# penghao-wu/vstar

Hardware: AMD Instinct MI355X
Metric: searched crops/sec (336x336 tiles, 7B VSM bf16) (higher is better)
Workload: dtype bf16; 1 GPU; BASELINE config 2: 32-crop batches/GPU, CLIP-ViT-L/14@336 (P=576) + LLaMA-7B prefill S=640 + OWL-ViT-B/16@768 + det/SAM heads, records all-gathered per step; seq_len=640, parallelism=dp1

## Files before the change

include/vstar_hip.h:

```cpp
#ifndef VSTAR_HIP_H
#define VSTAR_HIP_H

#include <stdint.h>
#include <stddef.h>

#ifdef __cplusplus
extern "C" {
#endif

#define VSTAR_ABI_VERSION 1

enum { VSTAR_F32 = 0, VSTAR_F16 = 1, VSTAR_BF16 = 2 };

enum {
  VSTAR_OK = 0,
  VSTAR_ERR_INVALID = -1,
  VSTAR_ERR_STATE = -2,
  VSTAR_ERR_MISSING = -3,
  VSTAR_ERR_HIP = -4,
  VSTAR_ERR_NOMEM = -5
};

typedef struct vstar_config {
  int32_t abi_version;
  int32_t clip_image_size;
  int32_t clip_patch;
  int32_t clip_hidden;
  int32_t clip_heads;
  int32_t clip_mlp;
  int32_t clip_layers;
  int32_t clip_select_layer;
  int32_t llm_hidden;
  int32_t llm_heads;
  int32_t llm_mlp;
  int32_t llm_layers;
  int32_t llm_vocab;
  float   llm_rms_eps;
  float   llm_rope_theta;
  int32_t owl_image_size;
  int32_t owl_patch;
  int32_t owl_hidden;
  int32_t owl_heads;
  int32_t owl_mlp;
  int32_t owl_layers;
  int32_t owl_query_dim;
  int32_t max_batch;
  int32_t max_text_len;
  int32_t llm_w8a8;
  int32_t reserved[7];
} vstar_config;

typedef struct vstar_engine vstar_handle;

#define VSTAR_N_BOXES 2304
#define VSTAR_MASK_RES 192
#define VSTAR_MAX_VERIFY 8
typedef struct vstar_result {
  float   pred_logits[VSTAR_N_BOXES];
  float   pred_boxes[VSTAR_N_BOXES * 4];
  float   lowres_mask[VSTAR_MASK_RES * VSTAR_MASK_RES];
  int32_t tf_argmax[VSTAR_MAX_VERIFY];
} vstar_result;

int vstar_create(const vstar_config* cfg, int device, vstar_handle** out);
void vstar_destroy(vstar_handle* h);
const char* vstar_last_error(const vstar_handle* h);
const char* vstar_build_source_hash(void);

int vstar_load_tensor(vstar_handle* h, const char* hf_key, const void* host_ptr, int dtype,
                      int ndim, const int64_t* shape);
int vstar_finalize_weights(vstar_handle* h);

#define VSTAR_F_SKIP_OWL       1u
#define VSTAR_F_DEVICE_INPUTS  2u
#define VSTAR_F_DEVICE_OUTPUT  4u
#define VSTAR_F_NO_SYNC        8u
#define VSTAR_F_INTERNAL_PIXELS 16u
#define VSTAR_F_SHARE_PREFIX   32u
int vstar_vsm_score_batch(vstar_handle* h, int B, const uint16_t* clip_pix, const uint16_t* owl_pix,
                          const int32_t* ids, int L, const int32_t* loc_pos,
                          const int32_t* verify_pos, int n_verify, unsigned flags, vstar_result* out);

int vstar_vsm_score_grouped(vstar_handle* h, int G, int T, const uint16_t* clip_pix, const uint16_t* owl_pix,
                            const int32_t* prefix_ids, int Lp, const int32_t* suffix_ids, int Ls, const int32_t* loc_in_suffix,
                            const int32_t* verify_in_suffix, int n_verify, unsigned flags, vstar_result* out);

int vstar_image_set(vstar_handle* h, const uint8_t* rgb, int height, int width);
int vstar_preprocess_crops(vstar_handle* h, int B, const int32_t* boxes_xyxy);

#define VSTAR_MAX_IMAGE_SLOTS 64
int vstar_image_set_slot(vstar_handle* h, int slot, const uint8_t* rgb, int height, int width);
int vstar_preprocess_crops_slots(vstar_handle* h, int B, const int32_t* boxes_xyxy, const int32_t* slots);
int vstar_image_set_slot_async(vstar_handle* h, int slot, const uint8_t* rgb, int height, int width);

int vstar_vsm_generate(vstar_handle* h, const uint16_t* clip_pix_bf16, const int32_t* ids, int L, int max_new_tokens,
                       int eos_id, unsigned flags, int32_t* out_ids, int32_t* n_out);

int vstar_upsample_mask(vstar_handle* h, const float* lowres, int h_out, int w_out, float* out);
int vstar_upsample_mask_ex(vstar_handle* h, const float* lowres, int h_out, int w_out, int clamp_min0, float* out);

int vstar_heatmap_stats(vstar_handle* h, const float* lowres, int h_out, int w_out, int n_rects, const int32_t* rects_xywh,
                        double* out);
int vstar_heatmap_stats_batch(vstar_handle* h, int n, const float* lowres, const int32_t* out_hw, const int32_t* n_rects,
                              const int32_t* rects_xywh, double* out);

int64_t vstar_debug_read(vstar_handle* h, const char* name, float* out, int64_t cap);

void* vstar_stream(vstar_handle* h);

#define VSTAR_COMM_ID_BYTES 128
int vstar_comm_unique_id(uint8_t* id_out );
int vstar_comm_init(vstar_handle* h, const uint8_t* id, int world, int rank);
int vstar_allgather_results(vstar_handle* h, const vstar_result* local_dev, int n_local, vstar_result* gathered_dev, unsigned flags);
int vstar_comm_destroy(vstar_handle* h);

int vstar_profile_enable(vstar_handle* h, int on);
int vstar_profile_read(vstar_handle* h, double* gemm_ms, int64_t* gemm_launches, double* gemm_flops);
int vstar_profile_read_fp8(vstar_handle* h, double* gemm_ms, int64_t* gemm_launches, double* gemm_flops);

enum { VSTAR_EPI_NONE = 0, VSTAR_EPI_QUICK_GELU = 1, VSTAR_EPI_GELU = 2, VSTAR_EPI_RELU = 3, VSTAR_EPI_SILU_MUL = 4,
       VSTAR_EPI_NOSYNC = 0x100,
       VSTAR_EPI_TILE128 = 0x200,
       VSTAR_EPI_TILE256 = 0x400,
       VSTAR_EPI_TILE4W = 0x800    };

int vstar_op_gemm(void* stream, const uint16_t* dev_A, int64_t lda, const uint16_t* dev_W, const uint16_t* dev_bias,
                  const uint16_t* dev_residual, int64_t ldr, void* dev_C, int64_t ldc, int out_f32,
                  int M, int N, int K, int epilogue);
int vstar_op_gemm_norm(void* stream, const uint16_t* dev_A, int64_t lda, const uint16_t* dev_W, const uint16_t* dev_bias,
                       const uint16_t* dev_residual, int64_t ldr, void* dev_C, int64_t ldc, int M, int N, int K, int epilogue,
                       const float* dev_row_scale, float* dev_sumsq_out, int sumsq_ld);
int vstar_op_rms_rstd(void* stream, const uint16_t* dev_x, const float* dev_partials, int ld, int rows, int cols, float eps,
                      float* dev_r);
int vstar_op_ln_fold(void* stream, uint16_t* dev_W, uint16_t* dev_bias, const uint16_t* dev_g, const uint16_t* dev_b_ln,
                     int n_rows, int K);
int vstar_op_gemm_last_tile(void);
int vstar_op_gemm_plan(int M, int N, int K, int epilogue, int has_residual, int fused_rope, int cus);
int vstar_op_gemm_fp8(void* stream, const uint16_t* dev_A, const uint16_t* dev_W, const uint16_t* dev_bias,
                      const uint16_t* dev_residual, uint16_t* dev_C, int M, int N, int K, int epilogue, int iters, float* gemm_ms);
size_t vstar_op_mx_scale_bytes(int rows, int cols);
int64_t vstar_op_mx_scale_offset(int row, int k_block, int rows);
int vstar_op_quantize_mx(void* stream, const uint16_t* dev_X, uint8_t* dev_q, uint8_t* dev_scales, int rows, int cols);
int vstar_op_gemm_mx(void* stream, const uint8_t* dev_Aq, const uint8_t* dev_a_scales, const float* dev_row_scale, const uint16_t* dev_W,
                     const uint16_t* dev_residual, uint16_t* dev_C, uint8_t* dev_C8, uint8_t* dev_c_scales, float* dev_sumsq, int M, int N, int K,
                     int epilogue, int iters, float* gemm_ms);
int vstar_op_gemm_fp8_mxout(void* stream, const uint16_t* dev_A, const uint16_t* dev_W, uint8_t* dev_C8, uint8_t* dev_c_scales, int M, int N,
                            int K, int iters, float* gemm_ms);
int vstar_op_attention_mx(void* stream, const uint16_t* dev_qkv, uint8_t* dev_out8, uint8_t* dev_scales, int B, int S, int H);
int vstar_w8a8_mx_active(vstar_handle* h);
int vstar_op_layernorm(void* stream, const uint16_t* dev_x, const uint16_t* dev_gamma, const uint16_t* dev_beta,
                       uint16_t* dev_y, int rows, int cols, float eps);
int vstar_op_rmsnorm(void* stream, const uint16_t* dev_x, const uint16_t* dev_gamma, uint16_t* dev_y,
                     int rows, int cols, float eps);
int vstar_op_attention(void* stream, uint16_t* dev_qkv, uint16_t* dev_out, void* dev_workspace, size_t workspace_bytes,
                       int B, int S, int H, int D, int causal, float rope_theta);
size_t vstar_op_attention_workspace(int B, int S, int H, int D);

#ifdef __cplusplus
}
#endif
#endif
```

vstar_amd/_lib.py:

```python
from __future__ import annotations

import ctypes
import os
from ctypes import POINTER, c_char_p, c_double, c_float, c_int, c_int32, c_int64, c_size_t, c_uint, c_uint16, c_void_p

from .config import CVqaConfig, CVstarConfig, MASK_RES, MAX_VERIFY, N_BOXES

LIB_PATH = os.environ.get("VSTAR_LIB") or os.path.join(os.path.dirname(os.path.abspath(__file__)), "libvstar_hip.so")

EXPORTS = [
    "vstar_create", "vstar_destroy", "vstar_last_error", "vstar_load_tensor", "vstar_finalize_weights",
    "vstar_vsm_score_batch", "vstar_upsample_mask", "vstar_debug_read", "vstar_stream", "vstar_profile_enable",
    "vstar_profile_read", "vstar_profile_read_fp8", "vstar_op_gemm", "vstar_op_layernorm", "vstar_op_rmsnorm", "vstar_op_attention",
    "vstar_op_attention_workspace", "vstar_image_set", "vstar_preprocess_crops", "vstar_heatmap_stats", "vstar_heatmap_stats_batch", "vstar_vsm_generate", "vstar_op_gemm_fp8",
    "vstar_op_gemm_last_tile", "vstar_op_gemm_plan", "vstar_op_gemm_norm", "vstar_op_rms_rstd", "vstar_op_ln_fold", "vstar_upsample_mask_ex", "vstar_vsm_score_grouped",
    "vstar_image_set_slot", "vstar_image_set_slot_async", "vstar_preprocess_crops_slots", "vstar_comm_unique_id", "vstar_comm_init", "vstar_allgather_results",
    "vstar_comm_destroy", "vstar_build_source_hash", "vstar_op_mx_scale_bytes", "vstar_op_mx_scale_offset", "vstar_op_quantize_mx",
    "vstar_op_gemm_mx", "vstar_op_gemm_fp8_mxout", "vstar_op_attention_mx", "vstar_w8a8_mx_active",
]

EXPORTS_VQA = [
    "vstar_vqa_create", "vstar_vqa_destroy", "vstar_vqa_last_error", "vstar_vqa_load_tensor", "vstar_vqa_finalize_weights",
    "vstar_vqa_encode_images", "vstar_vqa_forward", "vstar_vqa_debug_read", "vstar_vqa_last_forward_ms", "vstar_vqa_op_gemm",
    "vstar_vqa_forward_sample", "vstar_vqa_op_sample", "vstar_vqa_forward_beam", "vstar_vqa_kv_reorder", "vstar_vqa_kv_copy",
    "vstar_vqa_op_beam_select", "vstar_vqa_forward_score", "vstar_vqa_op_score",
]

F32, F16, BF16 = 0, 1, 2
MAX_IMAGE_SLOTS = 64
EPI_NONE, EPI_QUICK_GELU, EPI_GELU, EPI_RELU, EPI_SILU_MUL = range(5)
EPI_NOSYNC, EPI_TILE128, EPI_TILE256, EPI_TILE4W = 0x100, 0x200, 0x400, 0x800
TILE_4W = 2564
F_SKIP_OWL, F_DEVICE_INPUTS, F_DEVICE_OUTPUT, F_NO_SYNC, F_INTERNAL_PIXELS, F_SHARE_PREFIX = 1, 2, 4, 8, 16, 32


class VstarResult(ctypes.Structure):
    _fields_ = [
        ("pred_logits", c_float * N_BOXES),
        ("pred_boxes", c_float * (N_BOXES * 4)),
        ("lowres_mask", c_float * (MASK_RES * MASK_RES)),
        ("tf_argmax", c_int32 * MAX_VERIFY),
    ]


RESULT_FLOATS = ctypes.sizeof(VstarResult) // 4


class VqaSampling(ctypes.Structure):
    _fields_ = [
        ("temperature", c_float),
        ("top_k", c_int32),
        ("top_p", c_float),
        ("step", ctypes.c_uint32),
        ("seed", ctypes.c_uint64),
        ("stream", ctypes.c_uint64),
    ]


class VstarError(RuntimeError):
    pass


_lib = None


def load() -> ctypes.CDLL:
    global _lib
    if _lib is not None:
        return _lib
    if not os.path.exists(LIB_PATH):
        raise VstarError(f"{LIB_PATH} not built — run __graft_entry__.build() (hipcc --offload-arch=gfx950); "
                         "there is no CPU fallback for the HIP engine")
    import torch
    lib = ctypes.CDLL(LIB_PATH)
    H = c_void_p
    lib.vstar_create.argtypes = [POINTER(CVstarConfig), c_int, POINTER(H)]
    lib.vstar_create.restype = c_int
    lib.vstar_destroy.argtypes = [H]
    lib.vstar_destroy.restype = None
    lib.vstar_last_error.argtypes = [H]
    lib.vstar_last_error.restype = c_char_p
    lib.vstar_build_source_hash.argtypes = []
    lib.vstar_build_source_hash.restype = c_char_p
    lib.vstar_load_tensor.argtypes = [H, c_char_p, c_void_p, c_int, c_int, POINTER(c_int64)]
    lib.vstar_load_tensor.restype = c_int
    lib.vstar_finalize_weights.argtypes = [H]
    lib.vstar_finalize_weights.restype = c_int
    lib.vstar_vsm_score_batch.argtypes = [H, c_int, c_void_p, c_void_p, c_void_p, c_int, c_void_p, c_void_p, c_int, c_uint,
                                          c_void_p]
    lib.vstar_vsm_score_batch.restype = c_int
    lib.vstar_vsm_score_grouped.argtypes = [H, c_int, c_int, c_void_p, c_void_p, c_void_p, c_int, c_void_p, c_int, c_void_p, c_void_p, c_int,
                                            c_uint, c_void_p]
    lib.vstar_vsm_score_grouped.restype = c_int
    lib.vstar_vsm_generate.argtypes = [H, c_void_p, c_void_p, c_int, c_int, c_int, c_uint, c_void_p, c_void_p]
    lib.vstar_vsm_generate.restype = c_int
    lib.vstar_image_set.argtypes = [H, c_void_p, c_int, c_int]
    lib.vstar_image_set.restype = c_int
    lib.vstar_preprocess_crops.argtypes = [H, c_int, c_void_p]
    lib.vstar_preprocess_crops.restype = c_int
    lib.vstar_image_set_slot.argtypes = [H, c_int, c_void_p, c_int, c_int]
    lib.vstar_image_set_slot.restype = c_int
    lib.vstar_image_set_slot_async.argtypes = [H, c_int, c_void_p, c_int, c_int]
    lib.vstar_image_set_slot_async.restype = c_int
    lib.vstar_preprocess_crops_slots.argtypes = [H, c_int, c_void_p, c_void_p]
    lib.vstar_preprocess_crops_slots.restype = c_int
    lib.vstar_comm_unique_id.argtypes = [c_void_p]
    lib.vstar_comm_unique_id.restype = c_int
    lib.vstar_comm_init.argtypes = [H, c_void_p, c_int, c_int]
    lib.vstar_comm_init.restype = c_int
    lib.vstar_allgather_results.argtypes = [H, c_void_p, c_int, c_void_p, ctypes.c_uint]
    lib.vstar_allgather_results.restype = c_int
    lib.vstar_comm_destroy.argtypes = [H]
    lib.vstar_comm_destroy.restype = c_int
    lib.vstar_heatmap_stats.argtypes = [H, c_void_p, c_int, c_int, c_int, c_void_p, c_void_p]
    lib.vstar_heatmap_stats.restype = c_int
    lib.vstar_heatmap_stats_batch.argtypes = [H, c_int, c_void_p, c_void_p, c_void_p, c_void_p, c_void_p]
    lib.vstar_heatmap_stats_batch.restype = c_int
    lib.vstar_upsample_mask.argtypes = [H, c_void_p, c_int, c_int, c_void_p]
    lib.vstar_upsample_mask.restype = c_int
    lib.vstar_upsample_mask_ex.argtypes = [H, c_void_p, c_int, c_int, c_int, c_void_p]
    lib.vstar_upsample_mask_ex.restype = c_int
    lib.vstar_debug_read.argtypes = [H, c_char_p, c_void_p, c_int64]
    lib.vstar_debug_read.restype = c_int64
    lib.vstar_stream.argtypes = [H]
    lib.vstar_stream.restype = c_void_p
    lib.vstar_profile_enable.argtypes = [H, c_int]
    lib.vstar_profile_enable.restype = c_int
    lib.vstar_profile_read.argtypes = [H, POINTER(c_double), POINTER(c_int64), POINTER(c_double)]
    lib.vstar_profile_read.restype = c_int
    lib.vstar_profile_read_fp8.argtypes = [H, POINTER(c_double), POINTER(c_int64), POINTER(c_double)]
    lib.vstar_profile_read_fp8.restype = c_int
    lib.vstar_op_gemm.argtypes = [c_void_p, c_void_p, c_int64, c_void_p, c_void_p, c_void_p, c_int64, c_void_p, c_int64,
                                  c_int, c_int, c_int, c_int, c_int]
    lib.vstar_op_gemm.restype = c_int
    lib.vstar_op_gemm_norm.argtypes = [c_void_p, c_void_p, c_int64, c_void_p, c_void_p, c_void_p, c_int64, c_void_p, c_int64, c_int, c_int, c_int,
                                       c_int, c_void_p, c_void_p, c_int]
    lib.vstar_op_gemm_norm.restype = c_int
    lib.vstar_op_rms_rstd.argtypes = [c_void_p, c_void_p, c_void_p, c_int, c_int, c_int, c_float, c_void_p]
    lib.vstar_op_rms_rstd.restype = c_int
    lib.vstar_op_ln_fold.argtypes = [c_void_p, c_void_p, c_void_p, c_void_p, c_void_p, c_int, c_int]
    lib.vstar_op_ln_fold.restype = c_int
    lib.vstar_op_gemm_last_tile.argtypes = []
    lib.vstar_op_gemm_last_tile.restype = c_int
    lib.vstar_op_gemm_plan.argtypes = [c_int] * 7
    lib.vstar_op_gemm_plan.restype = c_int
    lib.vstar_op_gemm_fp8.argtypes = [c_void_p, c_void_p, c_void_p, c_void_p, c_void_p, c_void_p, c_int, c_int, c_int, c_int, c_int,
                                      POINTER(c_float)]
    lib.vstar_op_gemm_fp8.restype = c_int
    lib.vstar_op_mx_scale_bytes.argtypes = [c_int, c_int]
    lib.vstar_op_mx_scale_bytes.restype = c_size_t
    lib.vstar_op_mx_scale_offset.argtypes = [c_int, c_int, c_int]
    lib.vstar_op_mx_scale_offset.restype = ctypes.c_int64
    lib.vstar_op_quantize_mx.argtypes = [c_void_p, c_void_p, c_void_p, c_void_p, c_int, c_int]
    lib.vstar_op_quantize_mx.restype = c_int
    lib.vstar_op_gemm_mx.argtypes = [c_void_p] * 10 + [c_int, c_int, c_int, c_int, c_int, POINTER(c_float)]
    lib.vstar_op_gemm_mx.restype = c_int
    lib.vstar_op_gemm_fp8_mxout.argtypes = [c_void_p, c_void_p, c_void_p, c_void_p, c_void_p, c_int, c_int, c_int, c_int, POINTER(c_float)]
    lib.vstar_op_gemm_fp8_mxout.restype = c_int
    lib.vstar_op_attention_mx.argtypes = [c_void_p, c_void_p, c_void_p, c_void_p, c_int, c_int, c_int]
    lib.vstar_op_attention_mx.restype = c_int
    lib.vstar_w8a8_mx_active.argtypes = [c_void_p]
    lib.vstar_w8a8_mx_active.restype = c_int
    lib.vstar_op_layernorm.argtypes = [c_void_p, c_void_p, c_void_p, c_void_p, c_void_p, c_int, c_int, c_float]
    lib.vstar_op_layernorm.restype = c_int
    lib.vstar_op_rmsnorm.argtypes = [c_void_p, c_void_p, c_void_p, c_void_p, c_int, c_int, c_float]
    lib.vstar_op_rmsnorm.restype = c_int
    lib.vstar_op_attention.argtypes = [c_void_p, c_void_p, c_void_p, c_void_p, c_size_t, c_int, c_int, c_int, c_int, c_int,
                                       c_float]
    lib.vstar_op_attention.restype = c_int
    lib.vstar_op_attention_workspace.argtypes = [c_int, c_int, c_int, c_int]
    lib.vstar_op_attention_workspace.restype = c_size_t
    lib.vstar_vqa_create.argtypes = [POINTER(CVqaConfig), c_int, POINTER(H)]
    lib.vstar_vqa_create.restype = c_int
    lib.vstar_vqa_destroy.argtypes = [H]
    lib.vstar_vqa_destroy.restype = None
    lib.vstar_vqa_last_error.argtypes = [H]
    lib.vstar_vqa_last_error.restype = c_char_p
    lib.vstar_vqa_load_tensor.argtypes = [H, c_char_p, c_void_p, c_int, c_int, POINTER(c_int64)]
    lib.vstar_vqa_load_tensor.restype = c_int
    lib.vstar_vqa_finalize_weights.argtypes = [H]
    lib.vstar_vqa_finalize_weights.restype = c_int
    lib.vstar_vqa_encode_images.argtypes = [H, c_int, c_void_p, c_int]
    lib.vstar_vqa_encode_images.restype = c_int
    lib.vstar_vqa_forward.argtypes = [H, c_int, c_void_p, c_void_p, c_void_p, c_void_p, c_void_p, c_int, c_void_p, c_void_p,
                                      c_void_p]
    lib.vstar_vqa_forward.restype = c_int
    lib.vstar_vqa_forward_sample.argtypes = [H, c_int, c_void_p, c_void_p, c_void_p, c_void_p, c_void_p, c_int, c_void_p,
                                             c_void_p, c_void_p]
    lib.vstar_vqa_forward_sample.restype = c_int
    lib.vstar_vqa_op_sample.argtypes = [c_void_p, c_int, c_int, c_int, c_int64, c_void_p, c_void_p, c_void_p, c_void_p]
    lib.vstar_vqa_op_sample.restype = c_int
    lib.vstar_vqa_forward_beam.argtypes = [H, c_int, c_void_p, c_void_p, c_void_p, c_void_p, c_void_p, c_int, c_void_p,
                                           c_void_p, c_int, c_void_p, c_int, c_void_p, c_void_p, c_void_p, c_void_p]
    lib.vstar_vqa_forward_beam.restype = c_int
    lib.vstar_vqa_kv_reorder.argtypes = [H, c_int, c_void_p, c_void_p, c_int, c_int]
    lib.vstar_vqa_kv_reorder.restype = c_int
    lib.vstar_vqa_kv_copy.argtypes = [H, c_int, c_int, c_int, c_int]
    lib.vstar_vqa_kv_copy.restype = c_int
    lib.vstar_vqa_op_beam_select.argtypes = [c_void_p, c_int, c_int, c_int, c_int64, c_void_p, c_int, c_void_p, c_int, c_void_p,
                                             c_void_p, c_void_p, c_void_p]
    lib.vstar_vqa_op_beam_select.restype = c_int
    lib.vstar_vqa_forward_score.argtypes = [H, c_int, c_void_p, c_void_p, c_void_p, c_void_p, c_void_p, c_int, c_void_p,
                                            c_void_p, c_void_p, c_void_p]
    lib.vstar_vqa_forward_score.restype = c_int
    lib.vstar_vqa_op_score.argtypes = [c_void_p, c_int, c_int, c_int, c_int64, c_void_p, c_void_p, c_void_p, c_void_p]
    lib.vstar_vqa_op_score.restype = c_int
    lib.vstar_vqa_op_gemm.argtypes = [c_void_p, c_void_p, c_void_p, c_void_p, c_void_p, c_int, c_int, c_int, c_int, c_int,
                                      c_void_p, c_float]
    lib.vstar_vqa_op_gemm.restype = c_int
    lib.vstar_vqa_debug_read.argtypes = [H, c_char_p, c_void_p, c_int64]
    lib.vstar_vqa_debug_read.restype = c_int64
    lib.vstar_vqa_last_forward_ms.argtypes = [H]
    lib.vstar_vqa_last_forward_ms.restype = c_double
    _lib = lib
    return lib


def check_vqa(rc: int, handle=None) -> None:
    if rc != 0:
        msg = load().vstar_vqa_last_error(handle)
        raise VstarError(f"libvstar_hip (vqa) error {rc}: {msg.decode() if msg else '?'}")


def check(rc: int, handle=None) -> None:
    if rc != 0:
        msg = load().vstar_last_error(handle)
        raise VstarError(f"libvstar_hip error {rc}: {msg.decode() if msg else '?'}")
```

vstar_amd/csrc/elementwise.hip:

```cpp
#include "common.hpp"
#include "kernels.hpp"

namespace VS_NS {

namespace {

__global__ void im2col_patch_kernel(const lp_t* __restrict__ pix, lp_t* __restrict__ A, int B, int I, int ps, int Kpad) {
  const int G = I / ps, P = G * G;
  const int K = 3 * ps * ps;
  const int64_t idx = (int64_t)blockIdx.x * blockDim.x + threadIdx.x;
  const int64_t total = (int64_t)B * P * Kpad;
  if (idx >= total) return;
  const int k = (int)(idx % Kpad);
  const int64_t row = idx / Kpad;
  lp_t v = 0;
  if (k < K) {
    const int p = (int)(row % P), b = (int)(row / P);
    const int c = k / (ps * ps), rem = k - c * ps * ps;
    const int ky = rem / ps, kx = rem - ky * ps;
    const int y = (p / G) * ps + ky, x = (p % G) * ps + kx;
    v = pix[(((int64_t)b * 3 + c) * I + y) * I + x];
  }
  A[idx] = v;
}

__global__ void vit_assemble_kernel(const lp_t* __restrict__ patch, const lp_t* __restrict__ cls,
                                    const lp_t* __restrict__ pos, lp_t* __restrict__ tokens, int B, int P, int C) {
  const int cv = C >> 3;
  const int64_t idx = (int64_t)blockIdx.x * blockDim.x + threadIdx.x;
  const int64_t total = (int64_t)B * (P + 1) * cv;
  if (idx >= total) return;
  const int v = (int)(idx % cv);
  const int64_t row = idx / cv;
  const int t = (int)(row % (P + 1)), b = (int)(row / (P + 1));
  const lpx8 a = (t == 0) ? *(const lpx8*)(cls + v * 8)
                            : *(const lpx8*)(patch + ((int64_t)b * P + (t - 1)) * C + v * 8);
  const lpx8 pe = *(const lpx8*)(pos + (int64_t)t * C + v * 8);
  lpx8 o;
#pragma unroll
  for (int e = 0; e < 8; ++e) o[e] = (short)f2lp(lp2f((lp_t)a[e]) + lp2f((lp_t)pe[e]));
  *(lpx8*)(tokens + row * C + v * 8) = o;
}

__global__ void llm_embed_text_kernel(const int32_t* __restrict__ ids, int L, int img_col, int P,
                                      const lp_t* __restrict__ table, int vocab, lp_t* __restrict__ x, int B, int C) {
  const int cv = C >> 3;
  const int T = L - 1;
  const int64_t idx = (int64_t)blockIdx.x * blockDim.x + threadIdx.x;
  const int64_t total = (int64_t)B * T * cv;
  if (idx >= total) return;
  const int v = (int)(idx % cv);
  const int64_t r = idx / cv;
  const int t = (int)(r % T), b = (int)(r / T);
  const int col = t < img_col ? t : t + 1;
  const int s = t < img_col ? t : t + P;
  int id = ids[(int64_t)b * L + col];
  id = id < 0 ? 0 : (id >= vocab ? vocab - 1 : id);
  const int S = T + P;
  *(lpx8*)(x + ((int64_t)b * S + s) * C + v * 8) = *(const lpx8*)(table + (int64_t)id * C + v * 8);
}

__global__ void add_bcast_kernel(const lp_t* __restrict__ a, const lp_t* __restrict__ b, lp_t* __restrict__ out,
                                 int64_t rows, int cols, int64_t b_rows) {
  const int cv = cols >> 3;
  const int64_t idx = (int64_t)blockIdx.x * blockDim.x + threadIdx.x;
  if (idx >= rows * cv) return;
  const int v = (int)(idx % cv);
  const int64_t r = idx / cv;
  const lpx8 x = *(const lpx8*)(a + r * cols + v * 8);
  const lpx8 y = *(const lpx8*)(b + (r % b_rows) * cols + v * 8);
  lpx8 o;
#pragma unroll
  for (int e = 0; e < 8; ++e) o[e] = (short)f2lp(lp2f((lp_t)x[e]) + lp2f((lp_t)y[e]));
  *(lpx8*)(out + r * cols + v * 8) = o;
}

__global__ void bcast_rows_kernel(const lp_t* __restrict__ src, lp_t* __restrict__ dst, int nrep, int64_t rep_stride, int nrows, int cv,
                                  int64_t ld) {
  const int64_t idx = (int64_t)blockIdx.x * blockDim.x + threadIdx.x;
  const int64_t per = (int64_t)nrows * cv;
  if (idx >= per * nrep) return;
  const int r = (int)(idx / per);
  const int64_t rem = idx - (int64_t)r * per;
  const int i = (int)(rem / cv), c = (int)(rem - (int64_t)i * cv);
  *(lpx8*)(dst + ((int64_t)r * rep_stride + i) * ld + c * 8) = *(const lpx8*)(src + (int64_t)i * ld + c * 8);
}

__global__ void add_bcast_repeat_kernel(const lp_t* __restrict__ a, const lp_t* __restrict__ b, lp_t* __restrict__ out, int n_out,
                                        int rep, int rows_per, int cols) {
  const int cv = cols >> 3;
  const int64_t idx = (int64_t)blockIdx.x * blockDim.x + threadIdx.x;
  if (idx >= (int64_t)n_out * rows_per * cv) return;
  const int v = (int)(idx % cv);
  const int64_t r = idx / cv;
  const int n = (int)(r / rows_per), p = (int)(r % rows_per);
  const lpx8 x = *(const lpx8*)(a + ((int64_t)(n / rep) * rows_per + p) * cols + v * 8);
  const lpx8 y = *(const lpx8*)(b + v * 8);
  lpx8 o;
#pragma unroll
  for (int e = 0; e < 8; ++e) o[e] = (short)f2lp(lp2f((lp_t)x[e]) + lp2f((lp_t)y[e]));
  *(lpx8*)(out + r * cols + v * 8) = o;
}

__global__ void owl_cls_mul_kernel(const lp_t* __restrict__ x, lp_t* __restrict__ y, int B, int N, int C) {
  const int cv = C >> 3;
  const int64_t idx = (int64_t)blockIdx.x * blockDim.x + threadIdx.x;
  const int64_t total = (int64_t)B * (N - 1) * cv;
  if (idx >= total) return;
  const int v = (int)(idx % cv);
  const int64_t r = idx / cv;
  const int p = (int)(r % (N - 1)), b = (int)(r / (N - 1));
  const lpx8 t = *(const lpx8*)(x + ((int64_t)b * N + 1 + p) * C + v * 8);
  const lpx8 c = *(const lpx8*)(x + ((int64_t)b * N) * C + v * 8);
  lpx8 o;
#pragma unroll
  for (int e = 0; e < 8; ++e) o[e] = (short)f2lp(lp2f((lp_t)t[e]) * lp2f((lp_t)c[e]));
  *(lpx8*)(y + r * C + v * 8) = o;
}

__global__ void gather_rows_kernel(const lp_t* __restrict__ x, const int32_t* __restrict__ idx_, lp_t* __restrict__ y,
                                   int rows, int cols) {
  const int cv = cols >> 3;
  const int64_t idx = (int64_t)blockIdx.x * blockDim.x + threadIdx.x;
  if (idx >= (int64_t)rows * cv) return;
  const int v = (int)(idx % cv);
  const int r = (int)(idx / cv);
  *(lpx8*)(y + (int64_t)r * cols + v * 8) = *(const lpx8*)(x + (int64_t)idx_[r] * cols + v * 8);
}

__global__ __launch_bounds__(256) void argmax_rows_kernel(const float* __restrict__ x, int cols, int ld, int32_t* out,
                                                          int out_stride) {
  __shared__ float sv[4];
  __shared__ int si[4];
  const int row = blockIdx.x;
  const float* xr = x + (int64_t)row * ld;
  float best = -INFINITY;
  int bi = 0x7fffffff;
  for (int c = threadIdx.x; c < cols; c += 256) {
    const float v = xr[c];
    if (v > best || (v == best && c < bi)) { best = v; bi = c; }
  }
#pragma unroll
  for (int o = 32; o > 0; o >>= 1) {
    const float ov = __shfl_xor(best, o, 64);
    const int oi = __shfl_xor(bi, o, 64);
    if (ov > best || (ov == best && oi < bi)) { best = ov; bi = oi; }
  }
  if ((threadIdx.x & 63) == 0) { sv[threadIdx.x >> 6] = best; si[threadIdx.x >> 6] = bi; }
  __syncthreads();
  if (threadIdx.x == 0) {
    for (int w = 1; w < 4; ++w)
      if (sv[w] > best || (sv[w] == best && si[w] < bi)) { best = sv[w]; bi = si[w]; }
    out[(int64_t)row * out_stride] = bi;
  }
}

inline unsigned nblk(int64_t n) { return (unsigned)((n + 255) / 256); }

}

hipError_t im2col_patch(const lp_t* pix, lp_t* A, int B, int I, int ps, int Kpad, hipStream_t s) {
  const int G = I / ps;
  const int64_t total = (int64_t)B * G * G * Kpad;
  hipLaunchKernelGGL(im2col_patch_kernel, dim3(nblk(total)), dim3(256), 0, s, pix, A, B, I, ps, Kpad);
  return hipGetLastError();
}
hipError_t vit_assemble_tokens(const lp_t* patch, const lp_t* cls, const lp_t* pos, lp_t* tokens, int B, int P,
                               int C, hipStream_t s) {
  if (C % 8) return hipErrorInvalidValue;
  hipLaunchKernelGGL(vit_assemble_kernel, dim3(nblk((int64_t)B * (P + 1) * (C / 8))), dim3(256), 0, s, patch, cls, pos,
                     tokens, B, P, C);
  return hipGetLastError();
}
hipError_t llm_embed_text(const int32_t* ids, int L, int img_col, int P, const lp_t* table, int vocab, lp_t* x, int B,
                          int C, hipStream_t s) {
  if (C % 8) return hipErrorInvalidValue;
  hipLaunchKernelGGL(llm_embed_text_kernel, dim3(nblk((int64_t)B * (L - 1) * (C / 8))), dim3(256), 0, s, ids, L, img_col,
                     P, table, vocab, x, B, C);
  return hipGetLastError();
}
hipError_t add_bcast(const lp_t* a, const lp_t* b, lp_t* out, int64_t rows, int cols, int64_t b_rows, hipStream_t s) {
  if (cols % 8) return hipErrorInvalidValue;
  hipLaunchKernelGGL(add_bcast_kernel, dim3(nblk(rows * (cols / 8))), dim3(256), 0, s, a, b, out, rows, cols, b_rows);
  return hipGetLastError();
}
hipError_t bcast_rows(const lp_t* src, lp_t* dst, int nrep, int64_t rep_stride, int nrows, int cols, int64_t ld, hipStream_t s) {
  if (cols % 8 || nrep <= 0 || nrows <= 0) return hipErrorInvalidValue;
  hipLaunchKernelGGL(bcast_rows_kernel, dim3(nblk((int64_t)nrep * nrows * (cols / 8))), dim3(256), 0, s, src, dst, nrep, rep_stride, nrows,
                     cols / 8, ld);
  return hipGetLastError();
}

hipError_t add_bcast_repeat(const lp_t* a, const lp_t* b, lp_t* out, int n_out, int rep, int rows_per, int cols, hipStream_t s) {
  if (cols % 8 || rep < 1) return hipErrorInvalidValue;
  hipLaunchKernelGGL(add_bcast_repeat_kernel, dim3(nblk((int64_t)n_out * rows_per * (cols / 8))), dim3(256), 0, s, a, b, out, n_out, rep,
                     rows_per, cols);
  return hipGetLastError();
}
hipError_t owl_cls_mul(const lp_t* x, lp_t* y, int B, int N, int C, hipStream_t s) {
  if (C % 8) return hipErrorInvalidValue;
  hipLaunchKernelGGL(owl_cls_mul_kernel, dim3(nblk((int64_t)B * (N - 1) * (C / 8))), dim3(256), 0, s, x, y, B, N, C);
  return hipGetLastError();
}
hipError_t gather_rows(const lp_t* x, const int32_t* idx, lp_t* y, int rows, int cols, hipStream_t s) {
  if (cols % 8) return hipErrorInvalidValue;
  if (rows <= 0) return hipSuccess;
  hipLaunchKernelGGL(gather_rows_kernel, dim3(nblk((int64_t)rows * (cols / 8))), dim3(256), 0, s, x, idx, y, rows, cols);
  return hipGetLastError();
}
hipError_t argmax_rows(const float* x, int rows, int cols, int ld, int32_t* out, int out_stride, hipStream_t s) {
  if (rows <= 0) return hipSuccess;
  hipLaunchKernelGGL(argmax_rows_kernel, dim3(rows), dim3(256), 0, s, x, cols, ld, out, out_stride);
  return hipGetLastError();
}

}
```

vstar_amd/csrc/engine.hip:

```cpp
#include "llm_cached.hpp"
#include "mx.hpp"
#include <atomic>
#include <tuple>
#include <cstring>

namespace {
struct SamAttn { Lin q, k, v, out; int internal; };
struct SamLayer { SamAttn self_attn, t2i, i2t; lp_t *n1g, *n1b, *n2g, *n2b, *n3g, *n3b, *n4g, *n4b; Lin lin1, lin2; };
}

struct vstar_engine : EngineBase {
  vstar_config cfg{};
  VitTower clip, owl;
  Lin projector;
  lp_t* embed = nullptr;
  std::vector<LlmBlock> llm;
  lp_t* final_norm = nullptr;
  Lin lm_head;
  lp_t* rope = nullptr;
  Lin det0, det1, seg0, seg1;
  lp_t *owl_post_g = nullptr, *owl_post_b = nullptr, *owl_ln_g = nullptr, *owl_ln_b = nullptr;
  Lin cls_fused, box0, box1, box2;
  Lin vis_proj;
  lp_t *no_mask = nullptr, *dense_pe = nullptr, *iou_token = nullptr, *mask_tokens = nullptr;
  SamLayer sam_layers[2];
  SamAttn sam_final; lp_t *sam_nfg = nullptr, *sam_nfb = nullptr;
  Lin conv1, conv2; lp_t *ln2d_g = nullptr, *ln2d_b = nullptr;
  Lin hyp0, hyp1, hyp2;

  int Smax = 0;
  uint8_t* lq8 = nullptr; float* lsa = nullptr;
  uint8_t* lmx = nullptr;
  int make_lin8(const Lin& L, Lin8* out, const lp_t* fold_g = nullptr);
  uint8_t* lmxx = nullptr;
  int last_w8a8_chain = 0;
  int lin8(const uint8_t* Aq, const float* sa, const Lin& L, const Lin8& L8, void* C, int64_t ldc, int M, int epi,
           const lp_t* res, int64_t ldr, const lp_t* rope_cs = nullptr, int rope_S = 0, int rope_cols = 0, const uint8_t* a_mx = nullptr,
           uint8_t* c_mx = nullptr, uint8_t* c8 = nullptr, float* sumsq = nullptr);
  bool last_w8a8_mx = false;
  bool fused_rope = true;
  bool fold_norms = true;
  float *lr = nullptr, *lpart = nullptr;
  lp_t *lx = nullptr, *lh = nullptr, *lqkv = nullptr, *latt = nullptr, *lact = nullptr;
  lp_t* hsel = nullptr;
  lp_t *sel_att = nullptr, *sel_x = nullptr, *sel_h = nullptr, *sel_act = nullptr;
  float* vlogits = nullptr;
  lp_t *fc_tmp = nullptr, *emb_det = nullptr, *emb_seg = nullptr;
  int32_t *d_ids = nullptr, *d_rowidx = nullptr, *d_argmax = nullptr;
  lp_t *d_clip_pix = nullptr, *d_owl_pix = nullptr;
  lp_t *owl_feats_pre = nullptr, *owl_feats = nullptr, *box_t0 = nullptr, *box_t1 = nullptr;
  float *cls_emb = nullptr, *box_raw = nullptr;
  lp_t *s_src = nullptr, *s_keys = nullptr, *s_kpe = nullptr, *s_ia = nullptr, *s_ib = nullptr, *s_ic = nullptr;
  lp_t *s_tok0 = nullptr, *s_q = nullptr, *s_qpe = nullptr, *s_ta = nullptr, *s_tb = nullptr, *s_tc = nullptr, *s_td = nullptr,
         *s_mlp = nullptr;
  lp_t *s_col1 = nullptr, *s_c1 = nullptr, *s_c1n = nullptr, *s_col2 = nullptr, *s_c2 = nullptr, *s_hyp_in = nullptr,
         *s_hyp_a = nullptr, *s_hyp_b = nullptr, *s_hyper = nullptr;
  int32_t* d_tokidx = nullptr;
  vstar_result* d_results = nullptr;
  int last_B = 0, last_S = 0;
  void* d_stats = nullptr;
  void* d_stats_batch = nullptr; size_t stats_batch_cap = 0;
  void* comm = nullptr;
  float* d_up = nullptr; size_t up_cap = 0;
  struct ImageSlot { uint8_t* d = nullptr; size_t cap = 0; int H = 0, W = 0; };
  ImageSlot images[VSTAR_MAX_IMAGE_SLOTS];
  hipStream_t stream_up = nullptr;
  hipEvent_t ev_up[VSTAR_MAX_IMAGE_SLOTS] = {};
  std::atomic<int> up_pending[VSTAR_MAX_IMAGE_SLOTS] = {};
  uint8_t* h_stage[2] = {nullptr, nullptr};
  size_t stage_cap[2] = {0, 0};
  hipEvent_t ev_stage[2] = {nullptr, nullptr};
  bool stage_used[2] = {false, false};
  int stage_next = 0;
  hipEvent_t ev_pre = nullptr;
  int image_upload_async(int slot, const uint8_t* rgb, int height, int width);
  uint8_t* d_temp = nullptr; size_t temp_cap = 0;
  int32_t* d_tables = nullptr; size_t tables_cap = 0;
  PreJob* d_jobs = nullptr;
  lp_t* d_lut = nullptr;
  std::vector<int32_t> h_tables;
  std::vector<PreJob> h_jobs;
  struct AxisTab { int off_b, off_c, ks; };
  int preprocess(int B, const int32_t* boxes, const int32_t* slots = nullptr);
  std::vector<int32_t> h_rowidx;
  struct ScoreSig {
    int B, L, nv, img_col, psh; unsigned flags; const void *cpix, *opix;
    bool operator<(const ScoreSig& o) const {
      return std::tie(B, L, nv, img_col, psh, flags, cpix, opix) < std::tie(o.B, o.L, o.nv, o.img_col, o.psh, o.flags, o.cpix, o.opix);
    }
  };
  std::map<ScoreSig, hipGraphExec_t> score_graphs;
  int32_t* h_ids_pin = nullptr; int32_t* h_rowidx_pin = nullptr;
  bool score_graph_on = false;
  int score_graph_max_B = 8;
  int64_t score_graph_replays = 0;
  int score_body(int B, int L, int n_verify, unsigned flags, int img_col, int psh, const lp_t* cpix, const lp_t* opix, bool skip_owl,
                 const int32_t* ids_src, const int32_t* rowidx_src, size_t n_rowidx);

  LlmCached gen;
  lp_t* gen_feats = nullptr;
  int generate(const lp_t* clip_pix, const int32_t* ids, int L, int max_new, int eos_id, unsigned flags, int32_t* out_ids,
               int32_t* n_out);
  int finalize();
  int score(int B, const lp_t* clip_pix, const lp_t* owl_pix, const int32_t* ids, int L, const int32_t* loc_pos,
            const int32_t* verify_pos, int n_verify, unsigned flags, vstar_result* out);
  int score_grouped(int G, int T, const lp_t* clip_pix, const lp_t* owl_pix, const int32_t* prefix_ids, int Lp,
                    const int32_t* suffix_ids, int Ls, const int32_t* loc_in_suffix, const int32_t* verify_in_suffix, int n_verify,
                    unsigned flags, vstar_result* out);
  int grp_R0 = 0, grp_Lc = 0;
  int psh_Lp = 0;
  int llm_forward(int nseq, int S, int nsel);
  int llm_heads(int nrec, int n_verify);
  int owl_heads_sam(const lp_t* opix, int Bimg, int nrec, int img_div);
  int owl_features(const lp_t* opix, int Bimg);
  int owl_finish(int Bimg, int nrec, int img_div);
  hipStream_t stream2 = nullptr;
  hipEvent_t ev_fork = nullptr, ev_join = nullptr;
  int owl_overlap = -1;
  bool fork_owl(const lp_t* opix, int Bimg, int* rc);
  int finish_records(int nrec, int n_verify, unsigned flags, vstar_result* out);
  int stage_pixels(int B, const lp_t* clip_pix, const lp_t* owl_pix, unsigned flags, bool skip_owl, const lp_t** cpix, const lp_t** opix);
  lp_t* grp_feats = nullptr;
  int32_t* d_src = nullptr;
  std::vector<int32_t> h_src;
  int sam_attn(const SamAttn& a, const lp_t* q_in, int nq, const lp_t* k_in, const lp_t* v_in, int nk, int B,
               lp_t* pq, lp_t* pk, lp_t* pv, lp_t* att, lp_t* out, const lp_t* res);
  int make_sam_attn(const std::string& pre, SamAttn* a);
};

int vstar_engine::make_sam_attn(const std::string& pre, SamAttn* a) {
  RC(make_lin({pre + "q_proj.weight"}, {pre + "q_proj.bias"}, &a->q, 256));
  RC(make_lin({pre + "k_proj.weight"}, {pre + "k_proj.bias"}, &a->k, 256));
  RC(make_lin({pre + "v_proj.weight"}, {pre + "v_proj.bias"}, &a->v, 256));
  a->internal = a->q.N;
  RC(make_lin({pre + "out_proj.weight"}, {pre + "out_proj.bias"}, &a->out, a->internal));
  return 0;
}

int vstar_engine::make_lin8(const Lin& L, Lin8* out, const lp_t* fold_g) {
  const int Npad = (L.N + 255) / 256 * 256;
  if (L.K % 256) { set_error("W8A8 needs K % 256 == 0"); return VSTAR_ERR_INVALID; }
  RC(dalloc(&out->W, (size_t)Npad * L.K));
  RC(dalloc(&out->s, (size_t)Npad));
  if (fold_g) {
    lp_t* tmp = nullptr;
    HIPCHK(hipMalloc((void**)&tmp, (size_t)Npad * L.K * sizeof(lp_t)));
    hipError_t e = hipMemcpyAsync(tmp, L.W, (size_t)Npad * L.K * sizeof(lp_t), hipMemcpyDeviceToDevice, stream);
    if (e == hipSuccess) e = scale_cols_lp(tmp, fold_g, Npad, L.K, stream);
    if (e == hipSuccess) e = quantize_rows_fp8(tmp, L.K, out->W, L.K, out->s, Npad, L.K, stream);
    if (e == hipSuccess) e = hipStreamSynchronize(stream);
    hipFree(tmp);
    HIPCHK(e);
    return 0;
  }
  KCHK(quantize_rows_fp8(L.W, L.K, out->W, L.K, out->s, Npad, L.K, stream));
  return 0;
}

int vstar_engine::lin8(const uint8_t* Aq, const float* sa, const Lin& L, const Lin8& L8, void* C, int64_t ldc, int M, int epi,
                       const lp_t* res, int64_t ldr, const lp_t* rope_cs, int rope_S, int rope_cols, const uint8_t* a_mx, uint8_t* c_mx,
                       uint8_t* c8, float* sumsq) {
  GemmParams p{};
  p.A = (const lp_t*)Aq; p.lda = L.K; p.W = (const lp_t*)L8.W; p.res = res; p.ldr = ldr; p.C = C; p.ldc = ldc;
  p.M = M; p.N = L.N; p.K = L.K; p.a_scale = sa; p.w_scale = L8.s; p.a_mx = a_mx; p.c_mx = c_mx;
  p.c8 = c8; p.ldc8 = L.N; p.sumsq_out = c8 ? sumsq : nullptr; p.sumsq_ld = L.N / 64;
  p.rope_cs = rope_cs; p.rope_S = rope_S; p.rope_cols = rope_cols; p.rope_R0 = grp_R0; p.rope_Lc = grp_Lc;
  return gemm(p, epi, false);
}

int vstar_engine::finalize() {
  if (finalized) { set_error("weights already finalized"); return VSTAR_ERR_STATE; }
  const vstar_config& c = cfg;
  const int maxB = c.max_batch;
  HIPCHK(hipSetDevice(device));
  const int clip_blocks = c.clip_layers + 1 + c.clip_select_layer;
  if (clip_blocks < 0 || clip_blocks > c.clip_layers) { set_error("bad clip_select_layer"); return VSTAR_ERR_INVALID; }
  RC(build_tower(clip, "clip.vision_model.", "pre_layrnorm", c.clip_image_size, c.clip_patch, c.clip_hidden, c.clip_heads,
                 c.clip_mlp, clip_blocks, maxB));
  RC(make_lin({"model.mm_projector.weight"}, {"model.mm_projector.bias"}, &projector, c.clip_hidden));
  const int H = c.llm_hidden;
  if (H != c.llm_heads * 128) { set_error("LLaMA head dim must be 128"); return VSTAR_ERR_INVALID; }
  if (c.llm_mlp % 16) { set_error("llm_mlp must be a multiple of 16"); return VSTAR_ERR_INVALID; }
  RC(upload_vec("model.embed_tokens.weight", &embed, (int64_t)c.llm_vocab * H));
  std::vector<int> perm(2 * c.llm_mlp);
  for (int r = 0; r < 2 * c.llm_mlp; ++r) {
    const int blk = r / 32, w = r % 32;
    perm[r] = w < 16 ? blk * 16 + w : c.llm_mlp + blk * 16 + (w - 16);
  }
  llm.resize(c.llm_layers);
  for (int i = 0; i < c.llm_layers; ++i) {
    const std::string lp = "model.layers." + std::to_string(i) + ".";
    LlmBlock& b = llm[i];
    RC(upload_vec(lp + "input_layernorm.weight", &b.in_norm, H));
    RC(upload_vec(lp + "post_attention_layernorm.weight", &b.post_norm, H));
    RC(make_lin({lp + "self_attn.q_proj.weight", lp + "self_attn.k_proj.weight", lp + "self_attn.v_proj.weight"}, {}, &b.qkv, H));
    RC(make_lin({lp + "self_attn.o_proj.weight"}, {}, &b.o, H));
    RC(make_lin({lp + "mlp.gate_proj.weight", lp + "mlp.up_proj.weight"}, {}, &b.gate_up, H, &perm));
    RC(make_lin({lp + "mlp.down_proj.weight"}, {}, &b.down, c.llm_mlp));
  }
  if (c.llm_w8a8) fold_norms = false;
  if (fold_norms) {
    if (H % 64) { set_error("fold_norms needs llm_hidden % 64 == 0"); return VSTAR_ERR_INVALID; }
    for (auto& b : llm) {
      KCHK(scale_cols_lp(b.qkv.W, b.in_norm, (int64_t)((b.qkv.N + 255) / 256 * 256), b.qkv.K, stream));
      KCHK(scale_cols_lp(b.gate_up.W, b.post_norm, (int64_t)((b.gate_up.N + 255) / 256 * 256), b.gate_up.K, stream));
      KCHK(fill_lp(b.in_norm, H, 1.0f, stream));
      KCHK(fill_lp(b.post_norm, H, 1.0f, stream));
    }
    HIPCHK(hipStreamSynchronize(stream));
  }
  if (c.llm_w8a8) {
    for (auto& b : llm) {
      RC(make_lin8(b.qkv, &b.qkv8));
      RC(make_lin8(b.o, &b.o8));
      RC(make_lin8(b.gate_up, &b.gate_up8));
      RC(make_lin8(b.down, &b.down8));
      RC(make_lin8(b.qkv, &b.qkv8f, b.in_norm));
      RC(make_lin8(b.gate_up, &b.gate_up8f, b.post_norm));
    }
  }
  RC(upload_vec("model.norm.weight", &final_norm, H));
  RC(make_lin({"lm_head.weight"}, {}, &lm_head, H));
  Smax = c.max_text_len - 1 + clip.P;
  {
    const int rope_rows = Smax + 160;
    std::vector<lp_t> tab((size_t)rope_rows * 128);
    for (int s = 0; s < rope_rows; ++s)
      for (int i = 0; i < 64; ++i) {
        const float inv = 1.0f / powf(c.llm_rope_theta, (float)(2 * i) / 128.0f);
        const float f = (float)s * inv;
        tab[(size_t)s * 128 + i] = f2lp(cosf(f));
        tab[(size_t)s * 128 + 64 + i] = f2lp(sinf(f));
      }
    RC(dalloc(&rope, tab.size()));
    HIPCHK(hipMemcpy(rope, tab.data(), tab.size() * 2, hipMemcpyHostToDevice));
  }
  const size_t lrows = (size_t)(maxB + 1) * Smax;
  RC(dalloc(&lx, lrows * H));
  HIPCHK(hipMemset(lx, 0, lrows * H * sizeof(lp_t)));
  RC(dalloc(&lh, lrows * H));
  RC(dalloc(&lqkv, lrows * 3 * H));
  RC(dalloc(&latt, lrows * H));
  RC(dalloc(&lr, lrows));
  RC(dalloc(&lpart, lrows * (size_t)(H / 64 > 0 ? H / 64 : 1)));
  RC(dalloc(&lact, lrows * c.llm_mlp));
  if (c.llm_w8a8) {
    RC(dalloc(&lq8, lrows * (size_t)(c.llm_mlp > H ? c.llm_mlp : H)));
    RC(dalloc(&lsa, lrows));
    RC(dalloc(&lmx, (lrows + 127) / 128 * 128 * (size_t)((c.llm_mlp > H ? c.llm_mlp : H) / 32 + 1)));
    RC(dalloc(&lmxx, (lrows + 127) / 128 * 128 * (size_t)(H / 32 + 1)));
  }
  RC(dalloc(&hsel, (size_t)maxB * (1 + VSTAR_MAX_VERIFY) * H));
  RC(dalloc(&sel_att, (size_t)maxB * (1 + VSTAR_MAX_VERIFY) * H));
  RC(dalloc(&sel_x, (size_t)maxB * (1 + VSTAR_MAX_VERIFY) * H));
  RC(dalloc(&sel_h, (size_t)maxB * (1 + VSTAR_MAX_VERIFY) * H));
  RC(dalloc(&sel_act, (size_t)maxB * (1 + VSTAR_MAX_VERIFY) * c.llm_mlp));
  RC(dalloc(&vlogits, (size_t)maxB * VSTAR_MAX_VERIFY * c.llm_vocab));
  RC(dalloc(&d_ids, (size_t)maxB * c.max_text_len));
  RC(dalloc(&d_rowidx, (size_t)maxB * (1 + VSTAR_MAX_VERIFY)));
  if (hipHostMalloc((void**)&h_ids_pin, (size_t)maxB * c.max_text_len * 4, hipHostMallocDefault) != hipSuccess ||
      hipHostMalloc((void**)&h_rowidx_pin, (size_t)maxB * (1 + VSTAR_MAX_VERIFY) * 4, hipHostMallocDefault) != hipSuccess) {
    (void)hipGetLastError();
    h_ids_pin = h_rowidx_pin = nullptr;
  }
  RC(dalloc(&d_argmax, (size_t)maxB * VSTAR_MAX_VERIFY));
  RC(dalloc(&d_clip_pix, (size_t)maxB * 3 * c.clip_image_size * c.clip_image_size));
  RC(dalloc(&d_owl_pix, (size_t)maxB * 3 * c.owl_image_size * c.owl_image_size));
  RC(dalloc(&d_results, (size_t)maxB));
  RC(dalloc(&grp_feats, (size_t)maxB * clip.P * H));
  RC(dalloc(&d_src, lrows));
  HIPCHK(hipMemset(d_results, 0, sizeof(vstar_result) * maxB));
  RC(make_lin({"model.text_hidden_fcs_det.0.0.weight"}, {"model.text_hidden_fcs_det.0.0.bias"}, &det0, H));
  RC(make_lin({"model.text_hidden_fcs_det.0.2.weight"}, {"model.text_hidden_fcs_det.0.2.bias"}, &det1, H));
  RC(make_lin({"model.text_hidden_fcs_seg.0.0.weight"}, {"model.text_hidden_fcs_seg.0.0.bias"}, &seg0, H));
  RC(make_lin({"model.text_hidden_fcs_seg.0.2.weight"}, {"model.text_hidden_fcs_seg.0.2.bias"}, &seg1, H));
  if (det1.N != c.owl_query_dim || seg1.N != 256) { set_error("text_hidden_fcs output dims"); return VSTAR_ERR_INVALID; }
  RC(dalloc(&fc_tmp, (size_t)maxB * H));
  RC(dalloc(&emb_det, (size_t)maxB * det1.N));
  RC(dalloc(&emb_seg, (size_t)maxB * 256));
  const int OH = c.owl_hidden;
  RC(build_tower(owl, "model.owlvit.vision_model.", "pre_layernorm", c.owl_image_size, c.owl_patch, OH, c.owl_heads,
                 c.owl_mlp, c.owl_layers, maxB));
  if (owl.P != VSTAR_N_BOXES) { set_error("OWL-ViT grid must be 48x48"); return VSTAR_ERR_INVALID; }
  RC(upload_vec("model.owlvit.vision_model.post_layernorm.weight", &owl_post_g, OH));
  RC(upload_vec("model.owlvit.vision_model.post_layernorm.bias", &owl_post_b, OH));
  RC(upload_vec("model.owlvit.layer_norm.weight", &owl_ln_g, OH));
  RC(upload_vec("model.owlvit.layer_norm.bias", &owl_ln_b, OH));
  RC(make_lin({"model.owlvit.class_head.dense0.weight", "model.owlvit.class_head.logit_shift.weight",
               "model.owlvit.class_head.logit_scale.weight"},
              {"model.owlvit.class_head.dense0.bias", "model.owlvit.class_head.logit_shift.bias",
               "model.owlvit.class_head.logit_scale.bias"}, &cls_fused, OH));
  if (cls_fused.N != c.owl_query_dim + 2) { set_error("class head dims"); return VSTAR_ERR_INVALID; }
  RC(make_lin({"model.owlvit.box_head.dense0.weight"}, {"model.owlvit.box_head.dense0.bias"}, &box0, OH));
  RC(make_lin({"model.owlvit.box_head.dense1.weight"}, {"model.owlvit.box_head.dense1.bias"}, &box1, OH));
  RC(make_lin({"model.owlvit.box_head.dense2.weight"}, {"model.owlvit.box_head.dense2.bias"}, &box2, OH));
  const size_t prow = (size_t)maxB * owl.P;
  RC(dalloc(&owl_feats_pre, prow * OH));
  RC(dalloc(&owl_feats, prow * OH));
  RC(dalloc(&box_t0, prow * OH));
  RC(dalloc(&box_t1, prow * OH));
  RC(dalloc(&cls_emb, prow * (size_t)(cls_fused.N + 2)));
  RC(dalloc(&box_raw, prow * 4));
  RC(make_lin({"model.visual_projection.weight"}, {}, &vis_proj, OH));
  RC(upload_vec("model.prompt_encoder.no_mask_embed.weight", &no_mask, 256));
  RC(upload_vec("sam.dense_pe", &dense_pe, (int64_t)owl.P * 256));
  RC(upload_vec("model.mask_decoder.iou_token.weight", &iou_token, 256));
  RC(upload_vec("model.mask_decoder.mask_tokens.weight", &mask_tokens, 4 * 256));
  for (int i = 0; i < 2; ++i) {
    const std::string lp = "model.mask_decoder.transformer.layers." + std::to_string(i) + ".";
    SamLayer& L = sam_layers[i];
    RC(make_sam_attn(lp + "self_attn.", &L.self_attn));
    RC(make_sam_attn(lp + "cross_attn_token_to_image.", &L.t2i));
    RC(make_sam_attn(lp + "cross_attn_image_to_token.", &L.i2t));
    RC(upload_vec(lp + "norm1.weight", &L.n1g, 256)); RC(upload_vec(lp + "norm1.bias", &L.n1b, 256));
    RC(upload_vec(lp + "norm2.weight", &L.n2g, 256)); RC(upload_vec(lp + "norm2.bias", &L.n2b, 256));
    RC(upload_vec(lp + "norm3.weight", &L.n3g, 256)); RC(upload_vec(lp + "norm3.bias", &L.n3b, 256));
    RC(upload_vec(lp + "norm4.weight", &L.n4g, 256)); RC(upload_vec(lp + "norm4.bias", &L.n4b, 256));
    RC(make_lin({lp + "mlp.lin1.weight"}, {lp + "mlp.lin1.bias"}, &L.lin1, 256));
    RC(make_lin({lp + "mlp.lin2.weight"}, {lp + "mlp.lin2.bias"}, &L.lin2, L.lin1.N));
  }
  RC(make_sam_attn("model.mask_decoder.transformer.final_attn_token_to_image.", &sam_final));
  RC(upload_vec("model.mask_decoder.transformer.norm_final_attn.weight", &sam_nfg, 256));
  RC(upload_vec("model.mask_decoder.transformer.norm_final_attn.bias", &sam_nfb, 256));
  RC(make_lin({"model.mask_decoder.output_upscaling.0.conv.weight"}, {"model.mask_decoder.output_upscaling.0.conv.bias"},
              &conv1, 256 * 9, nullptr, true));
  RC(upload_vec("model.mask_decoder.output_upscaling.1.weight", &ln2d_g, 64));
  RC(upload_vec("model.mask_decoder.output_upscaling.1.bias", &ln2d_b, 64));
  RC(make_lin({"model.mask_decoder.output_upscaling.3.conv.weight"}, {"model.mask_decoder.output_upscaling.3.conv.bias"},
              &conv2, 64 * 9, nullptr, true));
  RC(make_lin({"model.mask_decoder.output_hypernetworks_mlps.0.layers.0.weight"},
              {"model.mask_decoder.output_hypernetworks_mlps.0.layers.0.bias"}, &hyp0, 256));
  RC(make_lin({"model.mask_decoder.output_hypernetworks_mlps.0.layers.1.weight"},
              {"model.mask_decoder.output_hypernetworks_mlps.0.layers.1.bias"}, &hyp1, 256));
  RC(make_lin({"model.mask_decoder.output_hypernetworks_mlps.0.layers.2.weight"},
              {"model.mask_decoder.output_hypernetworks_mlps.0.layers.2.bias"}, &hyp2, 256));
  if (conv1.N != 64 || conv2.N != 32 || hyp2.N != 32) { set_error("mask decoder dims"); return VSTAR_ERR_INVALID; }
  RC(dalloc(&s_src, prow * 256)); RC(dalloc(&s_keys, prow * 256)); RC(dalloc(&s_kpe, prow * 256));
  RC(dalloc(&s_ia, prow * 256)); RC(dalloc(&s_ib, prow * 256)); RC(dalloc(&s_ic, prow * 256));
  const size_t trow = (size_t)maxB * 6;
  RC(dalloc(&s_tok0, trow * 256)); RC(dalloc(&s_q, trow * 256)); RC(dalloc(&s_qpe, trow * 256));
  RC(dalloc(&s_ta, trow * 256)); RC(dalloc(&s_tb, trow * 256)); RC(dalloc(&s_tc, trow * 256)); RC(dalloc(&s_td, trow * 256));
  RC(dalloc(&s_mlp, trow * 2048));
  RC(dalloc(&s_col1, (size_t)maxB * 96 * 96 * 2304));
  RC(dalloc(&s_c1, (size_t)maxB * 96 * 96 * 64));
  RC(dalloc(&s_c1n, (size_t)maxB * 96 * 96 * 64));
  RC(dalloc(&s_col2, (size_t)maxB * 192 * 192 * 576));
  RC(dalloc(&s_c2, (size_t)maxB * 192 * 192 * 32));
  RC(dalloc(&s_hyp_in, (size_t)maxB * 256)); RC(dalloc(&s_hyp_a, (size_t)maxB * 256)); RC(dalloc(&s_hyp_b, (size_t)maxB * 256));
  RC(dalloc(&s_hyper, (size_t)maxB * 32));
  RC(dalloc(&d_tokidx, (size_t)maxB));
  {
    std::vector<int32_t> tix(maxB);
    for (int b = 0; b < maxB; ++b) tix[b] = b * 6 + 1;
    HIPCHK(hipMemcpy(d_tokidx, tix.data(), (size_t)maxB * 4, hipMemcpyHostToDevice));
  }
  RC(dalloc(&d_jobs, (size_t)maxB * 2));
  RC(dalloc(&d_lut, (size_t)3 * 256));
  {
    lp_t lut[3 * 256];
    clip_norm_lut(lut);
    HIPCHK(hipMemcpy(d_lut, lut, sizeof(lut), hipMemcpyHostToDevice));
  }
  HIPCHK(hipDeviceSynchronize());
  staged.clear();
  finalized = true;
  return 0;
}

int vstar_engine::preprocess(int B, const int32_t* boxes, const int32_t* slots) {
  if (!finalized) { set_error("vstar_finalize_weights has not been called"); return VSTAR_ERR_STATE; }
  if (B <= 0 || B > cfg.max_batch || !boxes) { set_error("bad preprocess arguments"); return VSTAR_ERR_INVALID; }
  for (int b = 0; b < B; ++b) {
    const int sl = slots ? slots[b] : 0;
    if (sl < 0 || sl >= VSTAR_MAX_IMAGE_SLOTS) { set_error("image slot out of range"); return VSTAR_ERR_INVALID; }
    if (!images[sl].d) { set_error("no image resident in the slot: call vstar_image_set / vstar_image_set_slot first"); return VSTAR_ERR_STATE; }
  }
  HIPCHK(hipSetDevice(device));
  HIPCHK(hipStreamSynchronize(stream));
  for (int b = 0; b < B; ++b) {
    const int sl = slots ? slots[b] : 0;
    if (up_pending[sl].exchange(0)) HIPCHK(hipStreamWaitEvent(stream, ev_up[sl], 0));
  }
  const int I = cfg.clip_image_size, O = cfg.owl_image_size;
  h_tables.clear();
  h_jobs.assign((size_t)B * 2, PreJob{});
  std::map<std::pair<int, int>, AxisTab> cache;
  auto axis = [&](int in_size, int out_size) -> AxisTab {
    auto key = std::make_pair(in_size, out_size);
    auto it = cache.find(key);
    if (it != cache.end()) return it->second;
    std::vector<int32_t> bnd, cf;
    int ks = 0;
    pil_bicubic_coeffs(in_size, out_size, &bnd, &cf, &ks);
    AxisTab t{(int)h_tables.size(), 0, ks};
    h_tables.insert(h_tables.end(), bnd.begin(), bnd.end());
    t.off_c = (int)h_tables.size();
    h_tables.insert(h_tables.end(), cf.begin(), cf.end());
    cache[key] = t;
    return t;
  };
  size_t temp_bytes = 0;
  int max_h_clip = 0, max_h_owl = 0;
  for (int b = 0; b < B; ++b) {
    const int x0 = boxes[b * 4], y0 = boxes[b * 4 + 1], x1 = boxes[b * 4 + 2], y1 = boxes[b * 4 + 3];
    const int cw = x1 - x0, ch = y1 - y0;
    const ImageSlot& im = images[slots ? slots[b] : 0];
    if (x0 < 0 || y0 < 0 || cw <= 0 || ch <= 0 || x1 > im.W || y1 > im.H) { set_error("crop box outside the image"); return VSTAR_ERR_INVALID; }
    const int side = cw > ch ? cw : ch;
    for (int which = 0; which < 2; ++which) {
      PreJob& j = h_jobs[(size_t)b * 2 + which];
      j.x0 = x0; j.y0 = y0; j.cw = cw; j.ch = ch;
      j.img = im.d; j.img_w = im.W;
      j.in_w = which == 0 ? side : cw;
      j.in_h = which == 0 ? side : ch;
      j.out = which == 0 ? I : O;
      const AxisTab hx = axis(j.in_w, j.out), vy = axis(j.in_h, j.out);
      j.hb_off = hx.off_b; j.hc_off = hx.off_c; j.hks = hx.ks;
      j.vb_off = vy.off_b; j.vc_off = vy.off_c; j.vks = vy.ks;
      j.temp_off = (int64_t)temp_bytes;
      temp_bytes += ((size_t)j.in_h * j.out * 3 + 255) / 256 * 256;
      j.out_off = (int64_t)b * 3 * j.out * j.out;
      if (which == 0) max_h_clip = j.in_h > max_h_clip ? j.in_h : max_h_clip;
      else max_h_owl = j.in_h > max_h_owl ? j.in_h : max_h_owl;
    }
  }
  if (temp_bytes > temp_cap) {
    if (d_temp) HIPCHK(hipFree(d_temp));
    temp_cap = temp_bytes + temp_bytes / 4;
    HIPCHK(hipMalloc((void**)&d_temp, temp_cap));
  }
  if (h_tables.size() > tables_cap) {
    if (d_tables) HIPCHK(hipFree(d_tables));
    tables_cap = h_tables.size() * 2;
    HIPCHK(hipMalloc((void**)&d_tables, tables_cap * 4));
  }
  HIPCHK(hipMemcpyAsync(d_tables, h_tables.data(), h_tables.size() * 4, hipMemcpyHostToDevice, stream));
  HIPCHK(hipMemcpyAsync(d_jobs, h_jobs.data(), h_jobs.size() * sizeof(PreJob), hipMemcpyHostToDevice, stream));
  KCHK(preprocess_launch(d_jobs, d_tables, d_temp, d_lut, d_clip_pix, 0, B, I, max_h_clip, stream));
  KCHK(preprocess_launch(d_jobs, d_tables, d_temp, d_lut, d_owl_pix, 1, B, O, max_h_owl, stream));
  HIPCHK(hipEventRecord(ev_pre, stream));
  return 0;
}

int vstar_engine::image_upload_async(int slot, const uint8_t* rgb, int height, int width) {
  HIPCHK(hipSetDevice(device));
  const size_t bytes = (size_t)height * width * 3;
  if (!ev_up[slot]) HIPCHK(hipEventCreateWithFlags(&ev_up[slot], hipEventDisableTiming));
  ImageSlot& im = images[slot];
  if (bytes > im.cap) {
    if (up_pending[slot].load()) HIPCHK(hipEventSynchronize(ev_up[slot]));
    if (im.d) { HIPCHK(hipStreamSynchronize(stream)); HIPCHK(hipFree(im.d)); }
    im.d = nullptr; im.cap = 0;
    HIPCHK(hipMalloc((void**)&im.d, bytes));
    im.cap = bytes;
  }
  const int k = stage_next;
  stage_next ^= 1;
  if (stage_used[k]) HIPCHK(hipEventSynchronize(ev_stage[k]));
  if (bytes > stage_cap[k]) {
    if (h_stage[k]) HIPCHK(hipHostFree(h_stage[k]));
    h_stage[k] = nullptr; stage_cap[k] = 0;
    HIPCHK(hipHostMalloc((void**)&h_stage[k], bytes, hipHostMallocDefault));
    stage_cap[k] = bytes;
  }
  memcpy(h_stage[k], rgb, bytes);
  HIPCHK(hipStreamWaitEvent(stream_up, ev_pre, 0));
  HIPCHK(hipMemcpyAsync(im.d, h_stage[k], bytes, hipMemcpyHostToDevice, stream_up));
  HIPCHK(hipEventRecord(ev_stage[k], stream_up));
  stage_used[k] = true;
  HIPCHK(hipEventRecord(ev_up[slot], stream_up));
  im.H = height;
  im.W = width;
  up_pending[slot].store(1);
  return 0;
}

int vstar_engine::sam_attn(const SamAttn& a, const lp_t* q_in, int nq, const lp_t* k_in, const lp_t* v_in, int nk,
                           int B, lp_t* pq, lp_t* pk, lp_t* pv, lp_t* att, lp_t* out, const lp_t* res) {
  const int I = a.internal;
  RC(lin(q_in, 256, a.q, pq, I, B * nq));
  RC(lin(k_in, 256, a.k, pk, I, B * nk));
  RC(lin(v_in, 256, a.v, pv, I, B * nk));
  KCHK(small_attention(pq, pk, pv, att, B, nq, nk, 8, I / 8, stream));
  RC(lin(att, I, a.out, out, 256, B * nq, VSTAR_EPI_NONE, res, 256));
  return 0;
}

namespace {
__global__ void sam_tokens_kernel(const lp_t* iou, const lp_t* mask_tokens, const lp_t* seg, lp_t* out, int B) {
  const int64_t idx = (int64_t)blockIdx.x * blockDim.x + threadIdx.x;
  if (idx >= (int64_t)B * 6 * 256) return;
  const int c = (int)(idx % 256), t = (int)((idx / 256) % 6), b = (int)(idx / (6 * 256));
  out[idx] = t == 0 ? iou[c] : (t < 5 ? mask_tokens[(t - 1) * 256 + c] : seg[b * 256 + c]);
}
}

int vstar_engine::stage_pixels(int B, const lp_t* clip_pix, const lp_t* owl_pix, unsigned flags, bool skip_owl, const lp_t** cpix,
                               const lp_t** opix) {
  const vstar_config& c = cfg;
// ... 119 lines not shown
      KCHK(rmsnorm_lp(sel_x, b.post_norm, sel_h, nsel, H, c.llm_rms_eps, nullptr, stream));
      RC(lin(sel_h, H, b.gate_up, sel_act, c.llm_mlp, nsel, VSTAR_EPI_SILU_MUL));
      RC(lin(sel_act, c.llm_mlp, b.down, sel_x, H, nsel, VSTAR_EPI_NONE, sel_x, H));
      break;
    }
    if (chain) {
      RC(lin8((const uint8_t*)latt, nullptr, b.o, b.o8, lx, H, rows, VSTAR_EPI_NONE, lx, H, nullptr, 0, 0, lmx, lmxx, lq8, lpart));
      KCHK(rms_rstd_partials(lpart, H / 64, rows, H, c.llm_rms_eps, lr, stream));
      RC(lin8(lq8, lr, b.gate_up, b.gate_up8f, lact, c.llm_mlp, rows, VSTAR_EPI_SILU_MUL, nullptr, 0, nullptr, 0, 0, lmxx, lmx));
      RC(lin8((const uint8_t*)lact, nullptr, b.down, b.down8, lx, H, rows, VSTAR_EPI_NONE, lx, H, nullptr, 0, 0, lmx, lmxx, lq8, lpart));
    } else if (mx) {
      RC(lin8((const uint8_t*)latt, nullptr, b.o, b.o8, lx, H, rows, VSTAR_EPI_NONE, lx, H, nullptr, 0, 0, lmx, nullptr));
      KCHK(rmsnorm_quant_fp8(lx, b.post_norm, lq8, lsa, rows, H, c.llm_rms_eps, stream));
      RC(lin8(lq8, lsa, b.gate_up, b.gate_up8, lact, c.llm_mlp, rows, VSTAR_EPI_SILU_MUL, nullptr, 0, nullptr, 0, 0, nullptr, lmx));
      RC(lin8((const uint8_t*)lact, nullptr, b.down, b.down8, lx, H, rows, VSTAR_EPI_NONE, lx, H, nullptr, 0, 0, lmx, nullptr));
    } else if (w8) {
      KCHK(quantize_rows_fp8(latt, H, lq8, H, lsa, rows, H, stream));
      RC(lin8(lq8, lsa, b.o, b.o8, lx, H, rows, VSTAR_EPI_NONE, lx, H));
      KCHK(rmsnorm_quant_fp8(lx, b.post_norm, lq8, lsa, rows, H, c.llm_rms_eps, stream));
      RC(lin8(lq8, lsa, b.gate_up, b.gate_up8, lact, c.llm_mlp, rows, VSTAR_EPI_SILU_MUL, nullptr, 0));
      KCHK(quantize_rows_fp8(lact, c.llm_mlp, lq8, c.llm_mlp, lsa, rows, c.llm_mlp, stream));
      RC(lin8(lq8, lsa, b.down, b.down8, lx, H, rows, VSTAR_EPI_NONE, lx, H));
    } else {
      if (fold) {
        next_sumsq = lpart; next_sumsq_ld = H / 64;
        RC(lin(latt, H, b.o, lx, H, M, VSTAR_EPI_NONE, lx, H));
        KCHK(rms_rstd_partials(lpart, H / 64, nrows, H, c.llm_rms_eps, lr, stream));
        next_row_scale = lr;
        RC(lin(lx, H, b.gate_up, lact, c.llm_mlp, M, VSTAR_EPI_SILU_MUL));
        next_sumsq = lpart; next_sumsq_ld = H / 64;
        RC(lin(lact, c.llm_mlp, b.down, lx, H, M, VSTAR_EPI_NONE, lx, H));
      } else {
        RC(lin(latt, H, b.o, lx, H, M, VSTAR_EPI_NONE, lx, H));
        KCHK(rmsnorm_lp(lx, b.post_norm, lh, nrows, H, c.llm_rms_eps, nullptr, stream));
        RC(lin(lh, H, b.gate_up, lact, c.llm_mlp, M, VSTAR_EPI_SILU_MUL));
        RC(lin(lact, c.llm_mlp, b.down, lx, H, M, VSTAR_EPI_NONE, lx, H));
      }
    }
  }
  return 0;
}

int vstar_engine::llm_heads(int nrec, int n_verify) {
  const vstar_config& c = cfg;
  const int H = c.llm_hidden;
  const int nsel = nrec * (1 + n_verify);
  KCHK(rmsnorm_lp(sel_x, final_norm, hsel, nsel, H, c.llm_rms_eps, nullptr, stream));
  if (n_verify > 0) {
    RC(lin(hsel + (size_t)nrec * H, H, lm_head, vlogits, c.llm_vocab, nrec * n_verify, VSTAR_EPI_NONE, nullptr, 0, true));
    KCHK(argmax_rows(vlogits, nrec * n_verify, c.llm_vocab, c.llm_vocab, d_argmax, 1, stream));
  }
  RC(lin(hsel, H, det0, fc_tmp, H, nrec, VSTAR_EPI_RELU));
  RC(lin(fc_tmp, H, det1, emb_det, det1.N, nrec));
  RC(lin(hsel, H, seg0, fc_tmp, H, nrec, VSTAR_EPI_RELU));
  RC(lin(fc_tmp, H, seg1, emb_seg, 256, nrec));
  return 0;
}

int vstar_engine::owl_heads_sam(const lp_t* opix, int Bimg, int nrec, int img_div) {
  RC(owl_features(opix, Bimg));
  return owl_finish(Bimg, nrec, img_div);
}

struct OwlJoinGuard {
  hipStream_t s2;
  bool armed;
  ~OwlJoinGuard() {
    if (!armed || !s2) return;
    hipStreamCaptureStatus st = hipStreamCaptureStatusNone;
    if (hipStreamIsCapturing(s2, &st) == hipSuccess && st != hipStreamCaptureStatusNone) return;
    (void)hipStreamSynchronize(s2);
  }
};

bool vstar_engine::fork_owl(const lp_t* opix, int Bimg, int* rc) {
  *rc = 0;
  const bool want = owl_overlap >= 0 ? owl_overlap != 0 : Bimg <= 8;
  if (!want || profile || !stream2) return false;
  if (hipEventRecord(ev_fork, stream) != hipSuccess || hipStreamWaitEvent(stream2, ev_fork, 0) != hipSuccess) {
    set_error("owl overlap: fork failed"); *rc = VSTAR_ERR_HIP; return false;
  }
  std::swap(stream, stream2);
  *rc = owl_features(opix, Bimg);
  std::swap(stream, stream2);
  if (*rc == 0 && hipEventRecord(ev_join, stream2) != hipSuccess) { set_error("owl overlap: join event failed"); *rc = VSTAR_ERR_HIP; }
  return true;
}

int vstar_engine::owl_features(const lp_t* opix, int Bimg) {
  const vstar_config& c = cfg;
  const int OH = c.owl_hidden, NP = owl.P, irow = Bimg * NP;
  RC(run_tower(owl, opix, Bimg));
  KCHK(layernorm_lp(owl.x, owl_post_g, owl_post_b, owl.h, Bimg * owl.N, OH, 1e-5f, nullptr, 0, stream));
  KCHK(owl_cls_mul(owl.h, owl_feats_pre, Bimg, owl.N, OH, stream));
  KCHK(layernorm_lp(owl_feats_pre, owl_ln_g, owl_ln_b, owl_feats, irow, OH, 1e-5f, nullptr, 0, stream));
  const int cld = cls_fused.N + 2;
  RC(lin(owl_feats, OH, cls_fused, cls_emb, cld, irow, VSTAR_EPI_NONE, nullptr, 0, true));
  RC(lin(owl_feats, OH, box0, box_t0, OH, irow, VSTAR_EPI_GELU));
  RC(lin(box_t0, OH, box1, box_t1, OH, irow, VSTAR_EPI_GELU));
  RC(lin(box_t1, OH, box2, box_raw, 4, irow, VSTAR_EPI_NONE, nullptr, 0, true));
  RC(lin(owl_feats, OH, vis_proj, s_src, 256, irow));
  return 0;
}

int vstar_engine::owl_finish(int Bimg, int nrec, int img_div) {
  const vstar_config& c = cfg;
  const int B = nrec;
  const int NP = owl.P, prow = nrec * NP;
  const int rstride = (int)(sizeof(vstar_result) / 4);
  float* res_f = (float*)d_results;
  const int cld = cls_fused.N + 2;
  (void)Bimg;
  KCHK(owl_class_logits(cls_emb, cld, c.owl_query_dim, emb_det, res_f + offsetof(vstar_result, pred_logits) / 4, rstride, nrec,
                        NP, stream, img_div));
  KCHK(owl_box_finish(box_raw, 4, res_f + offsetof(vstar_result, pred_boxes) / 4, rstride, nrec, owl.grid, stream, img_div));
  if (img_div <= 1) {
    KCHK(add_bcast(s_src, no_mask, s_keys, prow, 256, 1, stream));
  } else {
    KCHK(add_bcast_repeat(s_src, no_mask, s_keys, nrec, img_div, NP, 256, stream));
  }
  hipLaunchKernelGGL(sam_tokens_kernel, dim3((B * 6 * 256 + 255) / 256), dim3(256), 0, stream, iou_token, mask_tokens,
                     emb_seg, s_tok0, B);
  KCHK(hipGetLastError());
  const int T = 6, trow = B * T;
  HIPCHK(hipMemcpyAsync(s_q, s_tok0, (size_t)trow * 256 * 2, hipMemcpyDeviceToDevice, stream));
  for (int i = 0; i < 2; ++i) {
    SamLayer& Ly = sam_layers[i];
    if (i == 0) {
      RC(sam_attn(Ly.self_attn, s_q, T, s_q, s_q, T, B, s_ta, s_tb, s_tc, s_td, s_qpe, nullptr));
    } else {
      KCHK(add_bcast(s_q, s_tok0, s_mlp, trow, 256, trow, stream));
      RC(sam_attn(Ly.self_attn, s_mlp, T, s_mlp, s_q, T, B, s_ta, s_tb, s_tc, s_td, s_qpe, s_q));
    }
    KCHK(layernorm_lp(s_qpe, Ly.n1g, Ly.n1b, s_q, trow, 256, 1e-5f, nullptr, 0, stream));
    KCHK(add_bcast(s_q, s_tok0, s_qpe, trow, 256, trow, stream));
    KCHK(add_bcast(s_keys, dense_pe, s_kpe, prow, 256, NP, stream));
    RC(sam_attn(Ly.t2i, s_qpe, T, s_kpe, s_keys, NP, B, s_ta, s_ia, s_ib, s_td, s_tb, s_q));
    KCHK(layernorm_lp(s_tb, Ly.n2g, Ly.n2b, s_q, trow, 256, 1e-5f, nullptr, 0, stream));
    RC(lin(s_q, 256, Ly.lin1, s_mlp, Ly.lin1.N, trow, VSTAR_EPI_RELU));
    RC(lin(s_mlp, Ly.lin1.N, Ly.lin2, s_tb, 256, trow, VSTAR_EPI_NONE, s_q, 256));
    KCHK(layernorm_lp(s_tb, Ly.n3g, Ly.n3b, s_q, trow, 256, 1e-5f, nullptr, 0, stream));
    KCHK(add_bcast(s_q, s_tok0, s_qpe, trow, 256, trow, stream));
    RC(sam_attn(Ly.i2t, s_kpe, NP, s_qpe, s_q, T, B, s_ia, s_ta, s_tb, s_ib, s_ic, s_keys));
    KCHK(layernorm_lp(s_ic, Ly.n4g, Ly.n4b, s_keys, prow, 256, 1e-5f, nullptr, 0, stream));
  }
  KCHK(add_bcast(s_q, s_tok0, s_qpe, trow, 256, trow, stream));
  KCHK(add_bcast(s_keys, dense_pe, s_kpe, prow, 256, NP, stream));
  RC(sam_attn(sam_final, s_qpe, T, s_kpe, s_keys, NP, B, s_ta, s_ia, s_ib, s_td, s_tb, s_q));
  KCHK(layernorm_lp(s_tb, sam_nfg, sam_nfb, s_q, trow, 256, 1e-5f, nullptr, 0, stream));
  KCHK(gather_rows(s_q, d_tokidx, s_hyp_in, B, 256, stream));
  RC(lin(s_hyp_in, 256, hyp0, s_hyp_a, 256, B, VSTAR_EPI_RELU));
  RC(lin(s_hyp_a, 256, hyp1, s_hyp_b, 256, B, VSTAR_EPI_RELU));
  RC(lin(s_hyp_b, 256, hyp2, s_hyper, 32, B));
  KCHK(upsample2x_im2col3x3(s_keys, s_col1, B, 48, 48, 256, stream));
  RC(lin(s_col1, 2304, conv1, s_c1, 64, B * 96 * 96));
  KCHK(layernorm_lp(s_c1, ln2d_g, ln2d_b, s_c1n, B * 96 * 96, 64, 1e-6f, nullptr, 1, stream));
  KCHK(upsample2x_im2col3x3(s_c1n, s_col2, B, 96, 96, 64, stream));
  RC(lin(s_col2, 576, conv2, s_c2, 32, B * 192 * 192, VSTAR_EPI_GELU));
  KCHK(hyper_mask(s_hyper, s_c2, res_f + offsetof(vstar_result, lowres_mask) / 4, rstride, B, 192 * 192, 32, stream));
  return 0;
}

int vstar_engine::finish_records(int nrec, int n_verify, unsigned flags, vstar_result* out) {
  if (n_verify > 0) {
    HIPCHK(hipMemcpy2DAsync((char*)d_results + offsetof(vstar_result, tf_argmax), sizeof(vstar_result), d_argmax,
                            (size_t)n_verify * 4, (size_t)n_verify * 4, nrec, hipMemcpyDeviceToDevice, stream));
  }
  if (out) {
    HIPCHK(hipMemcpyAsync(out, d_results, sizeof(vstar_result) * nrec,
                          (flags & VSTAR_F_DEVICE_OUTPUT) ? hipMemcpyDeviceToDevice : hipMemcpyDeviceToHost, stream));
  }
  if (!(flags & VSTAR_F_NO_SYNC)) {
    HIPCHK(hipStreamSynchronize(stream));
    collect_profile();
  }
  return 0;
}

int vstar_engine::score(int B, const lp_t* clip_pix, const lp_t* owl_pix, const int32_t* ids, int L,
                        const int32_t* loc_pos, const int32_t* verify_pos, int n_verify, unsigned flags,
                        vstar_result* out) {
  if (!finalized) { set_error("vstar_finalize_weights has not been called"); return VSTAR_ERR_STATE; }
  const vstar_config& c = cfg;
  if (B <= 0 || B > c.max_batch) { set_error("B out of range"); return VSTAR_ERR_INVALID; }
  if (L < 2 || L > c.max_text_len) { set_error("L out of range"); return VSTAR_ERR_INVALID; }
  if (n_verify < 0 || n_verify > VSTAR_MAX_VERIFY) { set_error("n_verify out of range"); return VSTAR_ERR_INVALID; }
  const bool internal_pix = flags & VSTAR_F_INTERNAL_PIXELS;
  if (!ids || !loc_pos || (!clip_pix && !internal_pix) || (n_verify && !verify_pos)) { set_error("null input"); return VSTAR_ERR_INVALID; }
  const bool skip_owl = flags & VSTAR_F_SKIP_OWL;
  if (!skip_owl && !owl_pix && !internal_pix) { set_error("null owl_pix"); return VSTAR_ERR_INVALID; }
  HIPCHK(hipSetDevice(device));
  int img_col = -1;
  for (int b = 0; b < B; ++b) {
    int cnt = 0, col = -1;
    for (int j = 0; j < L; ++j)
      if (ids[(size_t)b * L + j] == -200) { cnt++; col = j; }
    if (cnt != 1) { set_error("each ids row must contain exactly one -200 image token"); return VSTAR_ERR_INVALID; }
    if (b == 0) img_col = col;
    else if (col != img_col) { set_error("image token column differs across the batch"); return VSTAR_ERR_INVALID; }
  }
  const int P = clip.P, S = L - 1 + P, H = c.llm_hidden;
  std::vector<int32_t>& rowidx = h_rowidx;
  rowidx.assign((size_t)B * (1 + n_verify), 0);
  for (int b = 0; b < B; ++b) {
    if (loc_pos[b] < 0 || loc_pos[b] >= S) { set_error("loc_pos out of range"); return VSTAR_ERR_INVALID; }
    rowidx[b] = b * S + loc_pos[b];
    for (int v = 0; v < n_verify; ++v) {
      const int pv = verify_pos[(size_t)b * n_verify + v];
      if (pv < 0 || pv >= S) { set_error("verify_pos out of range"); return VSTAR_ERR_INVALID; }
      rowidx[(size_t)B + (size_t)b * n_verify + v] = b * S + pv;
    }
  }
  const lp_t *cpix = nullptr, *opix = nullptr;
  RC(stage_pixels(B, clip_pix, owl_pix, flags, skip_owl, &cpix, &opix));
  int psh = 0;
  if ((flags & VSTAR_F_SHARE_PREFIX) && !c.llm_w8a8 && img_col >= 16 && 2 * img_col <= S) {
    bool same = true;
    for (int b = 1; b < B && same; ++b) same = memcmp(ids, ids + (size_t)b * L, (size_t)img_col * 4) == 0;
    if (same) psh = img_col;
  }
  last_B = B; last_S = S;
  const bool graphs_on = score_graph_on;
  const bool dev_pix = (flags & (VSTAR_F_INTERNAL_PIXELS | VSTAR_F_DEVICE_INPUTS)) != 0;
  grp_R0 = grp_Lc = 0;
  if (graphs_on && dev_pix && B <= score_graph_max_B && !profile && h_ids_pin && h_rowidx_pin && !(flags & VSTAR_F_NO_SYNC)) {
    memcpy(h_ids_pin, ids, (size_t)B * L * 4);
    memcpy(h_rowidx_pin, rowidx.data(), rowidx.size() * 4);
    const ScoreSig sig{B, L, n_verify, img_col, psh, flags & ~(unsigned)VSTAR_F_NO_SYNC, cpix, opix};
    auto it = score_graphs.find(sig);
    if (it != score_graphs.end() && it->second) {
      HIPCHK(hipGraphLaunch(it->second, stream));
      ++score_graph_replays;
      return finish_records(B, n_verify, flags, out);
    }
    if (it != score_graphs.end()) {
      hipGraph_t graph = nullptr;
      if (hipStreamBeginCapture(stream, hipStreamCaptureModeThreadLocal) == hipSuccess) {
        const int rc = score_body(B, L, n_verify, flags, img_col, psh, cpix, opix, skip_owl, h_ids_pin, h_rowidx_pin, rowidx.size());
        const hipError_t ce = hipStreamEndCapture(stream, &graph);
        hipGraphExec_t exec = nullptr;
        if (rc == 0 && ce == hipSuccess && graph && hipGraphInstantiate(&exec, graph, nullptr, nullptr, 0) == hipSuccess && exec) {
          hipGraphDestroy(graph);
          it->second = exec;
          HIPCHK(hipGraphLaunch(exec, stream));
          ++score_graph_replays;
          return finish_records(B, n_verify, flags, out);
        }
        if (graph) hipGraphDestroy(graph);
        (void)hipGetLastError();
        score_graphs.erase(it);
        score_graph_max_B = 0;
        set_error("");
      } else {
        (void)hipGetLastError();
        score_graph_max_B = 0;
      }
    } else {
      score_graphs[sig] = nullptr;
    }
    RC(score_body(B, L, n_verify, flags, img_col, psh, cpix, opix, skip_owl, h_ids_pin, h_rowidx_pin, rowidx.size()));
    return finish_records(B, n_verify, flags, out);
  }
  RC(score_body(B, L, n_verify, flags, img_col, psh, cpix, opix, skip_owl, ids, rowidx.data(), rowidx.size()));
  return finish_records(B, n_verify, flags, out);
}

int vstar_engine::score_body(int B, int L, int n_verify, unsigned flags, int img_col, int psh, const lp_t* cpix, const lp_t* opix,
                             bool skip_owl, const int32_t* ids_src, const int32_t* rowidx_src, size_t n_rowidx) {
  const vstar_config& c = cfg;
  const int P = clip.P, S = L - 1 + P, H = c.llm_hidden;
  HIPCHK(hipMemcpyAsync(d_ids, ids_src, (size_t)B * L * 4, hipMemcpyHostToDevice, stream));
  HIPCHK(hipMemcpyAsync(d_rowidx, rowidx_src, n_rowidx * 4, hipMemcpyHostToDevice, stream));
  int frc_owl = 0;
  const bool forked = !skip_owl && fork_owl(opix, B, &frc_owl);
  OwlJoinGuard join_guard{stream2, forked || frc_owl != 0};
  RC(frc_owl);
  grp_R0 = grp_Lc = 0;

  RC(run_tower(clip, cpix, B));
  {
    GemmParams p{};
    p.A = clip.x; p.lda = clip.hidden; p.a_group = P; p.a_gstride = clip.N; p.a_off = 1;
    p.W = projector.W; p.bias = projector.b; p.res = nullptr;
    p.C = lx; p.ldc = H; p.c_group = P; p.c_gstride = S; p.c_off = img_col;
    p.M = B * P; p.N = projector.N; p.K = projector.K;
    RC(gemm(p, VSTAR_EPI_NONE, false));
  }
  KCHK(llm_embed_text(d_ids, L, img_col, P, embed, c.llm_vocab, lx, B, H, stream));
  psh_Lp = psh;
  if (psh_Lp)
    HIPCHK(hipMemcpyAsync(lx + ((size_t)B * S + psh_Lp) * H, lx, (size_t)psh_Lp * H * sizeof(lp_t), hipMemcpyDeviceToDevice, stream));
  const int frc = llm_forward(B, S, B * (1 + n_verify));
  psh_Lp = 0;
  RC(frc);
  RC(llm_heads(B, n_verify));
  if (!skip_owl) {
    if (forked) {
      HIPCHK(hipStreamWaitEvent(stream, ev_join, 0));
      join_guard.armed = false;
      RC(owl_finish(B, B, 1));
    } else {
      RC(owl_heads_sam(opix, B, B, 1));
    }
  }
  return 0;
}

int vstar_engine::score_grouped(int G, int T, const lp_t* clip_pix, const lp_t* owl_pix, const int32_t* prefix_ids, int Lp,
                                const int32_t* suffix_ids, int Ls, const int32_t* loc_in_suffix, const int32_t* verify_in_suffix,
                                int n_verify, unsigned flags, vstar_result* out) {
  if (!finalized) { set_error("vstar_finalize_weights has not been called"); return VSTAR_ERR_STATE; }
// ... 250 lines not shown
  hipSetDevice(h->device);
  const size_t bytes = (size_t)height * width * 3;
  if (hipStreamSynchronize(h->stream) != hipSuccess) { h->set_error("stream sync failed"); return VSTAR_ERR_HIP; }
  if (h->up_pending[slot].exchange(0)) hipEventSynchronize(h->ev_up[slot]);
  auto& im = h->images[slot];
  if (bytes > im.cap) {
    if (im.d) hipFree(im.d);
    im.d = nullptr;
    im.cap = 0;
    if (hipMalloc((void**)&im.d, bytes) != hipSuccess) { h->set_error("hipMalloc(image) failed"); return VSTAR_ERR_NOMEM; }
    im.cap = bytes;
  }
  if (hipMemcpy(im.d, rgb, bytes, hipMemcpyHostToDevice) != hipSuccess) { h->set_error("image upload failed"); return VSTAR_ERR_HIP; }
  im.H = height;
  im.W = width;
  return VSTAR_OK;
}

int vstar_image_set(vstar_handle* h, const uint8_t* rgb, int height, int width) { return vstar_image_set_slot(h, 0, rgb, height, width); }

int vstar_image_set_slot_async(vstar_handle* h, int slot, const uint8_t* rgb, int height, int width) {
  if (!h || !rgb || height <= 0 || width <= 0 || slot < 0 || slot >= VSTAR_MAX_IMAGE_SLOTS) { tls_error() = "bad argument"; return VSTAR_ERR_INVALID; }
  return h->image_upload_async(slot, rgb, height, width);
}

int vstar_preprocess_crops_slots(vstar_handle* h, int B, const int32_t* boxes_xyxy, const int32_t* slots) {
  if (!h) { tls_error() = "null handle"; return VSTAR_ERR_INVALID; }
  return h->preprocess(B, boxes_xyxy, slots);
}

int vstar_preprocess_crops(vstar_handle* h, int B, const int32_t* boxes_xyxy) { return vstar_preprocess_crops_slots(h, B, boxes_xyxy, nullptr); }

int vstar_heatmap_stats(vstar_handle* h, const float* lowres, int h_out, int w_out, int n_rects, const int32_t* rects_xywh,
                        double* out) {
  if (!h || !lowres || !out || h_out <= 0 || w_out <= 0 || n_rects < 0 || n_rects > 8 || (n_rects && !rects_xywh)) {
    tls_error() = "bad argument";
    return VSTAR_ERR_INVALID;
  }
  int32_t hw[2] = {h_out, w_out}, rects[32] = {0};
  if (n_rects) memcpy(rects, rects_xywh, (size_t)n_rects * 16);
  double all[11];
  const int rc = vstar_heatmap_stats_batch(h, 1, lowres, hw, &n_rects, rects, all);
  if (rc != VSTAR_OK) return rc;
  memcpy(out, all, sizeof(double) * (3 + n_rects));
  return VSTAR_OK;
}

int vstar_heatmap_stats_batch(vstar_handle* h, int n, const float* lowres, const int32_t* out_hw, const int32_t* n_rects,
                              const int32_t* rects_xywh, double* out) {
  if (!h || n < 0 || (n && (!lowres || !out_hw || !n_rects || !rects_xywh || !out))) { tls_error() = "bad argument"; return VSTAR_ERR_INVALID; }
  if (n == 0) return VSTAR_OK;
  int64_t max_pixels = 0;
  for (int i = 0; i < n; ++i) {
    if (out_hw[2 * i] <= 0 || out_hw[2 * i + 1] <= 0 || n_rects[i] < 0 || n_rects[i] > 8) { tls_error() = "bad argument"; return VSTAR_ERR_INVALID; }
    const int64_t px = (int64_t)out_hw[2 * i] * out_hw[2 * i + 1];
    max_pixels = px > max_pixels ? px : max_pixels;
  }
  hipSetDevice(h->device);
  constexpr size_t MAPF = (size_t)VSTAR_MASK_RES * VSTAR_MASK_RES;
  const size_t per = MAPF * 4 + 11 * 8 + 32 * 4 + 2 * 4 + 2 * 4 + 2 * 4;
  const size_t need = per * (size_t)n;
  if (need > h->stats_batch_cap) {
    if (hipStreamSynchronize(h->stream) != hipSuccess) { h->set_error("stream sync failed"); return VSTAR_ERR_HIP; }
    if (h->d_stats_batch) hipFree(h->d_stats_batch);
    h->d_stats_batch = nullptr; h->stats_batch_cap = 0;
    const size_t want = need + need / 2;
    if (hipMalloc(&h->d_stats_batch, want) != hipSuccess) { h->set_error("hipMalloc failed in vstar_heatmap_stats_batch"); return VSTAR_ERR_NOMEM; }
    h->stats_batch_cap = want;
  }
  char* base = (char*)h->d_stats_batch;
  float* d_low = (float*)base;
  double* d_out = (double*)(base + MAPF * 4 * n);
  int* d_rects = (int*)(base + (MAPF * 4 + 11 * 8) * n);
  unsigned* d_mm = (unsigned*)(base + (MAPF * 4 + 11 * 8 + 32 * 4) * n);
  int* d_hw = (int*)(base + (MAPF * 4 + 11 * 8 + 32 * 4 + 2 * 4) * n);
  int* d_nr = (int*)(base + (MAPF * 4 + 11 * 8 + 32 * 4 + 2 * 4 + 2 * 4) * n);
  bool ok = hipMemcpyAsync(d_low, lowres, MAPF * 4 * n, hipMemcpyHostToDevice, h->stream) == hipSuccess;
  ok = ok && hipMemcpyAsync(d_rects, rects_xywh, (size_t)32 * 4 * n, hipMemcpyHostToDevice, h->stream) == hipSuccess;
  ok = ok && hipMemcpyAsync(d_hw, out_hw, (size_t)2 * 4 * n, hipMemcpyHostToDevice, h->stream) == hipSuccess;
  ok = ok && hipMemcpyAsync(d_nr, n_rects, (size_t)4 * n, hipMemcpyHostToDevice, h->stream) == hipSuccess;
  ok = ok && heat_stats_batch(d_low, VSTAR_MASK_RES, VSTAR_MASK_RES, d_hw, d_rects, d_nr, n, max_pixels, d_out, d_mm, h->stream) == hipSuccess;
  ok = ok && hipMemcpyAsync(out, d_out, sizeof(double) * 11 * n, hipMemcpyDeviceToHost, h->stream) == hipSuccess;
  ok = ok && hipStreamSynchronize(h->stream) == hipSuccess;
  if (!ok) { h->set_error("vstar_heatmap_stats_batch: HIP failure"); return VSTAR_ERR_HIP; }
  return VSTAR_OK;
}

int vstar_upsample_mask(vstar_handle* h, const float* lowres, int h_out, int w_out, float* out) {
  return vstar_upsample_mask_ex(h, lowres, h_out, w_out, 1, out);
}

int vstar_upsample_mask_ex(vstar_handle* h, const float* lowres, int h_out, int w_out, int clamp_min0, float* out) {
  if (!h || !lowres || !out || h_out <= 0 || w_out <= 0) { tls_error() = "bad argument"; return VSTAR_ERR_INVALID; }
  hipSetDevice(h->device);
  const size_t nin = (size_t)VSTAR_MASK_RES * VSTAR_MASK_RES, nout = (size_t)h_out * w_out;
  if (nin + nout > h->up_cap) {
    if (hipStreamSynchronize(h->stream) != hipSuccess) { h->set_error("stream sync failed"); return VSTAR_ERR_HIP; }
    if (h->d_up) hipFree(h->d_up);
    h->d_up = nullptr; h->up_cap = 0;
    const size_t want = nin + nout + nout / 4;
    if (hipMalloc((void**)&h->d_up, want * 4) != hipSuccess) { h->set_error("hipMalloc failed in vstar_upsample_mask"); return VSTAR_ERR_NOMEM; }
    h->up_cap = want;
  }
  float *din = h->d_up, *dout = h->d_up + nin;
  hipError_t e;
  const char* what = "H2D copy";
  if ((e = hipMemcpyAsync(din, lowres, nin * 4, hipMemcpyHostToDevice, h->stream)) == hipSuccess) {
    what = "resize kernel";
    if ((e = resize_bilinear_clamp(din, VSTAR_MASK_RES, VSTAR_MASK_RES, dout, h_out, w_out, h->stream, clamp_min0)) == hipSuccess) {
      what = "D2H copy";
      if ((e = hipMemcpyAsync(out, dout, nout * 4, hipMemcpyDeviceToHost, h->stream)) == hipSuccess) {
        what = "stream sync";
        e = hipStreamSynchronize(h->stream);
      }
    }
  }
  if (e != hipSuccess) {
    char dbg[256];
    hipPointerAttribute_t at{};
    const hipError_t pa = hipPointerGetAttributes(&at, din);
    snprintf(dbg, sizeof(dbg), " [din=%p cap=%zu nin=%zu nout=%zu lowres=%p out=%p attr=%d type=%d dev=%d]", (void*)din, h->up_cap, nin, nout,
             (const void*)lowres, (void*)out, (int)pa, (int)at.type, at.device);
    h->set_error(std::string("vstar_upsample_mask: ") + what + ": " + hipGetErrorString(e) + dbg);
    return VSTAR_ERR_HIP;
  }
  return VSTAR_OK;
}

int64_t vstar_debug_read(vstar_handle* h, const char* name, float* out, int64_t cap) {
  if (!h || !name || !out) { tls_error() = "bad argument"; return VSTAR_ERR_INVALID; }
  if (!h->finalized) { h->set_error("weights not finalized"); return VSTAR_ERR_STATE; }
  hipSetDevice(h->device);
  if (!strcmp(name, "score_graph_stats")) {
    if (cap < 3) { h->set_error("score_graph_stats needs room for 3 values"); return VSTAR_ERR_INVALID; }
    int captured = 0;
    for (auto& kv : h->score_graphs) captured += kv.second != nullptr;
    out[0] = (float)h->score_graph_replays; out[1] = (float)captured; out[2] = (float)h->score_graphs.size();
    return 3;
  }
  const bool pix = !strcmp(name, "clip_pixels") || !strcmp(name, "owl_pixels");
  if (!pix && h->last_B == 0) { h->set_error("no forward has run"); return VSTAR_ERR_STATE; }
  const int B = pix ? (int)h->h_jobs.size() / 2 : h->last_B;
  const std::string n(name);
  const lp_t* src = nullptr;
  int64_t cnt = 0;
  if (n == "clip_pixels") { src = h->d_clip_pix; cnt = (int64_t)B * 3 * h->cfg.clip_image_size * h->cfg.clip_image_size; }
  else if (n == "owl_pixels") { src = h->d_owl_pix; cnt = (int64_t)B * 3 * h->cfg.owl_image_size * h->cfg.owl_image_size; }
  else if (n == "clip_features") { src = h->clip.x; cnt = (int64_t)B * h->clip.N * h->clip.hidden; }
  else if (n == "llm_input") { src = h->lx; cnt = 0; }
  else if (n == "llm_hidden_loc") { src = h->hsel; cnt = (int64_t)B * h->cfg.llm_hidden; }
  else if (n == "embed_det") { src = h->emb_det; cnt = (int64_t)B * h->det1.N; }
  else if (n == "embed_seg") { src = h->emb_seg; cnt = (int64_t)B * 256; }
  else if (n == "owl_feats") { src = h->owl_feats; cnt = (int64_t)B * h->owl.P * h->owl.hidden; }
  else if (n == "sam_tokens") { src = h->s_q; cnt = (int64_t)B * 6 * 256; }
  else if (n == "sam_keys") { src = h->s_keys; cnt = (int64_t)B * h->owl.P * 256; }
  else if (n == "sam_src") { src = h->s_src; cnt = (int64_t)B * h->owl.P * 256; }
  else if (n == "sam_c1") { src = h->s_c1; cnt = (int64_t)B * 96 * 96 * 64; }
  else if (n == "sam_c1n") { src = h->s_c1n; cnt = (int64_t)B * 96 * 96 * 64; }
  else if (n == "sam_c2") { src = h->s_c2; cnt = (int64_t)B * 192 * 192 * 32; }
  else if (n == "sam_hyper") { src = h->s_hyper; cnt = (int64_t)B * 32; }
  else { h->set_error("unknown debug tensor: " + n); return VSTAR_ERR_INVALID; }
  if (cnt > cap) cnt = cap;
  std::vector<lp_t> tmp((size_t)cnt);
  if (hipStreamSynchronize(h->stream) != hipSuccess ||
      hipMemcpy(tmp.data(), src, (size_t)cnt * 2, hipMemcpyDeviceToHost) != hipSuccess) {
    h->set_error("debug_read: HIP failure");
    return VSTAR_ERR_HIP;
  }
  for (int64_t i = 0; i < cnt; ++i) out[i] = lp2f(tmp[(size_t)i]);
  return cnt;
}

void* vstar_stream(vstar_handle* h) { return h ? (void*)h->stream : nullptr; }

int vstar_profile_enable(vstar_handle* h, int on) {
  if (!h) return VSTAR_ERR_INVALID;
  h->profile = on != 0;
  h->prof_ms = 0; h->prof_flops = 0; h->prof_launches = 0; h->pending_flops = 0; h->ev_used = 0;
  h->prof_ms8 = 0; h->prof_flops8 = 0; h->prof_launches8 = 0; h->ev_flops.clear();
  return VSTAR_OK;
}
int vstar_profile_read(vstar_handle* h, double* gemm_ms, int64_t* gemm_launches, double* gemm_flops) {
  if (!h) return VSTAR_ERR_INVALID;
  hipSetDevice(h->device);
  hipStreamSynchronize(h->stream);
  h->collect_profile();
  if (gemm_ms) *gemm_ms = h->prof_ms;
  if (gemm_launches) *gemm_launches = h->prof_launches;
  if (gemm_flops) *gemm_flops = h->prof_flops;
  return VSTAR_OK;
}

int vstar_profile_read_fp8(vstar_handle* h, double* gemm_ms, int64_t* gemm_launches, double* gemm_flops) {
  if (!h) return VSTAR_ERR_INVALID;
  hipSetDevice(h->device);
  hipStreamSynchronize(h->stream);
  h->collect_profile();
  if (gemm_ms) *gemm_ms = h->prof_ms8;
  if (gemm_launches) *gemm_launches = h->prof_launches8;
  if (gemm_flops) *gemm_flops = h->prof_flops8;
  return VSTAR_OK;
}

static int op_rc(hipError_t e) {
  if (e != hipSuccess) { tls_error() = std::string("HIP: ") + hipGetErrorString(e); return VSTAR_ERR_HIP; }
  return VSTAR_OK;
}

int vstar_op_gemm(void* stream, const uint16_t* A, int64_t lda, const uint16_t* W, const uint16_t* bias,
                  const uint16_t* residual, int64_t ldr, void* C, int64_t ldc, int out_f32, int M, int N, int K,
                  int epilogue) {
  GemmParams p{};
  p.A = A; p.lda = lda; p.W = W; p.bias = bias; p.res = residual; p.ldr = ldr; p.C = C; p.ldc = ldc;
  p.M = M; p.N = N; p.K = K;
  { const char* e = getenv("VSTAR_GEMM_DEBUG"); p.debug_flags = e ? atoi(e) : 0; }
  const bool nosync = (epilogue & VSTAR_EPI_NOSYNC) != 0;
  if ((epilogue & VSTAR_EPI_TILE128) && (epilogue & VSTAR_EPI_TILE256)) { tls_error() = "both tile overrides set"; return VSTAR_ERR_INVALID; }
  p.tile_force = (epilogue & VSTAR_EPI_TILE4W) ? GEMM_TILE_4W : (epilogue & VSTAR_EPI_TILE256) ? 256 : (epilogue & VSTAR_EPI_TILE128) ? 128 : 0;
  if (p.tile_force == 256 && !gemm256_eligible(p)) {
    tls_error() = "VSTAR_EPI_TILE256: shape outside the 256x256 kernel's domain (M >= 1024, N >= 256, K % 128 == 0)";
    return VSTAR_ERR_INVALID;
  }
  hipError_t e = gemm_lp(p, epilogue & 0xff, out_f32 != 0, (hipStream_t)stream);
  if (e == hipSuccess && !nosync) e = hipStreamSynchronize((hipStream_t)stream);
  return op_rc(e);
}
int vstar_op_gemm_norm(void* stream, const uint16_t* A, int64_t lda, const uint16_t* W, const uint16_t* bias,
                       const uint16_t* residual, int64_t ldr, void* C, int64_t ldc, int M, int N, int K, int epilogue,
                       const float* row_scale, float* sumsq_out, int sumsq_ld) {
  GemmParams p{};
  p.A = A; p.lda = lda; p.W = W; p.bias = bias; p.res = residual; p.ldr = ldr; p.C = C; p.ldc = ldc;
  p.M = M; p.N = N; p.K = K;
  p.row_scale = row_scale; p.sumsq_out = sumsq_out; p.sumsq_ld = sumsq_ld;
  { const char* e = getenv("VSTAR_GEMM_DEBUG"); p.debug_flags = e ? atoi(e) : 0; }
  if ((epilogue & VSTAR_EPI_TILE128) && (epilogue & VSTAR_EPI_TILE256)) { tls_error() = "both tile overrides set"; return VSTAR_ERR_INVALID; }
  if (sumsq_out && ((epilogue & 0xff) != VSTAR_EPI_NONE || N % 64)) { tls_error() = "sumsq_out: VSTAR_EPI_NONE and N % 64 == 0 only"; return VSTAR_ERR_INVALID; }
  p.tile_force = (epilogue & VSTAR_EPI_TILE4W) ? GEMM_TILE_4W : (epilogue & VSTAR_EPI_TILE256) ? 256 : (epilogue & VSTAR_EPI_TILE128) ? 128 : 0;
  if (p.tile_force == 256 && !gemm256_eligible(p)) { tls_error() = "VSTAR_EPI_TILE256: shape outside the 256x256 kernel's domain"; return VSTAR_ERR_INVALID; }
  hipError_t e = gemm_lp(p, epilogue & 0xff, false, (hipStream_t)stream);
  if (e == hipSuccess) e = hipStreamSynchronize((hipStream_t)stream);
  return op_rc(e);
}
int vstar_op_rms_rstd(void* stream, const uint16_t* x, const float* partials, int ld, int rows, int cols, float eps, float* r) {
  hipError_t e = x ? rms_rstd_rows(x, rows, cols, eps, r, (hipStream_t)stream)
                   : rms_rstd_partials(partials, ld, rows, cols, eps, r, (hipStream_t)stream);
  if (e == hipSuccess) e = hipStreamSynchronize((hipStream_t)stream);
  return op_rc(e);
}
int vstar_op_ln_fold(void* stream, uint16_t* W, uint16_t* bias, const uint16_t* g, const uint16_t* b_ln, int n_rows, int K) {
  hipError_t e = ln_fold_weights(W, bias, g, b_ln, n_rows, K, (hipStream_t)stream);
  if (e == hipSuccess) e = hipStreamSynchronize((hipStream_t)stream);
  return op_rc(e);
}
int vstar_op_gemm_last_tile(void) { return gemm_last_tile(); }
int vstar_op_gemm_plan(int M, int N, int K, int epilogue, int has_residual, int fused_rope, int cus) {
  if (M <= 0 || N <= 0 || K <= 0 || cus <= 0) { tls_error() = "vstar_op_gemm_plan: bad argument"; return VSTAR_ERR_INVALID; }
  static const uintptr_t fake = 0x10000;
  GemmParams p{};
  p.A = (const lp_t*)fake; p.lda = K; p.W = (const lp_t*)fake; p.C = (void*)fake;
  p.M = M; p.N = N; p.K = K;
  const int n_out = (epilogue & 0xff) == VSTAR_EPI_SILU_MUL ? N / 2 : N;
  p.ldc = n_out;
  if (has_residual) { p.res = (const lp_t*)fake; p.ldr = n_out; }
  if (fused_rope) { p.rope_cs = (const lp_t*)fake; p.rope_S = 640; p.rope_cols = N * 2 / 3; }
  p.tile_force = (epilogue & VSTAR_EPI_TILE256) ? 256 : (epilogue & VSTAR_EPI_TILE128) ? 128 : 0;
  gemm_set_plan(true, cus);
  const hipError_t e = gemm_lp(p, epilogue & 0xff, false, nullptr);
  gemm_set_plan(false, 0);
  if (e != hipSuccess) { tls_error() = std::string("vstar_op_gemm_plan: ") + hipGetErrorString(e); return VSTAR_ERR_INVALID; }
  return gemm_last_tile() * 10 + gemm_last_mode();
}
int vstar_op_layernorm(void* stream, const uint16_t* x, const uint16_t* g, const uint16_t* b, uint16_t* y, int rows,
                       int cols, float eps) {
  hipError_t e = layernorm_lp(x, g, b, y, rows, cols, eps, nullptr, 0, (hipStream_t)stream);
  if (e == hipSuccess) e = hipStreamSynchronize((hipStream_t)stream);
  return op_rc(e);
}
int vstar_op_rmsnorm(void* stream, const uint16_t* x, const uint16_t* g, uint16_t* y, int rows, int cols, float eps) {
  hipError_t e = rmsnorm_lp(x, g, y, rows, cols, eps, nullptr, (hipStream_t)stream);
  if (e == hipSuccess) e = hipStreamSynchronize((hipStream_t)stream);
  return op_rc(e);
}
int vstar_op_gemm_fp8(void* stream, const uint16_t* A, const uint16_t* W, const uint16_t* bias, const uint16_t* res, uint16_t* C,
                      int M, int N, int K, int epilogue, int iters, float* gemm_ms) {
  if (!A || !W || !C || M <= 0 || N <= 0 || K <= 0) { tls_error() = "bad argument"; return VSTAR_ERR_INVALID; }
  hipStream_t s = (hipStream_t)stream;
  const int Npad = (N + 255) / 256 * 256;
  const int n_out = (epilogue & 0xff) == VSTAR_EPI_SILU_MUL ? N / 2 : N;
  uint8_t *Aq = nullptr, *Wq = nullptr;
  float *sa = nullptr, *sw = nullptr;
  hipError_t e = hipMalloc((void**)&Aq, (size_t)M * K);
  if (e == hipSuccess) e = hipMalloc((void**)&Wq, (size_t)Npad * K);
  if (e == hipSuccess) e = hipMalloc((void**)&sa, (size_t)M * 4);
  if (e == hipSuccess) e = hipMalloc((void**)&sw, (size_t)Npad * 4);
  if (e == hipSuccess) e = quantize_rows_fp8(A, K, Aq, K, sa, M, K, s);
  if (e == hipSuccess) e = quantize_rows_fp8(W, K, Wq, K, sw, Npad, K, s);
  GemmParams p{};
  p.A = (const lp_t*)Aq; p.lda = K; p.W = (const lp_t*)Wq; p.bias = bias; p.res = res; p.ldr = n_out; p.C = C; p.ldc = n_out;
  p.M = M; p.N = N; p.K = K; p.a_scale = sa; p.w_scale = sw;
  p.tile_force = (epilogue & VSTAR_EPI_TILE4W) ? GEMM_TILE_4W : (epilogue & VSTAR_EPI_TILE256) ? 256 : 0;
  epilogue &= 0xff;
  if (e == hipSuccess && !gemm256_eligible(p)) { tls_error() = "shape not accepted by the W8A8 kernel"; e = hipErrorInvalidValue; }
  if (e == hipSuccess) e = gemm_lp(p, epilogue, false, s);
  if (e == hipSuccess && iters > 0 && gemm_ms) {
    hipEvent_t e0, e1;
    hipEventCreate(&e0); hipEventCreate(&e1);
    hipEventRecord(e0, s);
    for (int i = 0; i < iters && e == hipSuccess; ++i) e = gemm_lp(p, epilogue, false, s);
    hipEventRecord(e1, s);
    hipEventSynchronize(e1);
    float ms = 0;
    hipEventElapsedTime(&ms, e0, e1);
    *gemm_ms = ms / iters;
    hipEventDestroy(e0); hipEventDestroy(e1);
  }
  if (e == hipSuccess) e = hipStreamSynchronize(s);
  hipFree(Aq); hipFree(Wq); hipFree(sa); hipFree(sw);
  return op_rc(e);
}
size_t vstar_op_mx_scale_bytes(int rows, int cols) { return (rows % 128 || cols % 128) ? 0 : mx_scale_bytes(rows, cols); }
int64_t vstar_op_mx_scale_offset(int row, int k_block, int rows) { return mx_scale_offset(row, k_block, rows >> 7); }
int vstar_op_quantize_mx(void* stream, const uint16_t* X, uint8_t* q, uint8_t* scales, int rows, int cols) {
  hipError_t e = quantize_rows_mx(X, cols, q, cols, scales, rows, cols, (hipStream_t)stream);
  if (e == hipSuccess) e = hipStreamSynchronize((hipStream_t)stream);
  return op_rc(e);
}
int vstar_op_gemm_mx(void* stream, const uint8_t* Aq, const uint8_t* a_scales, const float* row_scale, const uint16_t* W, const uint16_t* res,
                     uint16_t* C, uint8_t* C8, uint8_t* c_scales, float* sumsq, int M, int N, int K, int epilogue, int iters, float* gemm_ms) {
  if (!Aq || !a_scales || !W || (!C && !C8) || M <= 0 || N <= 0 || K <= 0) { tls_error() = "bad argument"; return VSTAR_ERR_INVALID; }
  hipStream_t s = (hipStream_t)stream;
  const int Npad = (N + 255) / 256 * 256;
  const int n_out = epilogue == VSTAR_EPI_SILU_MUL ? N / 2 : N;
  uint8_t* Wq = nullptr;
  float* sw = nullptr;
  hipError_t e = hipMalloc((void**)&Wq, (size_t)Npad * K);
  if (e == hipSuccess) e = hipMalloc((void**)&sw, (size_t)Npad * 4);
  if (e == hipSuccess) e = quantize_rows_fp8(W, K, Wq, K, sw, Npad, K, s);
  GemmParams p{};
  p.A = (const lp_t*)Aq; p.lda = K; p.W = (const lp_t*)Wq; p.res = res; p.ldr = n_out; p.M = M; p.N = N; p.K = K;
  p.w_scale = sw; p.a_mx = a_scales; p.a_scale = row_scale;
  if (epilogue == VSTAR_EPI_SILU_MUL && C8) { p.C = C8; p.ldc = n_out; p.c_mx = c_scales; }
  else { p.C = C; p.ldc = n_out; p.c8 = C8; p.ldc8 = n_out; p.c_mx = C8 ? c_scales : nullptr; p.sumsq_out = C8 ? sumsq : nullptr; p.sumsq_ld = n_out / 64; }
  if (e == hipSuccess && !gemm_mx_supported(p, epilogue)) { tls_error() = "shape not accepted by the block-scaled W8A8 kernel"; e = hipErrorInvalidValue; }
  if (e == hipSuccess) e = gemm_lp(p, epilogue, false, s);
  if (e == hipSuccess && iters > 0 && gemm_ms) {
    hipEvent_t e0, e1;
    hipEventCreate(&e0); hipEventCreate(&e1);
    hipEventRecord(e0, s);
    for (int i = 0; i < iters && e == hipSuccess; ++i) e = gemm_lp(p, epilogue, false, s);
    hipEventRecord(e1, s);
    hipEventSynchronize(e1);
    float ms = 0;
    hipEventElapsedTime(&ms, e0, e1);
    *gemm_ms = ms / iters;
    hipEventDestroy(e0); hipEventDestroy(e1);
  }
  if (e == hipSuccess) e = hipStreamSynchronize(s);
  hipFree(Wq); hipFree(sw);
  return op_rc(e);
}
int vstar_op_gemm_fp8_mxout(void* stream, const uint16_t* A, const uint16_t* W, uint8_t* C8, uint8_t* c_scales, int M, int N, int K, int iters,
                            float* gemm_ms) {
  if (!A || !W || !C8 || !c_scales || M <= 0 || N <= 0 || K <= 0) { tls_error() = "bad argument"; return VSTAR_ERR_INVALID; }
  hipStream_t s = (hipStream_t)stream;
  const int Npad = (N + 255) / 256 * 256;
  uint8_t *Aq = nullptr, *Wq = nullptr;
  float *sa = nullptr, *sw = nullptr;
  hipError_t e = hipMalloc((void**)&Aq, (size_t)M * K);
  if (e == hipSuccess) e = hipMalloc((void**)&Wq, (size_t)Npad * K);
  if (e == hipSuccess) e = hipMalloc((void**)&sa, (size_t)M * 4);
  if (e == hipSuccess) e = hipMalloc((void**)&sw, (size_t)Npad * 4);
  if (e == hipSuccess) e = quantize_rows_fp8(A, K, Aq, K, sa, M, K, s);
  if (e == hipSuccess) e = quantize_rows_fp8(W, K, Wq, K, sw, Npad, K, s);
  GemmParams p{};
  p.A = (const lp_t*)Aq; p.lda = K; p.W = (const lp_t*)Wq; p.C = C8; p.ldc = N / 2;
  p.M = M; p.N = N; p.K = K; p.a_scale = sa; p.w_scale = sw; p.c_mx = c_scales;
  if (e == hipSuccess && !gemm_mx_supported(p, VSTAR_EPI_SILU_MUL)) { tls_error() = "shape not accepted by the block-scaled W8A8 kernel"; e = hipErrorInvalidValue; }
  if (e == hipSuccess) e = gemm_lp(p, VSTAR_EPI_SILU_MUL, false, s);
// ... 56 lines not shown
```

vstar_amd/csrc/engine_base.hpp:

```cpp
#pragma once
#include <hip/hip_runtime.h>
#include <cmath>
#include <cstddef>
#include <cstdio>
#include <cstdlib>
#include <cstring>
#include <map>
#include <string>
#include <vector>
#include "common.hpp"
#include "kernels.hpp"

namespace VS_NS {

inline std::string& tls_error() {
  static thread_local std::string s;
  return s;
}

struct HostTensor {
  std::vector<lp_t> data;
  std::vector<int64_t> shape;
  int64_t numel() const { int64_t n = 1; for (auto d : shape) n *= d; return n; }
};

struct Lin { lp_t* W = nullptr; lp_t* b = nullptr; int N = 0, K = 0; };
struct VitBlock { lp_t *ln1_g, *ln1_b, *ln2_g, *ln2_b; Lin qkv, out, fc1, fc2; };
struct VitTower {
  int image = 0, patch = 0, grid = 0, P = 0, N = 0, hidden = 0, heads = 0, mlp = 0, nblocks = 0, kpad = 0;
  Lin patch_lin; lp_t *cls = nullptr, *pos = nullptr, *pre_g = nullptr, *pre_b = nullptr;
  std::vector<VitBlock> blocks;
  lp_t *im2col = nullptr, *patch_out = nullptr, *x = nullptr, *h = nullptr, *qkv = nullptr, *att = nullptr, *mlp_buf = nullptr;
  bool fold = false;
  float *part = nullptr, *rstd = nullptr;
};
struct Lin8 { uint8_t* W = nullptr; float* s = nullptr; };
struct LlmBlock {
  lp_t *in_norm, *post_norm; Lin qkv, o, gate_up, down; Lin8 qkv8, o8, gate_up8, down8;
  Lin8 qkv8f, gate_up8f;
};

#define HIPCHK(expr)                                                                         \
  do {                                                                                       \
    hipError_t _e = (expr);                                                                  \
    if (_e != hipSuccess) {                                                                  \
      set_error(std::string(#expr) + ": " + hipGetErrorString(_e));                          \
      return VSTAR_ERR_HIP;                                                                  \
    }                                                                                        \
  } while (0)
#define KCHK(expr) HIPCHK(expr)
#define RC(expr) do { int _rc = (expr); if (_rc) return _rc; } while (0)

struct EngineBase {
  int device = 0;
  hipStream_t stream = nullptr;
  std::string error;
  bool finalized = false;
  std::map<std::string, HostTensor> staged;
  std::vector<void*> allocs;

  bool profile = false;
  std::vector<hipEvent_t> ev;
  size_t ev_used = 0;
  double prof_ms = 0, prof_flops = 0;
  int64_t prof_launches = 0;
  double pending_flops = 0;
  double prof_ms8 = 0, prof_flops8 = 0;
  int64_t prof_launches8 = 0;
  std::vector<double> ev_flops;

  void set_error(const std::string& m) { error = m; tls_error() = m; }

  int stage_tensor(const char* key, const void* host_ptr, int dtype, int ndim, const int64_t* shape);
  void release_base() {
    for (void* p : allocs) hipFree(p);
    allocs.clear();
    for (auto e : ev) hipEventDestroy(e);
    ev.clear();
  }

  template <typename T> int dalloc(T** p, size_t count) {
    void* q = nullptr;
    size_t bytes = count * sizeof(T);
    if (bytes == 0) bytes = 16;
    hipError_t e = hipMalloc(&q, bytes);
    if (e != hipSuccess) { set_error("hipMalloc(" + std::to_string(bytes) + "): " + hipGetErrorString(e)); return VSTAR_ERR_NOMEM; }
    allocs.push_back(q);
    *p = (T*)q;
    return 0;
  }
  const HostTensor* find(const std::string& k) {
    auto it = staged.find(k);
    return it == staged.end() ? nullptr : &it->second;
  }
  int need(const std::string& k, const HostTensor** out) {
    *out = find(k);
    if (!*out) { set_error("missing checkpoint tensor: " + k); return VSTAR_ERR_MISSING; }
    return 0;
  }
  int upload_vec(const std::string& k, lp_t** dev, int64_t expect = -1) {
    const HostTensor* t;
    int rc = need(k, &t);
    if (rc) return rc;
    if (expect >= 0 && t->numel() != expect) { set_error("bad size for " + k); return VSTAR_ERR_INVALID; }
    rc = dalloc(dev, (size_t)t->numel());
    if (rc) return rc;
    HIPCHK(hipMemcpy(*dev, t->data.data(), t->numel() * 2, hipMemcpyHostToDevice));
    return 0;
  }
  int make_lin(const std::vector<std::string>& wkeys, const std::vector<std::string>& bkeys, Lin* out, int K_expect = -1,
               const std::vector<int>* perm = nullptr, bool conv3x3 = false, bool conv_patch = false) {
    std::vector<const HostTensor*> ws;
    int N = 0, K = -1;
    for (auto& k : wkeys) {
      const HostTensor* t;
      int rc = need(k, &t);
      if (rc) return rc;
      int n = (int)t->shape[0];
      int kk = (int)(t->numel() / n);
      if (K < 0) K = kk;
      if (kk != K) { set_error("K mismatch in " + k); return VSTAR_ERR_INVALID; }
      ws.push_back(t);
      N += n;
    }
    if (K_expect >= 0 && K != K_expect) { set_error("unexpected K for " + wkeys[0]); return VSTAR_ERR_INVALID; }
    const int Kpad = (K + 63) / 64 * 64, Npad = (N + 255) / 256 * 256;
    std::vector<lp_t> host((size_t)Npad * Kpad, 0);
    int r0 = 0;
    for (auto* t : ws) {
      const int n = (int)t->shape[0];
      for (int r = 0; r < n; ++r) {
        lp_t* dst = &host[(size_t)(r0 + r) * Kpad];
        const lp_t* src = &t->data[(size_t)r * K];
        if (conv3x3) {
          const int C = K / 9;
          for (int c = 0; c < C; ++c)
            for (int tap = 0; tap < 9; ++tap) dst[tap * C + c] = src[c * 9 + tap];
        } else {
          (void)conv_patch;
          memcpy(dst, src, (size_t)K * 2);
        }
      }
      r0 += n;
    }
    if (perm) {
      std::vector<lp_t> tmp((size_t)Npad * Kpad, 0);
      for (int r = 0; r < N; ++r) memcpy(&tmp[(size_t)r * Kpad], &host[(size_t)(*perm)[r] * Kpad], (size_t)Kpad * 2);
      host.swap(tmp);
    }
    int rc = dalloc(&out->W, host.size());
    if (rc) return rc;
    HIPCHK(hipMemcpy(out->W, host.data(), host.size() * 2, hipMemcpyHostToDevice));
    out->N = N;
    out->K = Kpad;
    out->b = nullptr;
    if (!bkeys.empty()) {
      std::vector<lp_t> hb((size_t)Npad, 0);
      int o = 0;
      for (auto& k : bkeys) {
        const HostTensor* t;
        rc = need(k, &t);
        if (rc) return rc;
        memcpy(&hb[o], t->data.data(), (size_t)t->numel() * 2);
        o += (int)t->numel();
      }
      if (o != N) { set_error("bias size mismatch for " + wkeys[0]); return VSTAR_ERR_INVALID; }
      if (perm) {
        std::vector<lp_t> tb((size_t)Npad, 0);
        for (int r = 0; r < N; ++r) tb[r] = hb[(*perm)[r]];
        hb.swap(tb);
      }
      rc = dalloc(&out->b, hb.size());
      if (rc) return rc;
      HIPCHK(hipMemcpy(out->b, hb.data(), hb.size() * 2, hipMemcpyHostToDevice));
    }
    return 0;
  }

  int gemm(const GemmParams& p, int epi, bool f32) {
    hipEvent_t e0 = nullptr, e1 = nullptr;
    if (profile) {
      if (ev_used + 2 > ev.size()) {
        for (int i = 0; i < 256; ++i) { hipEvent_t e; hipEventCreate(&e); ev.push_back(e); }
      }
      e0 = ev[ev_used++]; e1 = ev[ev_used++];
      hipEventRecord(e0, stream);
    }
    hipError_t e = gemm_lp(p, epi, f32, stream);
    if (e != hipSuccess) { set_error(std::string("gemm launch: ") + hipGetErrorString(e)); return VSTAR_ERR_HIP; }
    if (profile) {
      hipEventRecord(e1, stream);
      const double fl = 2.0 * p.M * (double)p.N * p.K;
      pending_flops += fl;
      ev_flops.push_back((p.a_scale || p.a_mx) ? -fl : fl);
      prof_launches++;
      if (p.a_scale || p.a_mx) prof_launches8++;
    }
    return 0;
  }
  int lin(const lp_t* A, int64_t lda, const Lin& L, void* C, int64_t ldc, int M, int epi = VSTAR_EPI_NONE,
          const lp_t* res = nullptr, int64_t ldr = 0, bool f32 = false) {
    GemmParams p{};
    p.A = A; p.lda = lda; p.a_group = 0;
    p.W = L.W; p.bias = L.b; p.res = res; p.ldr = ldr;
    p.C = C; p.ldc = ldc; p.c_group = 0;
    p.M = M; p.N = L.N; p.K = L.K;
    p.row_scale = next_row_scale; p.sumsq_out = next_sumsq; p.sumsq_ld = next_sumsq_ld;
    p.stats_sum = next_stats_sum;
    next_row_scale = nullptr; next_sumsq = nullptr; next_sumsq_ld = 0; next_stats_sum = 0;
    if (map_group > 0) {
      p.a_group = p.c_group = map_group;
      p.a_gstride = p.c_gstride = map_gstride;
      p.a_off = p.c_off = map_off;
    }
    return gemm(p, epi, f32);
  }
  int map_group = 0; int64_t map_gstride = 0, map_off = 0;
  const float* next_row_scale = nullptr; float* next_sumsq = nullptr; int next_sumsq_ld = 0;
  int next_stats_sum = 0;
  bool fold_vit_norms = true;
  void collect_profile() {
    if (!profile) return;
    for (size_t i = 0; i + 1 < ev_used; i += 2) {
      float ms = 0;
      if (hipEventElapsedTime(&ms, ev[i], ev[i + 1]) == hipSuccess) {
        prof_ms += ms;
        if (i / 2 < ev_flops.size() && ev_flops[i / 2] < 0) { prof_ms8 += ms; prof_flops8 += -ev_flops[i / 2]; }
      }
    }
    prof_flops += pending_flops;
    pending_flops = 0;
    ev_flops.clear();
    ev_used = 0;
  }

  int build_tower(VitTower& t, const std::string& pre, const std::string& preln_name, int image, int patch, int hidden,
                  int heads, int mlp, int nblocks, int maxB);
  int run_tower(VitTower& t, const lp_t* pix, int B);
};

inline float half_bits_to_float(uint16_t hb) {
  const uint32_t sign = (hb & 0x8000u) << 16;
  uint32_t exp = (hb >> 10) & 0x1f, man = hb & 0x3ff;
  uint32_t bits;
  if (exp == 0) {
    if (man == 0) bits = sign;
    else { int sh = 0; while (!(man & 0x400)) { man <<= 1; sh++; } man &= 0x3ff; bits = sign | ((127 - 15 - sh + 1) << 23) | (man << 13); }
  } else if (exp == 31) bits = sign | 0x7f800000u | (man << 13);
  else bits = sign | ((exp - 15 + 127) << 23) | (man << 13);
  float f; memcpy(&f, &bits, 4);
  return f;
}
inline float bf16_bits_to_float(uint16_t b) { uint32_t u = (uint32_t)b << 16; float f; memcpy(&f, &u, 4); return f; }

inline int EngineBase::stage_tensor(const char* key, const void* host_ptr, int dtype, int ndim, const int64_t* shape) {
  HostTensor t;
  t.shape.assign(shape, shape + ndim);
  const int64_t n = t.numel();
  t.data.resize((size_t)n);
#ifdef VSTAR_LP_F16
  const int native = VSTAR_F16, other = VSTAR_BF16;
#else
  const int native = VSTAR_BF16, other = VSTAR_F16;
#endif
  if (dtype == native) {
    memcpy(t.data.data(), host_ptr, (size_t)n * 2);
  } else if (dtype == VSTAR_F32) {
    const float* s = (const float*)host_ptr;
    for (int64_t i = 0; i < n; ++i) t.data[i] = f2lp(s[i]);
  } else if (dtype == other) {
    const uint16_t* s = (const uint16_t*)host_ptr;
    for (int64_t i = 0; i < n; ++i) t.data[i] = f2lp(other == VSTAR_F16 ? half_bits_to_float(s[i]) : bf16_bits_to_float(s[i]));
  } else { set_error("unknown dtype"); return VSTAR_ERR_INVALID; }
  staged[key] = std::move(t);
  return VSTAR_OK;
}

inline int EngineBase::build_tower(VitTower& t, const std::string& pre, const std::string& preln_name, int image, int patch,
                              int hidden, int heads, int mlp, int nblocks, int maxB) {
  t.image = image; t.patch = patch; t.grid = image / patch; t.P = t.grid * t.grid; t.N = t.P + 1;
  t.hidden = hidden; t.heads = heads; t.mlp = mlp; t.nblocks = nblocks;
  if (hidden != heads * 64) { set_error("ViT head dim must be 64"); return VSTAR_ERR_INVALID; }
  RC(make_lin({pre + "embeddings.patch_embedding.weight"}, {}, &t.patch_lin, 3 * patch * patch));
  t.kpad = t.patch_lin.K;
  RC(upload_vec(pre + "embeddings.class_embedding", &t.cls, hidden));
  RC(upload_vec(pre + "embeddings.position_embedding.weight", &t.pos, (int64_t)t.N * hidden));
  RC(upload_vec(pre + preln_name + ".weight", &t.pre_g, hidden));
  RC(upload_vec(pre + preln_name + ".bias", &t.pre_b, hidden));
  t.blocks.resize(nblocks);
  for (int i = 0; i < nblocks; ++i) {
    const std::string lp = pre + "encoder.layers." + std::to_string(i) + ".";
    VitBlock& b = t.blocks[i];
    RC(upload_vec(lp + "layer_norm1.weight", &b.ln1_g, hidden));
    RC(upload_vec(lp + "layer_norm1.bias", &b.ln1_b, hidden));
    RC(upload_vec(lp + "layer_norm2.weight", &b.ln2_g, hidden));
    RC(upload_vec(lp + "layer_norm2.bias", &b.ln2_b, hidden));
    RC(make_lin({lp + "self_attn.q_proj.weight", lp + "self_attn.k_proj.weight", lp + "self_attn.v_proj.weight"},
                {lp + "self_attn.q_proj.bias", lp + "self_attn.k_proj.bias", lp + "self_attn.v_proj.bias"}, &b.qkv, hidden));
    RC(make_lin({lp + "self_attn.out_proj.weight"}, {lp + "self_attn.out_proj.bias"}, &b.out, hidden));
    RC(make_lin({lp + "mlp.fc1.weight"}, {lp + "mlp.fc1.bias"}, &b.fc1, hidden));
    RC(make_lin({lp + "mlp.fc2.weight"}, {lp + "mlp.fc2.bias"}, &b.fc2, mlp));
  }
  for (const char* e : {"VSTAR_FOLD_NORMS", "VSTAR_FOLD_VIT_NORMS"})
    if (const char* v = getenv(e)) if (atoi(v) == 0) fold_vit_norms = false;
  t.fold = fold_vit_norms && hidden % 64 == 0;
  if (t.fold) {
    for (auto& b : t.blocks) {
      if (b.qkv.K != hidden || b.fc1.K != hidden || !b.qkv.b || !b.fc1.b) { t.fold = false; break; }
    }
  }
  if (t.fold) {
    for (auto& b : t.blocks) {
      KCHK(ln_fold_weights(b.qkv.W, b.qkv.b, b.ln1_g, b.ln1_b, b.qkv.N, b.qkv.K, stream));
      KCHK(ln_fold_weights(b.fc1.W, b.fc1.b, b.ln2_g, b.ln2_b, b.fc1.N, b.fc1.K, stream));
    }
    HIPCHK(hipStreamSynchronize(stream));
  }
  const size_t rows = (size_t)maxB * t.N;
  RC(dalloc(&t.im2col, (size_t)maxB * t.P * t.kpad));
  RC(dalloc(&t.patch_out, (size_t)maxB * t.P * hidden));
  RC(dalloc(&t.x, rows * hidden));
  RC(dalloc(&t.h, rows * hidden));
  RC(dalloc(&t.qkv, rows * 3 * hidden));
  RC(dalloc(&t.att, rows * hidden));
  RC(dalloc(&t.mlp_buf, rows * mlp));
  if (t.fold) {
    RC(dalloc(&t.part, rows * (size_t)(2 * (hidden / 64))));
    RC(dalloc(&t.rstd, rows));
  }
  return 0;
}

inline int EngineBase::run_tower(VitTower& t, const lp_t* pix, int B) {
  const int C = t.hidden, rows = B * t.N;
  KCHK(im2col_patch(pix, t.im2col, B, t.image, t.patch, t.kpad, stream));
  RC(lin(t.im2col, t.kpad, t.patch_lin, t.patch_out, C, B * t.P));
  KCHK(vit_assemble_tokens(t.patch_out, t.cls, t.pos, t.h, B, t.P, C, stream));
  KCHK(layernorm_lp(t.h, t.pre_g, t.pre_b, t.x, rows, C, 1e-5f, nullptr, 0, stream));
  if (t.fold) {
    const int nsp = C / 64;
    for (int i = 0; i < t.nblocks; ++i) {
      VitBlock& b = t.blocks[i];
      if (i == 0) KCHK(ln_rstd_rows(t.x, rows, C, 1e-5f, t.rstd, stream));
      else KCHK(ln_rstd_partials(t.part, 2 * nsp, rows, C, 1e-5f, t.rstd, stream));
      next_row_scale = t.rstd;
      RC(lin(t.x, C, b.qkv, t.qkv, 3 * C, rows));
      KCHK(attn_forward(t.qkv, t.att, B, t.N, t.heads, 64, 0, 0.125f, stream));
      next_sumsq = t.part; next_sumsq_ld = 2 * nsp; next_stats_sum = nsp;
      RC(lin(t.att, C, b.out, t.x, C, rows, VSTAR_EPI_NONE, t.x, C));
      KCHK(ln_rstd_partials(t.part, 2 * nsp, rows, C, 1e-5f, t.rstd, stream));
      next_row_scale = t.rstd;
      RC(lin(t.x, C, b.fc1, t.mlp_buf, t.mlp, rows, VSTAR_EPI_QUICK_GELU));
      if (i + 1 < t.nblocks) { next_sumsq = t.part; next_sumsq_ld = 2 * nsp; next_stats_sum = nsp; }
      RC(lin(t.mlp_buf, t.mlp, b.fc2, t.x, C, rows, VSTAR_EPI_NONE, t.x, C));
    }
    return 0;
  }
  for (int i = 0; i < t.nblocks; ++i) {
    VitBlock& b = t.blocks[i];
    KCHK(layernorm_lp(t.x, b.ln1_g, b.ln1_b, t.h, rows, C, 1e-5f, nullptr, 0, stream));
    RC(lin(t.h, C, b.qkv, t.qkv, 3 * C, rows));
    KCHK(attn_forward(t.qkv, t.att, B, t.N, t.heads, 64, 0, 0.125f, stream));
    RC(lin(t.att, C, b.out, t.x, C, rows, VSTAR_EPI_NONE, t.x, C));
    KCHK(layernorm_lp(t.x, b.ln2_g, b.ln2_b, t.h, rows, C, 1e-5f, nullptr, 0, stream));
    RC(lin(t.h, C, b.fc1, t.mlp_buf, t.mlp, rows, VSTAR_EPI_QUICK_GELU));
    RC(lin(t.mlp_buf, t.mlp, b.fc2, t.x, C, rows, VSTAR_EPI_NONE, t.x, C));
  }
  return 0;
}

}
using namespace VS_NS;
```

vstar_amd/csrc/gemm.hip:

```cpp
#include "common.hpp"
#include "kernels.hpp"
#include "gemm_epilogue.hpp"
#include <cstdlib>

namespace VS_NS {

static thread_local bool t_plan_only = false;
static thread_local int t_plan_cus = 0;
static thread_local int t_last_mode = 0;
void gemm_set_plan(bool on, int cus) { t_plan_only = on; t_plan_cus = on ? cus : 0; }
bool gemm_plan_only() { return t_plan_only; }
int gemm_last_mode() { return t_last_mode; }

namespace {

constexpr int BM = 128, BN = 128, BK = 64;
constexpr int LDS_TILE = BM * BK * 2;
constexpr int LDS_BUF = 2 * LDS_TILE;

typedef const __attribute__((address_space(1))) void* gptr_t;
typedef __attribute__((address_space(3))) void* lptr_t;

__device__ __forceinline__ int64_t map_row(int r, int group, int64_t gstride, int64_t off) {
  return gemm_map_row(r, group, gstride, off);
}

#define BAR128()                                       \
  do {                                                 \
    __builtin_amdgcn_sched_barrier(0);                 \
    asm volatile("s_barrier" ::: "memory");            \
    __builtin_amdgcn_sched_barrier(0);                 \
  } while (0)

template <int EPI, bool OUT_F32, int MODE, int NW = 2>
__global__ __launch_bounds__(MODE == 5 ? (NW == 4 ? 576 : 320) : 256, (NW != 4 && (MODE == 2 || NW == 1)) ? 2 : 1) void gemm128_kernel(const GemmParams p) {
  constexpr bool LDR = MODE == 5;
  constexpr int STAGES = LDR ? 3 : MODE;
  static_assert(NW == 2 || LDR, "the 128 x 64 and 128 x 256 tiles exist in loader-wave mode only");
  constexpr int BN = 64 * NW;
  constexpr int MF = NW == 1 ? 2 : 4;
  constexpr int NCW = NW == 4 ? 8 : 4;
  constexpr int W_TILE = BN * BK * 2;
  constexpr int LDS_BUF = LDS_TILE + W_TILE;
  extern __shared__ __attribute__((aligned(16))) char smem[];
  const int tid = threadIdx.x;
  const int lane = tid & 63;
  const int wave = __builtin_amdgcn_readfirstlane(tid >> 6);

  const int tiles_m = (p.M + BM - 1) / BM;
  const int tiles_n = (p.N + BN - 1) / BN;
  const int nwg = tiles_m * tiles_n;
  int t;
  {
    const int bid = blockIdx.x;
    const int xcd = bid & 7, q = nwg >> 3, r = nwg & 7;
    t = (xcd < r ? xcd * (q + 1) : r * (q + 1) + (xcd - r) * q) + (bid >> 3);
  }
  constexpr int GROUP_M = 8;
  const int in_group = GROUP_M * tiles_n;
  const int grp = t / in_group;
  const int first_m = grp * GROUP_M;
  const int gsz = min(tiles_m - first_m, GROUP_M);
  const int rem = t - grp * in_group;
  const int tm = first_m + rem % gsz;
  const int tn = rem / gsz;
  const int m0 = tm * BM, n0 = tn * BN;

  const int st_r = lane >> 3;
  const int st_c = lane & 7;
  const lp_t* a_src[4];
  const lp_t* w_src[4];
#pragma unroll
  for (int i = 0; i < 4; ++i) {
    const int r = (i * 4 + wave) * 8 + st_r;
    const int cg = st_c ^ ((r >> 1) & 7);
    int ar = m0 + r;
    ar = ar < p.M ? ar : p.M - 1;
    a_src[i] = p.A + map_row(ar, p.a_group, p.a_gstride, p.a_off) * p.lda + cg * 8;
    w_src[i] = p.W + (int64_t)(n0 + r) * p.K + cg * 8;
  }

  auto stage = [&](int buf, int k0) {
    char* base = smem + buf * LDS_BUF;
#pragma unroll
    for (int i = 0; i < 4; ++i) {
      const int piece = (i * 4 + wave) * 1024;
      __builtin_amdgcn_global_load_lds((gptr_t)(a_src[i] + k0), (lptr_t)(base + piece), 16, 0, 0);
      __builtin_amdgcn_global_load_lds((gptr_t)(w_src[i] + k0), (lptr_t)(base + LDS_TILE + piece), 16, 0, 0);
    }
  };

  if constexpr (LDR) {
    if (wave == NCW) {
      constexpr int WP = BN / 8;
      constexpr int NP = WP > 16 ? WP : 16;
      const lp_t* a_all[16];
      const lp_t* w_all[WP];
#pragma unroll
      for (int j = 0; j < NP; ++j) {
        const int r = j * 8 + st_r;
        const int cg = st_c ^ ((r >> 1) & 7);
        if (j < 16) {
          int ar = m0 + r;
          ar = ar < p.M ? ar : p.M - 1;
          a_all[j] = p.A + map_row(ar, p.a_group, p.a_gstride, p.a_off) * p.lda + cg * 8;
        }
        if (j < WP) w_all[j] = p.W + (int64_t)(n0 + r) * p.K + cg * 8;
      }
      auto issue = [&](int buf, int k0) {
        char* base = smem + buf * LDS_BUF;
#pragma unroll
        for (int j = 0; j < NP; ++j) {
          if (j < 16) __builtin_amdgcn_global_load_lds((gptr_t)(a_all[j] + k0), (lptr_t)(base + j * 1024), 16, 0, 0);
          if (j < WP) __builtin_amdgcn_global_load_lds((gptr_t)(w_all[j] + k0), (lptr_t)(base + LDS_TILE + j * 1024), 16, 0, 0);
        }
      };
      const int nk = p.K / BK;
      issue(0, 0);
      if (nk > 1) issue(1, BK);
      int slot = 2;
      for (int kt = 0; kt < nk; ++kt) {
        __builtin_amdgcn_sched_barrier(0);
        if (kt + 1 >= nk) asm volatile("s_waitcnt vmcnt(0)" ::: "memory");
        else if constexpr (NW == 4) asm volatile("s_waitcnt vmcnt(48)" ::: "memory");
        else if constexpr (NW == 2) asm volatile("s_waitcnt vmcnt(32)" ::: "memory");
        else asm volatile("s_waitcnt vmcnt(24)" ::: "memory");
        BAR128();
        if (kt + 2 < nk) issue(slot, (kt + 2) * BK);
        slot = slot == 2 ? 0 : slot + 1;
      }
      return;
    }
  }

  const int wr = NW == 4 ? wave >> 2 : (NW == 2 ? wave >> 1 : wave), wc = NW == 4 ? wave & 3 : (NW == 2 ? wave & 1 : 0);
  const int fr = lane & 15, fq = lane >> 4;
  const int swz = (fr >> 1) & 7;
  int a_rd[2], w_rd[2];
#pragma unroll
  for (int kk = 0; kk < 2; ++kk) {
    const int ch = ((kk * 4 + fq) ^ swz) * 16;
    a_rd[kk] = (wr * (MF * 16) + fr) * 128 + ch;
    w_rd[kk] = LDS_TILE + (wc * 64 + fr) * 128 + ch;
  }

  f32x4 acc[MF][4];
#pragma unroll
  for (int m = 0; m < MF; ++m)
#pragma unroll
    for (int n = 0; n < 4; ++n) acc[m][n] = (f32x4){0.f, 0.f, 0.f, 0.f};

  const int nkt = p.K / BK;
  if constexpr (!LDR) stage(0, 0);
  if constexpr (LDR) {
  } else if constexpr (STAGES == 2) {
    __syncthreads();
  } else {
#pragma unroll
    for (int t = 1; t < STAGES - 1; ++t)
      if (t < nkt) stage(t, t * BK);
  }

  int cur = 0;
  for (int kt = 0; kt < nkt; ++kt) {
    if constexpr (LDR) {
      BAR128();
    } else if constexpr (STAGES == 2) {
      cur = kt & 1;
      if (kt + 1 < nkt) stage(cur ^ 1, (kt + 1) * BK);
    } else {
      __builtin_amdgcn_sched_barrier(0);
      if (kt + 1 < nkt) asm volatile("s_waitcnt vmcnt(8)" ::: "memory");
      else asm volatile("s_waitcnt vmcnt(0)" ::: "memory");
      BAR128();
      if (kt + STAGES - 1 < nkt) stage(cur >= 1 ? cur - 1 : STAGES - 1, (kt + STAGES - 1) * BK);
      __builtin_amdgcn_sched_barrier(0);
    }
    const char* base = smem + cur * LDS_BUF;
#pragma unroll
    for (int kk = 0; kk < 2; ++kk) {
      lpx8 af[MF], wf[4];
#pragma unroll
      for (int m = 0; m < MF; ++m) af[m] = *(const lpx8*)(base + a_rd[kk] + m * 2048);
#pragma unroll
      for (int n = 0; n < 4; ++n) wf[n] = *(const lpx8*)(base + w_rd[kk] + n * 2048);
#pragma unroll
      for (int m = 0; m < MF; ++m)
#pragma unroll
        for (int n = 0; n < 4; ++n)
          acc[m][n] = mfma_16x16x32(wf[n], af[m], acc[m][n]);
    }
    if constexpr (!LDR && STAGES == 2) {
      __syncthreads();
    } else {
      cur = cur == STAGES - 1 ? 0 : cur + 1;
    }
  }

  const int n_out = (EPI == VSTAR_EPI_SILU_MUL) ? p.N / 2 : p.N;
  if (p.row_scale) {
#pragma unroll
    for (int m = 0; m < MF; ++m) {
      const int row = m0 + wr * (MF * 16) + m * 16 + fr;
      const float rs = p.row_scale[map_row(row < p.M ? row : p.M - 1, p.a_group, p.a_gstride, p.a_off)];
#pragma unroll
      for (int n = 0; n < 4; ++n)
#pragma unroll
        for (int e = 0; e < 4; ++e) acc[m][n][e] *= rs;
    }
  }
  if constexpr (EPI == VSTAR_EPI_NONE && !OUT_F32) {
    if (p.sumsq_out) {
#pragma unroll
      for (int m = 0; m < MF; ++m) {
        const int row = m0 + wr * (MF * 16) + m * 16 + fr;
        const int64_t crow = map_row(row < p.M ? row : p.M - 1, p.c_group, p.c_gstride, p.c_off);
        float o[4][4];
#pragma unroll
        for (int n = 0; n < 4; ++n) {
          if (row < p.M) gemm_epilogue_store<EPI, OUT_F32>(p, crow, n0 + wc * 64 + n * 16 + fq * 4, n_out, acc[m][n], acc[m][n], o[n]);
          else o[n][0] = o[n][1] = o[n][2] = o[n][3] = 0.f;
        }
        const float ss = gemm_sumsq_span64_frags(o);
        if (fq == 0 && row < p.M && n0 + wc * 64 < n_out) p.sumsq_out[crow * p.sumsq_ld + (n0 + wc * 64) / 64] = ss;
        if (p.stats_sum) {
          const float sm = gemm_sum_span64_frags(o);
          if (fq == 0 && row < p.M && n0 + wc * 64 < n_out) p.sumsq_out[crow * p.sumsq_ld + p.stats_sum + (n0 + wc * 64) / 64] = sm;
        }
      }
      return;
    }
  }
#pragma unroll
  for (int m = 0; m < MF; ++m) {
    const int row = m0 + wr * (MF * 16) + m * 16 + fr;
    if (row >= p.M) continue;
    const int64_t crow = map_row(row, p.c_group, p.c_gstride, p.c_off);
    if (EPI == VSTAR_EPI_SILU_MUL) {
#pragma unroll
      for (int j = 0; j < 2; ++j)
        gemm_epilogue_store<EPI, OUT_F32>(p, crow, (n0 + wc * 64) / 2 + j * 16 + fq * 4, n_out, acc[m][2 * j], acc[m][2 * j + 1]);
    } else {
#pragma unroll
      for (int n = 0; n < 4; ++n)
        gemm_epilogue_store<EPI, OUT_F32>(p, crow, n0 + wc * 64 + n * 16 + fq * 4, n_out, acc[m][n], acc[m][n]);
    }
  }
}

}
int gemm_device_cus();
namespace {

template <int EPI, bool OUT_F32, int MODE, int NW = 2>
hipError_t launch_stages(const GemmParams& p, hipStream_t s) {
  t_last_mode = MODE == 5 ? (NW == 4 ? 7 : (NW == 1 ? 6 : 5)) : MODE;
  if (t_plan_only) return hipSuccess;
  static bool attr_done = false;
  auto kern = gemm128_kernel<EPI, OUT_F32, MODE, NW>;
  constexpr int bn = 64 * NW;
  constexpr int lds = (MODE == 5 ? 3 : MODE) * (LDS_TILE + bn * BK * 2);
  if (!attr_done) {
    hipError_t e = hipFuncSetAttribute((const void*)kern, hipFuncAttributeMaxDynamicSharedMemorySize, lds);
    if (e != hipSuccess) return e;
    attr_done = true;
  }
  const int tiles = ((p.M + BM - 1) / BM) * ((p.N + bn - 1) / bn);
  hipLaunchKernelGGL(kern, dim3(tiles), dim3(MODE == 5 ? (NW == 4 ? 576 : 320) : 256), lds, s, p);
  return hipGetLastError();
}

template <int EPI, bool OUT_F32>
hipError_t launch(const GemmParams& p, hipStream_t s) {
  static const int force = [] { const char* e = getenv("VSTAR_GEMM128_STAGES"); return e ? atoi(e) : 0; }();
  const int64_t tiles = (int64_t)((p.M + BM - 1) / BM) * ((p.N + BN - 1) / BN);
  const int64_t cus = gemm_device_cus();
  const int64_t tiles7 = (int64_t)((p.M + BM - 1) / BM) * ((p.N + 255) / 256);
  const bool wide = p.K >= 2048 && tiles > cus &&
                    1.05 * (double)((tiles7 + cus - 1) / cus) <= 1.28 * (double)((tiles + 2 * cus - 1) / (2 * cus));
  const int mode = force == 2 || force == 5 || force == 6 || force == 7 ? force
                   : (p.K < 4 * BK ? 2 : (wide ? 7 : (tiles > cus ? 2 : (2 * tiles <= cus ? 6 : 5))));
  if (mode == 7) return launch_stages<EPI, OUT_F32, 5, 4>(p, s);
  if (mode == 6) return launch_stages<EPI, OUT_F32, 5, 1>(p, s);
  if (mode == 5) return launch_stages<EPI, OUT_F32, 5, 2>(p, s);
  return launch_stages<EPI, OUT_F32, 2, 2>(p, s);
}

}

bool gemm256_eligible(const GemmParams& p);
hipError_t gemm256_lp(const GemmParams& p, int epilogue, bool out_f32, hipStream_t s);
bool gemm4w_eligible(const GemmParams& p, int epilogue, bool out_f32);
hipError_t gemm4w_lp(const GemmParams& p, int epilogue, hipStream_t s);

static thread_local int t_last_tile = 0;
int gemm_last_tile() { return t_last_tile; }

int gemm_device_cus() {
  if (t_plan_only && t_plan_cus > 0) return t_plan_cus;
  static int n_cu = 0;
  if (n_cu == 0) {
    int dev = 0;
    hipDeviceProp_t prop;
    if (hipGetDevice(&dev) != hipSuccess || hipGetDeviceProperties(&prop, dev) != hipSuccess) return 8;
    n_cu = prop.multiProcessorCount / 8 * 8;
    if (n_cu <= 0) n_cu = 8;
  }
  return n_cu;
}

hipError_t gemm_lp(const GemmParams& p, int epilogue, bool out_f32, hipStream_t s) {
  t_last_tile = 0;
  t_last_mode = 0;
  if (p.M <= 0 || p.N <= 0) return hipSuccess;
  if (p.K % BK != 0 || p.K <= 0 || p.norm_w) return hipErrorInvalidValue;
  if (((uintptr_t)p.A & 15) || ((uintptr_t)p.W & 15) || (p.lda % 8)) return hipErrorInvalidValue;
  static const int env_force = [] { const char* e = getenv("VSTAR_GEMM_TILE"); return e ? atoi(e) : 0; }();
  const int force = p.tile_force ? p.tile_force : env_force;
  if (force != 0 && force != 128 && force != 256 && force != GEMM_TILE_4W) return hipErrorInvalidValue;
  if (p.a_mx || p.c_mx) {
    if (out_f32 || (force != 0 && force != GEMM_TILE_4W) || !gemm4w_eligible(p, epilogue, out_f32)) return hipErrorInvalidValue;
    t_last_tile = GEMM_TILE_4W;
    return gemm4w_lp(p, epilogue, s);
  }
  const bool elig = gemm256_eligible(p);
  if (p.tile_force == 256 && !elig) return hipErrorInvalidValue;
  static const int env4w = [] { const char* e = getenv("VSTAR_GEMM4W"); return e ? atoi(e) : GEMM4W_DEFAULT; }();
  if (force == GEMM_TILE_4W) {
    if (!(elig && gemm4w_eligible(p, epilogue, out_f32))) return hipErrorInvalidValue;
    t_last_tile = GEMM_TILE_4W;
    return gemm4w_lp(p, epilogue, s);
  }
  auto big = [&](const GemmParams& q) -> hipError_t {
    if (force == 0 && env4w != 0 && gemm4w_eligible(q, epilogue, out_f32)) {
      t_last_tile = GEMM_TILE_4W;
      return gemm4w_lp(q, epilogue, s);
    }
    t_last_tile = 256;
    return gemm256_lp(q, epilogue, out_f32, s);
  };
  if (force != 128 && elig) {
    const int64_t cus = gemm_device_cus();
    const int64_t t256 = (int64_t)((p.M + 255) / 256) * ((p.N + 255) / 256), t128 = (int64_t)((p.M + 127) / 128) * ((p.N + 127) / 128);
    const bool prefer128 = force != 256 && !p.rope_cs && !p.a_scale && t256 < cus &&
                           0.36 * (double)((t128 + cus - 1) / cus) < (double)((t256 + cus - 1) / cus);
    if (!prefer128) {
      const int64_t rt = (p.M + 255) / 256, ct = (p.N + 255) / 256;
      const int64_t full = t256 / cus, rem = t256 - full * cus;
      static const bool env_split = [] { const char* e = getenv("VSTAR_GEMM_SPLIT"); return !e || atoi(e) != 0; }();
      const bool split_ok = env_split && force == 0 && p.a_group <= 0 && p.c_group <= 0 && !p.rope_cs && !p.a_scale && !p.debug_flags;
      if (split_ok && full >= 1 && rem > 0) {
        const int64_t rt1 = full * cus / ct;
        const int64_t M1 = rt1 * 256, M2 = p.M - M1;
        const int64_t t128b = ((M2 + 127) / 128) * ((p.N + 127) / 128);
        if (rt1 >= 4 && rt1 < rt && M2 > 0 && t128b <= cus) {
          GemmParams a = p, b = p;
          a.M = (int)M1;
          b.M = (int)M2;
          b.A = p.A + M1 * p.lda;
          b.C = out_f32 ? (void*)((float*)p.C + M1 * p.ldc) : (void*)((lp_t*)p.C + M1 * p.ldc);
          if (p.res) b.res = p.res + M1 * p.ldr;
          if (p.row_scale) b.row_scale = p.row_scale + M1;
          if (p.sumsq_out) b.sumsq_out = p.sumsq_out + M1 * p.sumsq_ld;
          b.tile_force = 128;
          hipError_t e = big(a);
          if (e != hipSuccess) return e;
          e = gemm_lp(b, epilogue, out_f32, s);
          t_last_tile = 256 + 128;
          return e;
        }
      }
      return big(p);
    }
  }
  if (p.rope_cs || p.a_scale) return hipErrorInvalidValue;
  t_last_tile = 128;
#define GEMM_CASE(E)                                                   \
  case E:                                                              \
    return out_f32 ? launch<E, true>(p, s) : launch<E, false>(p, s);
  switch (epilogue) {
    GEMM_CASE(VSTAR_EPI_NONE)
    GEMM_CASE(VSTAR_EPI_QUICK_GELU)
    GEMM_CASE(VSTAR_EPI_GELU)
    GEMM_CASE(VSTAR_EPI_RELU)
    GEMM_CASE(VSTAR_EPI_SILU_MUL)
  }
#undef GEMM_CASE
  t_last_tile = 0;
  return hipErrorInvalidValue;
}

}
```

vstar_amd/csrc/heads.hip:

```cpp
#include "common.hpp"
#include "kernels.hpp"

namespace VS_NS {

namespace {

__global__ __launch_bounds__(256) void owl_class_kernel(const float* __restrict__ emb, int ld, int Q,
                                                        const lp_t* __restrict__ query, float* __restrict__ out,
                                                        int out_stride_crop, int B, int rows_per_crop, int img_div) {
  const int lane = threadIdx.x & 63;
  const int64_t row = (int64_t)blockIdx.x * 4 + (threadIdx.x >> 6);
  if (row >= (int64_t)B * rows_per_crop) return;
  const int b = (int)(row / rows_per_crop), p = (int)(row % rows_per_crop);
  const float* er = emb + ((int64_t)(b / img_div) * rows_per_crop + p) * ld;
  const lp_t* qr = query + (int64_t)b * Q;
  float ee = 0.f, qq = 0.f;
  for (int d = lane; d < Q; d += 64) {
    const float e = rlp(er[d]), q = lp2f(qr[d]);
    ee += e * e;
    qq += q * q;
  }
  ee = wave_sum(ee);
  qq = wave_sum(qq);
  const float en = rlp(rlp(sqrtf(ee)) + 1e-6f), qn = rlp(rlp(sqrtf(qq)) + 1e-6f);
  float dot = 0.f;
  for (int d = lane; d < Q; d += 64) dot += rlp(rlp(er[d]) / en) * rlp(lp2f(qr[d]) / qn);
  dot = rlp(wave_sum(dot));
  if (lane == 0) {
    const float shift = rlp(er[Q]);
    const float sc = rlp(er[Q + 1]);
    const float elu = sc > 0.f ? sc : (__expf(sc) - 1.0f);
    const float scale = rlp(rlp(elu) + 1.0f);
    out[(int64_t)b * out_stride_crop + p] = rlp(rlp(dot + shift) * scale);
  }
}

__global__ void owl_box_kernel(const float* __restrict__ raw, int ld, float* __restrict__ out, int out_stride_crop, int B,
                               int grid, int img_div) {
  const int npatch = grid * grid;
  const int64_t idx = (int64_t)blockIdx.x * blockDim.x + threadIdx.x;
  if (idx >= (int64_t)B * npatch * 4) return;
  const int c = (int)(idx & 3);
  const int64_t row = idx >> 2;
  const int p = (int)(row % npatch), b = (int)(row / npatch);
  float coord;
  if (c == 0) coord = (float)(p % grid + 1) / (float)grid;
  else if (c == 1) coord = (float)(p / grid + 1) / (float)grid;
  else coord = 1.0f / (float)grid;
  coord = fminf(fmaxf(coord, 0.f), 1.f);
  const float bias = logf(coord + 1e-4f) - log1pf(-coord + 1e-4f);
  const float v = rlp(rlp(raw[((int64_t)(b / img_div) * npatch + p) * ld + c]) + bias);
  out[(int64_t)b * out_stride_crop + p * 4 + c] = rlp(1.0f / (1.0f + __expf(-v)));
}

__global__ void up2x_im2col_kernel(const lp_t* __restrict__ src, lp_t* __restrict__ A, int B, int h, int w, int C) {
  const int cv = C >> 3;
  const int H2 = 2 * h, W2 = 2 * w;
  const int64_t idx = (int64_t)blockIdx.x * blockDim.x + threadIdx.x;
  const int64_t total = (int64_t)B * H2 * W2 * 9 * cv;
  if (idx >= total) return;
  const int v = (int)(idx % cv);
  int64_t r = idx / cv;
  const int tap = (int)(r % 9);
  r /= 9;
  const int X = (int)(r % W2);
  const int Y = (int)((r / W2) % H2);
  const int b = (int)(r / ((int64_t)W2 * H2));
  const int yy = Y + tap / 3 - 1, xx = X + tap % 3 - 1;
  lpx8 o = {0, 0, 0, 0, 0, 0, 0, 0};
  if (yy >= 0 && yy < H2 && xx >= 0 && xx < W2) {
    const float sy = fmaxf(0.5f * (yy + 0.5f) - 0.5f, 0.f), sx = fmaxf(0.5f * (xx + 0.5f) - 0.5f, 0.f);
    const int y0 = (int)sy, x0 = (int)sx;
    const int y1 = y0 + (y0 < h - 1 ? 1 : 0), x1 = x0 + (x0 < w - 1 ? 1 : 0);
    const float ly = sy - y0, lx = sx - x0;
    const lp_t* base = src + (int64_t)b * h * w * C + v * 8;
    const lpx8 v00 = *(const lpx8*)(base + ((int64_t)y0 * w + x0) * C);
    const lpx8 v01 = *(const lpx8*)(base + ((int64_t)y0 * w + x1) * C);
    const lpx8 v10 = *(const lpx8*)(base + ((int64_t)y1 * w + x0) * C);
    const lpx8 v11 = *(const lpx8*)(base + ((int64_t)y1 * w + x1) * C);
#pragma unroll
    for (int e = 0; e < 8; ++e) {
      const float t = (1.f - ly) * ((1.f - lx) * lp2f((lp_t)v00[e]) + lx * lp2f((lp_t)v01[e])) +
                      ly * ((1.f - lx) * lp2f((lp_t)v10[e]) + lx * lp2f((lp_t)v11[e]));
      o[e] = (short)f2lp(t);
    }
  }
  *(lpx8*)(A + idx * 8) = o;
}

template <int C>
__global__ void hyper_mask_kernel(const lp_t* __restrict__ hyper, const lp_t* __restrict__ up, float* __restrict__ out,
                                  int out_stride_crop, int B, int npix) {
  const int64_t idx = (int64_t)blockIdx.x * blockDim.x + threadIdx.x;
  if (idx >= (int64_t)B * npix) return;
  const int b = (int)(idx / npix), pix = (int)(idx % npix);
  const lp_t* u = up + idx * C;
  const lp_t* hy = hyper + (int64_t)b * C;
  float a = 0.f;
#pragma unroll
  for (int v = 0; v < C / 8; ++v) {
    const lpx8 x = *(const lpx8*)(u + v * 8);
    const lpx8 w = *(const lpx8*)(hy + v * 8);
#pragma unroll
    for (int e = 0; e < 8; ++e) a += lp2f((lp_t)x[e]) * lp2f((lp_t)w[e]);
  }
  out[(int64_t)b * out_stride_crop + pix] = rlp(a);
}

__global__ void resize_bilinear_kernel(const float* __restrict__ in, int hin, int win, float* __restrict__ out, int hout,
                                       int wout, float rh, float rw, int clamp_min0) {
  const int64_t idx = (int64_t)blockIdx.x * blockDim.x + threadIdx.x;
  if (idx >= (int64_t)hout * wout) return;
  const int x = (int)(idx % wout), y = (int)(idx / wout);
  const float sy = fmaxf(rh * (y + 0.5f) - 0.5f, 0.f), sx = fmaxf(rw * (x + 0.5f) - 0.5f, 0.f);
  const int y0 = (int)sy, x0 = (int)sx;
  const int y1 = y0 + (y0 < hin - 1 ? 1 : 0), x1 = x0 + (x0 < win - 1 ? 1 : 0);
  const float ly = sy - y0, lx = sx - x0;
  const float t = (1.f - ly) * ((1.f - lx) * in[y0 * win + x0] + lx * in[y0 * win + x1]) +
                  ly * ((1.f - lx) * in[y1 * win + x0] + lx * in[y1 * win + x1]);
  out[idx] = clamp_min0 ? fmaxf(t, 0.f) : t;
}

constexpr int MAX_RECTS = 8;
__global__ __launch_bounds__(256) void heat_stats_kernel(const float* __restrict__ in_all, int hin, int win, const int* __restrict__ hw,
                                                         const int* __restrict__ rects_all, const int* __restrict__ n_rects_all,
                                                         double* __restrict__ out_all, unsigned* __restrict__ mm_all) {
  const int item = blockIdx.y;
  const float* in = in_all + (size_t)item * hin * win;
  const int hout = hw[2 * item], wout = hw[2 * item + 1], n_rects = n_rects_all[item];
  const int* rects = rects_all + item * MAX_RECTS * 4;
  double* out = out_all + item * (3 + MAX_RECTS);
  unsigned* mm = mm_all + item * 2;
  const float rh = (float)hin / (float)hout, rw = (float)win / (float)wout;
  const int64_t total = (int64_t)hout * wout;
  float mn = INFINITY, mx = 0.f;
  double sum = 0.0, rs[MAX_RECTS];
#pragma unroll
  for (int k = 0; k < MAX_RECTS; ++k) rs[k] = 0.0;
  int rx[MAX_RECTS], ry[MAX_RECTS], rx1[MAX_RECTS], ry1[MAX_RECTS];
#pragma unroll
  for (int k = 0; k < MAX_RECTS; ++k) {
    const bool on = k < n_rects;
    rx[k] = on ? rects[k * 4] : 0; ry[k] = on ? rects[k * 4 + 1] : 0;
    rx1[k] = on ? rx[k] + rects[k * 4 + 2] : 0; ry1[k] = on ? ry[k] + rects[k * 4 + 3] : 0;
  }
  for (int64_t idx = (int64_t)blockIdx.x * blockDim.x + threadIdx.x; idx < total; idx += (int64_t)gridDim.x * blockDim.x) {
    const int x = (int)(idx % wout), y = (int)(idx / wout);
    const float sy = fmaxf(rh * (y + 0.5f) - 0.5f, 0.f), sx = fmaxf(rw * (x + 0.5f) - 0.5f, 0.f);
    const int y0 = (int)sy, x0 = (int)sx;
    const int y1 = y0 + (y0 < hin - 1 ? 1 : 0), x1 = x0 + (x0 < win - 1 ? 1 : 0);
    const float ly = sy - y0, lx = sx - x0;
    const float t = (1.f - ly) * ((1.f - lx) * in[y0 * win + x0] + lx * in[y0 * win + x1]) +
                    ly * ((1.f - lx) * in[y1 * win + x0] + lx * in[y1 * win + x1]);
    const float hv = fmaxf(t, 0.f);
    mn = fminf(mn, hv);
    mx = fmaxf(mx, hv);
    sum += hv;
#pragma unroll
    for (int k = 0; k < MAX_RECTS; ++k)
      if (x >= rx[k] && x < rx1[k] && y >= ry[k] && y < ry1[k]) rs[k] += hv;
  }
  for (int o = 32; o > 0; o >>= 1) {
    mn = fminf(mn, __shfl_xor(mn, o, 64));
    mx = fmaxf(mx, __shfl_xor(mx, o, 64));
    sum += __shfl_xor(sum, o, 64);
#pragma unroll
    for (int k = 0; k < MAX_RECTS; ++k) rs[k] += __shfl_xor(rs[k], o, 64);
  }
  __shared__ double s_sum[4][1 + MAX_RECTS];
  __shared__ float s_mn[4], s_mx[4];
  const int wave = threadIdx.x >> 6;
  if ((threadIdx.x & 63) == 0) {
    s_mn[wave] = mn; s_mx[wave] = mx; s_sum[wave][0] = sum;
#pragma unroll
    for (int k = 0; k < MAX_RECTS; ++k) s_sum[wave][1 + k] = rs[k];
  }
  __syncthreads();
  if (threadIdx.x == 0) {
    atomicMin(&mm[0], __float_as_uint(fminf(fminf(s_mn[0], s_mn[1]), fminf(s_mn[2], s_mn[3]))));
    atomicMax(&mm[1], __float_as_uint(fmaxf(fmaxf(s_mx[0], s_mx[1]), fmaxf(s_mx[2], s_mx[3]))));
  }
  if (threadIdx.x <= n_rects)
    atomicAdd(&out[2 + threadIdx.x], (s_sum[0][threadIdx.x] + s_sum[1][threadIdx.x]) + (s_sum[2][threadIdx.x] + s_sum[3][threadIdx.x]));
}
__global__ void heat_stats_init(double* out, unsigned* mm, int n) {
  const int i = blockIdx.x * blockDim.x + threadIdx.x;
  if (i < n * (3 + MAX_RECTS)) out[i] = 0.0;
  if (i < n) { mm[2 * i] = 0x7f800000u; mm[2 * i + 1] = 0u; }
}
__global__ void heat_stats_finish(double* out, const unsigned* mm, int n) {
  const int i = blockIdx.x * blockDim.x + threadIdx.x;
  if (i >= n) return;
  out[i * (3 + MAX_RECTS)] = (double)__uint_as_float(mm[2 * i]);
  out[i * (3 + MAX_RECTS) + 1] = (double)__uint_as_float(mm[2 * i + 1]);
}

inline unsigned nblk(int64_t n) { return (unsigned)((n + 255) / 256); }

}

hipError_t heat_stats_batch(const float* lowres, int hin, int win, const int* hw, const int* rects, const int* n_rects, int n,
                            int64_t max_pixels, double* out, unsigned* mm_scratch, hipStream_t s) {
  if (n <= 0) return hipSuccess;
  const int cells = n * (3 + MAX_RECTS);
  hipLaunchKernelGGL(heat_stats_init, dim3((cells + 255) / 256), dim3(256), 0, s, out, mm_scratch, n);
  int64_t bx = (max_pixels + 256 * 8 - 1) / (256 * 8);
  if (bx < 1) bx = 1;
  if (bx > 256) bx = 256;
  hipLaunchKernelGGL(heat_stats_kernel, dim3((unsigned)bx, (unsigned)n), dim3(256), 0, s, lowres, hin, win, hw, rects, n_rects, out,
                     mm_scratch);
  hipLaunchKernelGGL(heat_stats_finish, dim3((n + 255) / 256), dim3(256), 0, s, out, mm_scratch, n);
  return hipGetLastError();
}

hipError_t owl_class_logits(const float* emb, int ld, int Q, const lp_t* query, float* out, int out_stride_crop, int B,
                            int rows_per_crop, hipStream_t s, int img_div) {
  const int64_t rows = (int64_t)B * rows_per_crop;
  hipLaunchKernelGGL(owl_class_kernel, dim3((unsigned)((rows + 3) / 4)), dim3(256), 0, s, emb, ld, Q, query, out,
                     out_stride_crop, B, rows_per_crop, img_div < 1 ? 1 : img_div);
  return hipGetLastError();
}
hipError_t owl_box_finish(const float* raw, int ld, float* out, int out_stride_crop, int B, int grid, hipStream_t s, int img_div) {
  hipLaunchKernelGGL(owl_box_kernel, dim3(nblk((int64_t)B * grid * grid * 4)), dim3(256), 0, s, raw, ld, out,
                     out_stride_crop, B, grid, img_div < 1 ? 1 : img_div);
  return hipGetLastError();
}
hipError_t upsample2x_im2col3x3(const lp_t* src, lp_t* A, int B, int h, int w, int C, hipStream_t s) {
  if (C % 8) return hipErrorInvalidValue;
  hipLaunchKernelGGL(up2x_im2col_kernel, dim3(nblk((int64_t)B * 4 * h * w * 9 * (C / 8))), dim3(256), 0, s, src, A, B, h,
                     w, C);
  return hipGetLastError();
}
hipError_t hyper_mask(const lp_t* hyper, const lp_t* up, float* out, int out_stride_crop, int B, int npix, int C,
                      hipStream_t s) {
  if (C != 32) return hipErrorInvalidValue;
  hipLaunchKernelGGL(hyper_mask_kernel<32>, dim3(nblk((int64_t)B * npix)), dim3(256), 0, s, hyper, up, out,
                     out_stride_crop, B, npix);
  return hipGetLastError();
}
hipError_t resize_bilinear_clamp(const float* in, int hin, int win, float* out, int hout, int wout, hipStream_t s, int clamp_min0) {
  hipLaunchKernelGGL(resize_bilinear_kernel, dim3(nblk((int64_t)hout * wout)), dim3(256), 0, s, in, hin, win, out, hout,
                     wout, (float)hin / (float)hout, (float)win / (float)wout, clamp_min0);
  return hipGetLastError();
}

}
```

vstar_amd/csrc/kernels.hpp:

```cpp
#pragma once
#include <hip/hip_runtime.h>
#include <stdint.h>
#include <vector>
#include "../../include/vstar_hip.h"
#include "common.hpp"

namespace VS_NS {

struct GemmParams {
  const lp_t* A; int64_t lda; int a_group; int64_t a_gstride; int64_t a_off;
  const lp_t* W;
  const lp_t* bias;
  const lp_t* res; int64_t ldr;
  void* C; int64_t ldc; int c_group; int64_t c_gstride; int64_t c_off;
  int M, N, K;
  int debug_flags;
  const lp_t* norm_w; float norm_eps;
  const lp_t* rope_cs; int rope_S; int rope_cols;
  int rope_R0, rope_Lc;
  int rope_pos0, rope_tail;
  const float* a_scale; const float* w_scale;
  const float* row_scale; float* sumsq_out; int sumsq_ld;
  int stats_sum;
  int tile_force;
  const lp_t* W_tiled;
  const uint8_t* a_mx; uint8_t* c_mx;
  uint8_t* c8; int64_t ldc8;
};
bool gemm_mx_supported(const GemmParams& p, int epilogue);
hipError_t gemm_lp(const GemmParams& p, int epilogue, bool out_f32, hipStream_t s);
constexpr int GEMM_TILE_4W = 2564;
#ifndef GEMM4W_DEFAULT
#define GEMM4W_DEFAULT 1
#endif
int gemm_last_tile();
int gemm_device_cus();
void gemm_set_plan(bool on, int cus);
bool gemm_plan_only();
int gemm_last_mode();
bool gemm256_eligible(const GemmParams& p);

bool gemm_skinny_eligible(const GemmParams& p);
hipError_t gemm_skinny_lp(const GemmParams& p, int epilogue, bool out_f32, hipStream_t s);
hipError_t skinny_pack_tiles(const lp_t* W, lp_t* Wt, int n_rows, int K, int nt, hipStream_t s);

hipError_t embed_rows(const int32_t* src, const lp_t* table, int vocab, const lp_t* feats, int64_t n_feat_rows, lp_t* x, int R,
                      int C, hipStream_t s);
hipError_t rope_kv_append(lp_t* qkv, const lp_t* cos_sin, const int32_t* row_pos, const int32_t* row_slot, lp_t* kc, lp_t* vc,
                          int64_t slot_stride, int ctx, int R, int H, hipStream_t s);
hipError_t cached_attention(const lp_t* qkv, lp_t* kc, lp_t* vc, const int32_t* row_seq, const int32_t* row_pos,
                            const int32_t* seq_kv, const int32_t* seq_prefix, const int32_t* seq_past, const lp_t* fused_cos_sin,
                            lp_t* out, int R, int H, int ctx, int64_t slot_stride, int max_keys, hipStream_t s,
                            void* split_ws = nullptr, int split_max_rows = 0, const int32_t* anc = nullptr);
hipError_t kv_anc_mark(const int32_t* row_slot, const int32_t* row_pos, int R, int32_t* anc, int ctx, hipStream_t s);
hipError_t kv_anc_fill(int32_t* anc, int slot, int value, int lo, int hi, int ctx, hipStream_t s);
hipError_t kv_anc_reorder(int32_t* anc, int32_t* tmp, const int32_t* d_dst, const int32_t* d_src, int n, int lo, int hi, int ctx,
                          hipStream_t s);
hipError_t kv_copy_rows(lp_t* kc, lp_t* vc, const int32_t* anc, int dst, int src, int lo, int hi, int layers, int H, int ctx,
                        int64_t slot_stride, int64_t layer_stride, hipStream_t s);
size_t cached_attention_split_ws_bytes(int max_rows, int H, int ctx);
hipError_t perceiver_attention(const lp_t* q, const lp_t* kv, lp_t* out, int n, int L, int NK, int H, int DH, hipStream_t s);
hipError_t argmax_rows_lp(const lp_t* x, int rows, int cols, int64_t ld, int32_t* out, hipStream_t s);

hipError_t quantize_rows_fp8(const lp_t* x, int64_t ldx, uint8_t* q, int64_t ldq, float* scale, int rows, int cols,
                             hipStream_t s);
hipError_t rmsnorm_quant_fp8(const lp_t* x, const lp_t* gamma, uint8_t* q, float* scale, int rows, int cols, float eps,
                             hipStream_t s);

hipError_t quantize_rows_mx(const lp_t* x, int64_t ldx, uint8_t* q, int64_t ldq, uint8_t* scales, int rows, int cols, hipStream_t s);

hipError_t layernorm_lp(const lp_t* x, const lp_t* gamma, const lp_t* beta, lp_t* y, int rows, int cols,
                          float eps, const int32_t* row_index, int act, hipStream_t s);
hipError_t rms_rstd_rows(const lp_t* x, int rows, int cols, float eps, float* r, hipStream_t s);
hipError_t rms_rstd_partials(const float* partials, int ld, int rows, int cols, float eps, float* r, hipStream_t s);
hipError_t ln_rstd_rows(const lp_t* x, int rows, int cols, float eps, float* r, hipStream_t s);
hipError_t ln_rstd_partials(const float* partials, int ld, int rows, int cols, float eps, float* r, hipStream_t s);
hipError_t ln_fold_weights(lp_t* W, lp_t* bias, const lp_t* g, const lp_t* b_ln, int n_rows, int K, hipStream_t s);
hipError_t scale_cols_lp(lp_t* W, const lp_t* w, int64_t rows, int K, hipStream_t s);
hipError_t fill_lp(lp_t* v, int64_t n, float value, hipStream_t s);
hipError_t rmsnorm_lp(const lp_t* x, const lp_t* gamma, lp_t* y, int rows, int cols, float eps,
                        const int32_t* row_index, hipStream_t s);

hipError_t attn_prepare(lp_t* qkv, const lp_t* cos_sin , int B, int S, int H, int D,
                        hipStream_t s, int grp_R0 = 0, int grp_Lc = 0);
hipError_t attn_forward(const lp_t* qkv, lp_t* out, int B, int S, int H, int D, int causal, float scale, hipStream_t s,
                        int grp_R0 = 0, int grp_Lc = 0);
hipError_t attn_forward_mx(const lp_t* qkv, uint8_t* out8, uint8_t* scales, int B, int S, int H, float scale, hipStream_t s,
                           int grp_R0 = 0, int grp_Lc = 0);
hipError_t small_attention(const lp_t* q, const lp_t* k, const lp_t* v, lp_t* out, int B, int Nq, int Nk, int H,
                           int D, hipStream_t s);

hipError_t im2col_patch(const lp_t* pix, lp_t* A, int B, int I, int ps, int Kpad, hipStream_t s);
hipError_t vit_assemble_tokens(const lp_t* patch, const lp_t* cls, const lp_t* pos, lp_t* tokens, int B, int P,
                               int C, hipStream_t s);
hipError_t llm_embed_text(const int32_t* ids, int L, int img_col, int P, const lp_t* table, int vocab, lp_t* x, int B,
                          int C, hipStream_t s);
hipError_t add_bcast(const lp_t* a, const lp_t* b, lp_t* out, int64_t rows, int cols, int64_t b_rows, hipStream_t s);
hipError_t add_bcast_repeat(const lp_t* a, const lp_t* b, lp_t* out, int n_out, int rep, int rows_per, int cols, hipStream_t s);
hipError_t bcast_rows(const lp_t* src, lp_t* dst, int nrep, int64_t rep_stride, int nrows, int cols, int64_t ld, hipStream_t s);
hipError_t owl_cls_mul(const lp_t* x, lp_t* y, int B, int N, int C, hipStream_t s);
hipError_t gather_rows(const lp_t* x, const int32_t* idx, lp_t* y, int rows, int cols, hipStream_t s);
hipError_t argmax_rows(const float* x, int rows, int cols, int ld, int32_t* out, int out_stride, hipStream_t s);

hipError_t owl_class_logits(const float* emb, int ld, int Q, const lp_t* query, float* out, int out_stride_crop,
                            int B, int rows_per_crop, hipStream_t s, int img_div = 1);
hipError_t owl_box_finish(const float* raw, int ld, float* out, int out_stride_crop, int B, int grid, hipStream_t s, int img_div = 1);
hipError_t upsample2x_im2col3x3(const lp_t* src, lp_t* A, int B, int h, int w, int C, hipStream_t s);
hipError_t hyper_mask(const lp_t* hyper, const lp_t* up, float* out, int out_stride_crop, int B, int npix, int C,
                      hipStream_t s);
hipError_t resize_bilinear_clamp(const float* in, int hin, int win, float* out, int hout, int wout, hipStream_t s, int clamp_min0 = 1);

hipError_t heat_stats_batch(const float* lowres, int hin, int win, const int* hw, const int* rects, const int* n_rects, int n,
                            int64_t max_pixels, double* out, unsigned* mm_scratch, hipStream_t s);

struct PreJob {
  int x0, y0, cw, ch;
  int in_w, in_h;
  int out;
  int hb_off, hc_off, hks;
  int vb_off, vc_off, vks;
  int img_w;
  int64_t temp_off;
  int64_t out_off;
  const uint8_t* img;
};
void pil_bicubic_coeffs(int in_size, int out_size, std::vector<int32_t>* bounds, std::vector<int32_t>* coeffs, int* ksize);
void clip_norm_lut(lp_t* lut);
hipError_t preprocess_launch(const PreJob* jobs, const int32_t* tables, uint8_t* temp,
                             const lp_t* lut, lp_t* out, int which, int B, int out_size, int max_in_h, hipStream_t s);

}
using namespace VS_NS;
```

Before: 142.3 crops/s.

## Replace im2col buffers with implicit-gather GEMM for SAM convs and patch embed

```diff
diff --git a/include/vstar_hip.h b/include/vstar_hip.h
--- a/include/vstar_hip.h
+++ b/include/vstar_hip.h
@@ -127,6 +127,10 @@
 int vstar_op_gemm(void* stream, const uint16_t* dev_A, int64_t lda, const uint16_t* dev_W, const uint16_t* dev_bias,
                   const uint16_t* dev_residual, int64_t ldr, void* dev_C, int64_t ldc, int out_f32,
                   int M, int N, int K, int epilogue);
+int vstar_op_conv_up2x3x3(void* stream, const uint16_t* dev_src, int B, int h, int w, int C, const uint16_t* dev_W,
+                          const uint16_t* dev_bias, uint16_t* dev_out, int N, int epilogue, int materialise);
+int vstar_op_patch_embed(void* stream, const uint16_t* dev_pix, int B, int img_h, int img_w, int patch, const uint16_t* dev_W,
+                         uint16_t* dev_out, int N, int materialise);
 int vstar_op_gemm_norm(void* stream, const uint16_t* dev_A, int64_t lda, const uint16_t* dev_W, const uint16_t* dev_bias,
                        const uint16_t* dev_residual, int64_t ldr, void* dev_C, int64_t ldc, int M, int N, int K, int epilogue,
                        const float* dev_row_scale, float* dev_sumsq_out, int sumsq_ld);
diff --git a/vstar_amd/_lib.py b/vstar_amd/_lib.py
--- a/vstar_amd/_lib.py
+++ b/vstar_amd/_lib.py
@@ -17,6 +17,7 @@
     "vstar_image_set_slot", "vstar_image_set_slot_async", "vstar_preprocess_crops_slots", "vstar_comm_unique_id", "vstar_comm_init", "vstar_allgather_results",
     "vstar_comm_destroy", "vstar_build_source_hash", "vstar_op_mx_scale_bytes", "vstar_op_mx_scale_offset", "vstar_op_quantize_mx",
     "vstar_op_gemm_mx", "vstar_op_gemm_fp8_mxout", "vstar_op_attention_mx", "vstar_w8a8_mx_active",
+    "vstar_op_conv_up2x3x3", "vstar_op_patch_embed",
 ]
 
 EXPORTS_VQA = [
@@ -136,6 +137,10 @@
     lib.vstar_op_gemm_norm.argtypes = [c_void_p, c_void_p, c_int64, c_void_p, c_void_p, c_void_p, c_int64, c_void_p, c_int64, c_int, c_int, c_int,
                                        c_int, c_void_p, c_void_p, c_int]
     lib.vstar_op_gemm_norm.restype = c_int
+    lib.vstar_op_conv_up2x3x3.argtypes = [c_void_p, c_void_p, c_int, c_int, c_int, c_int, c_void_p, c_void_p, c_void_p, c_int, c_int, c_int]
+    lib.vstar_op_conv_up2x3x3.restype = c_int
+    lib.vstar_op_patch_embed.argtypes = [c_void_p, c_void_p, c_int, c_int, c_int, c_int, c_void_p, c_void_p, c_int, c_int]
+    lib.vstar_op_patch_embed.restype = c_int
     lib.vstar_op_rms_rstd.argtypes = [c_void_p, c_void_p, c_void_p, c_int, c_int, c_int, c_float, c_void_p]
     lib.vstar_op_rms_rstd.restype = c_int
     lib.vstar_op_ln_fold.argtypes = [c_void_p, c_void_p, c_void_p, c_void_p, c_void_p, c_int, c_int]
diff --git a/vstar_amd/csrc/elementwise.hip b/vstar_amd/csrc/elementwise.hip
--- a/vstar_amd/csrc/elementwise.hip
+++ b/vstar_amd/csrc/elementwise.hip
@@ -5,8 +5,8 @@
 
 namespace {
 
-__global__ void im2col_patch_kernel(const lp_t* __restrict__ pix, lp_t* __restrict__ A, int B, int I, int ps, int Kpad) {
-  const int G = I / ps, P = G * G;
+__global__ void im2col_patch_kernel(const lp_t* __restrict__ pix, lp_t* __restrict__ A, int B, int IH, int IW, int ps, int Kpad) {
+  const int G = IW / ps, P = G * (IH / ps);
   const int K = 3 * ps * ps;
   const int64_t idx = (int64_t)blockIdx.x * blockDim.x + threadIdx.x;
   const int64_t total = (int64_t)B * P * Kpad;
@@ -19,7 +19,7 @@
     const int c = k / (ps * ps), rem = k - c * ps * ps;
     const int ky = rem / ps, kx = rem - ky * ps;
     const int y = (p / G) * ps + ky, x = (p % G) * ps + kx;
-    v = pix[(((int64_t)b * 3 + c) * I + y) * I + x];
+    v = pix[(((int64_t)b * 3 + c) * IH + y) * IW + x];
   }
   A[idx] = v;
 }
@@ -159,11 +159,14 @@
 
 }
 
+hipError_t im2col_patch_hw(const lp_t* pix, lp_t* A, int B, int IH, int IW, int ps, int Kpad, hipStream_t s) {
+  if (ps <= 0 || IH % ps || IW % ps || Kpad < 3 * ps * ps) return hipErrorInvalidValue;
+  const int64_t total = (int64_t)B * (IH / ps) * (IW / ps) * Kpad;
+  hipLaunchKernelGGL(im2col_patch_kernel, dim3(nblk(total)), dim3(256), 0, s, pix, A, B, IH, IW, ps, Kpad);
+  return hipGetLastError();
+}
 hipError_t im2col_patch(const lp_t* pix, lp_t* A, int B, int I, int ps, int Kpad, hipStream_t s) {
-  const int G = I / ps;
-  const int64_t total = (int64_t)B * G * G * Kpad;
-  hipLaunchKernelGGL(im2col_patch_kernel, dim3(nblk(total)), dim3(256), 0, s, pix, A, B, I, ps, Kpad);
-  return hipGetLastError();
+  return im2col_patch_hw(pix, A, B, I, I, ps, Kpad, s);
 }
 hipError_t vit_assemble_tokens(const lp_t* patch, const lp_t* cls, const lp_t* pos, lp_t* tokens, int B, int P,
                                int C, hipStream_t s) {
diff --git a/vstar_amd/csrc/engine.hip b/vstar_amd/csrc/engine.hip
--- a/vstar_amd/csrc/engine.hip
+++ b/vstar_amd/csrc/engine.hip
@@ -53,7 +53,7 @@
   lp_t *s_src = nullptr, *s_keys = nullptr, *s_kpe = nullptr, *s_ia = nullptr, *s_ib = nullptr, *s_ic = nullptr;
   lp_t *s_tok0 = nullptr, *s_q = nullptr, *s_qpe = nullptr, *s_ta = nullptr, *s_tb = nullptr, *s_tc = nullptr, *s_td = nullptr,
          *s_mlp = nullptr;
-  lp_t *s_col1 = nullptr, *s_c1 = nullptr, *s_c1n = nullptr, *s_col2 = nullptr, *s_c2 = nullptr, *s_hyp_in = nullptr,
+  lp_t *s_up = nullptr, *s_c1 = nullptr, *s_c1n = nullptr, *s_c2 = nullptr, *s_hyp_in = nullptr,
          *s_hyp_a = nullptr, *s_hyp_b = nullptr, *s_hyper = nullptr;
   int32_t* d_tokidx = nullptr;
   vstar_result* d_results = nullptr;
@@ -341,10 +341,9 @@
   RC(dalloc(&s_tok0, trow * 256)); RC(dalloc(&s_q, trow * 256)); RC(dalloc(&s_qpe, trow * 256));
   RC(dalloc(&s_ta, trow * 256)); RC(dalloc(&s_tb, trow * 256)); RC(dalloc(&s_tc, trow * 256)); RC(dalloc(&s_td, trow * 256));
   RC(dalloc(&s_mlp, trow * 2048));
-  RC(dalloc(&s_col1, (size_t)maxB * 96 * 96 * 2304));
+  RC(dalloc(&s_up, (size_t)maxB * 96 * 96 * 256));
   RC(dalloc(&s_c1, (size_t)maxB * 96 * 96 * 64));
   RC(dalloc(&s_c1n, (size_t)maxB * 96 * 96 * 64));
-  RC(dalloc(&s_col2, (size_t)maxB * 192 * 192 * 576));
   RC(dalloc(&s_c2, (size_t)maxB * 192 * 192 * 32));
   RC(dalloc(&s_hyp_in, (size_t)maxB * 256)); RC(dalloc(&s_hyp_a, (size_t)maxB * 256)); RC(dalloc(&s_hyp_b, (size_t)maxB * 256));
   RC(dalloc(&s_hyper, (size_t)maxB * 32));
@@ -770,11 +769,11 @@
   RC(lin(s_hyp_in, 256, hyp0, s_hyp_a, 256, B, VSTAR_EPI_RELU));
   RC(lin(s_hyp_a, 256, hyp1, s_hyp_b, 256, B, VSTAR_EPI_RELU));
   RC(lin(s_hyp_b, 256, hyp2, s_hyper, 32, B));
-  KCHK(upsample2x_im2col3x3(s_keys, s_col1, B, 48, 48, 256, stream));
-  RC(lin(s_col1, 2304, conv1, s_c1, 64, B * 96 * 96));
+  KCHK(upsample2x_bilinear(s_keys, s_up, B, 48, 48, 256, stream));
+  RC(lin_gather(GEMM_GATHER_CONV3X3, s_up, 96, 96, 256, conv1, s_c1, 64, B * 96 * 96));
   KCHK(layernorm_lp(s_c1, ln2d_g, ln2d_b, s_c1n, B * 96 * 96, 64, 1e-6f, nullptr, 1, stream));
-  KCHK(upsample2x_im2col3x3(s_c1n, s_col2, B, 96, 96, 64, stream));
-  RC(lin(s_col2, 576, conv2, s_c2, 32, B * 192 * 192, VSTAR_EPI_GELU));
+  KCHK(upsample2x_bilinear(s_c1n, s_up, B, 96, 96, 64, stream));
+  RC(lin_gather(GEMM_GATHER_CONV3X3, s_up, 192, 192, 64, conv2, s_c2, 32, B * 192 * 192, VSTAR_EPI_GELU));
   KCHK(hyper_mask(s_hyper, s_c2, res_f + offsetof(vstar_result, lowres_mask) / 4, rstride, B, 192 * 192, 32, stream));
   return 0;
 }
@@ -1331,6 +1330,8 @@
   else if (n == "embed_det") { src = h->emb_det; cnt = (int64_t)B * h->det1.N; }
   else if (n == "embed_seg") { src = h->emb_seg; cnt = (int64_t)B * 256; }
   else if (n == "owl_feats") { src = h->owl_feats; cnt = (int64_t)B * h->owl.P * h->owl.hidden; }
+  else if (n == "clip_patch_embed") { src = h->clip.patch_out; cnt = (int64_t)B * h->clip.P * h->clip.hidden; }
+  else if (n == "owl_patch_embed") { src = h->owl.patch_out; cnt = (int64_t)B * h->owl.P * h->owl.hidden; }
   else if (n == "sam_tokens") { src = h->s_q; cnt = (int64_t)B * 6 * 256; }
   else if (n == "sam_keys") { src = h->s_keys; cnt = (int64_t)B * h->owl.P * 256; }
   else if (n == "sam_src") { src = h->s_src; cnt = (int64_t)B * h->owl.P * 256; }
@@ -1403,6 +1404,53 @@
   hipError_t e = gemm_lp(p, epilogue & 0xff, out_f32 != 0, (hipStream_t)stream);
   if (e == hipSuccess && !nosync) e = hipStreamSynchronize((hipStream_t)stream);
   return op_rc(e);
+}
+int vstar_op_conv_up2x3x3(void* stream, const uint16_t* src, int B, int h, int w, int C, const uint16_t* W, const uint16_t* bias,
+                          uint16_t* out, int N, int epilogue, int materialise) {
+  if (!src || !W || !out || B <= 0 || h <= 0 || w <= 0 || C <= 0 || C % 64 || N <= 0) { tls_error() = "vstar_op_conv_up2x3x3: bad argument"; return VSTAR_ERR_INVALID; }
+  hipStream_t s = (hipStream_t)stream;
+  const int64_t M = (int64_t)B * 4 * h * w;
+  lp_t* ws = nullptr;
+  if (hipMalloc((void**)&ws, (size_t)M * (materialise ? 9 * C : C) * 2) != hipSuccess) { tls_error() = "vstar_op_conv_up2x3x3: out of memory"; return VSTAR_ERR_NOMEM; }
+  GemmParams p{};
+  p.A = ws; p.lda = 9 * C; p.W = W; p.bias = bias; p.C = out; p.ldc = N; p.M = (int)M; p.N = N; p.K = 9 * C;
+  hipError_t e;
+  if (materialise) {
+    e = upsample2x_im2col3x3(src, ws, B, h, w, C, s);
+  } else {
+    e = upsample2x_bilinear(src, ws, B, h, w, C, s);
+    p.a_gather = GEMM_GATHER_CONV3X3; p.g_h = 2 * h; p.g_w = 2 * w; p.g_c = C; p.g_k = 9 * C;
+  }
+  if (e == hipSuccess) e = gemm_lp(p, epilogue & 0xff, false, s);
+  const hipError_t e2 = hipStreamSynchronize(s);
+  hipFree(ws);
+  return op_rc(e != hipSuccess ? e : e2);
+}
+int vstar_op_patch_embed(void* stream, const uint16_t* pix, int B, int img_h, int img_w, int patch, const uint16_t* W, uint16_t* out,
+                         int N, int materialise) {
+  if (!pix || !W || !out || B <= 0 || patch <= 0 || img_h <= 0 || img_w <= 0 || img_h % patch || img_w % patch || N <= 0) {
+    tls_error() = "vstar_op_patch_embed: bad argument";
+    return VSTAR_ERR_INVALID;
+  }
+  hipStream_t s = (hipStream_t)stream;
+  const int K = 3 * patch * patch, Kpad = (K + 63) / 64 * 64;
+  const int64_t M = (int64_t)B * (img_h / patch) * (img_w / patch);
+  GemmParams p{};
+  p.lda = Kpad; p.W = W; p.C = out; p.ldc = N; p.M = (int)M; p.N = N; p.K = Kpad;
+  lp_t* ws = nullptr;
+  hipError_t e;
+  if (materialise) {
+    if (hipMalloc((void**)&ws, (size_t)M * Kpad * 2) != hipSuccess) { tls_error() = "vstar_op_patch_embed: out of memory"; return VSTAR_ERR_NOMEM; }
+    p.A = ws;
+    e = im2col_patch_hw(pix, ws, B, img_h, img_w, patch, Kpad, s);
+  } else {
+    p.A = pix; p.a_gather = GEMM_GATHER_PATCH; p.g_h = img_h; p.g_w = img_w; p.g_c = patch; p.g_k = K;
+    e = hipSuccess;
+  }
+  if (e == hipSuccess) e = gemm_lp(p, VSTAR_EPI_NONE, false, s);
+  const hipError_t e2 = hipStreamSynchronize(s);
+  if (ws) hipFree(ws);
+  return op_rc(e != hipSuccess ? e : e2);
 }
 int vstar_op_gemm_norm(void* stream, const uint16_t* A, int64_t lda, const uint16_t* W, const uint16_t* bias,
                        const uint16_t* residual, int64_t ldr, void* C, int64_t ldc, int M, int N, int K, int epilogue,
diff --git a/vstar_amd/csrc/engine_base.hpp b/vstar_amd/csrc/engine_base.hpp
--- a/vstar_amd/csrc/engine_base.hpp
+++ b/vstar_amd/csrc/engine_base.hpp
@@ -33,6 +33,7 @@
   lp_t *im2col = nullptr, *patch_out = nullptr, *x = nullptr, *h = nullptr, *qkv = nullptr, *att = nullptr, *mlp_buf = nullptr;
   bool fold = false;
   float *part = nullptr, *rstd = nullptr;
+  bool gather_patch = false;
 };
 struct Lin8 { uint8_t* W = nullptr; float* s = nullptr; };
 struct LlmBlock {
@@ -214,6 +215,13 @@
       p.a_off = p.c_off = map_off;
     }
     return gemm(p, epi, f32);
+  }
+  int lin_gather(int mode, const lp_t* img, int h, int w, int c, const Lin& L, void* C, int64_t ldc, int M, int epi = VSTAR_EPI_NONE) {
+    GemmParams p{};
+    p.A = img; p.lda = L.K; p.a_gather = mode; p.g_h = h; p.g_w = w; p.g_c = c; p.g_k = mode == GEMM_GATHER_PATCH ? 3 * c * c : L.K;
+    p.W = L.W; p.bias = L.b; p.C = C; p.ldc = ldc;
+    p.M = M; p.N = L.N; p.K = L.K;
+    return gemm(p, epi, false);
   }
   int map_group = 0; int64_t map_gstride = 0, map_off = 0;
   const float* next_row_scale = nullptr; float* next_sumsq = nullptr; int next_sumsq_ld = 0;
@@ -317,7 +325,9 @@
     HIPCHK(hipStreamSynchronize(stream));
   }
   const size_t rows = (size_t)maxB * t.N;
-  RC(dalloc(&t.im2col, (size_t)maxB * t.P * t.kpad));
+  t.gather_patch = patch % 8 == 0 && image % 8 == 0 && t.kpad == 3 * patch * patch;
+  if (const char* v = getenv("VSTAR_PATCH_GATHER")) if (atoi(v) == 0) t.gather_patch = false;
+  if (!t.gather_patch) RC(dalloc(&t.im2col, (size_t)maxB * t.P * t.kpad));
   RC(dalloc(&t.patch_out, (size_t)maxB * t.P * hidden));
   RC(dalloc(&t.x, rows * hidden));
   RC(dalloc(&t.h, rows * hidden));
@@ -333,8 +343,12 @@
 
 inline int EngineBase::run_tower(VitTower& t, const lp_t* pix, int B) {
   const int C = t.hidden, rows = B * t.N;
-  KCHK(im2col_patch(pix, t.im2col, B, t.image, t.patch, t.kpad, stream));
-  RC(lin(t.im2col, t.kpad, t.patch_lin, t.patch_out, C, B * t.P));
+  if (t.gather_patch) {
+    RC(lin_gather(GEMM_GATHER_PATCH, pix, t.image, t.image, t.patch, t.patch_lin, t.patch_out, C, B * t.P));
+  } else {
+    KCHK(im2col_patch(pix, t.im2col, B, t.image, t.patch, t.kpad, stream));
+    RC(lin(t.im2col, t.kpad, t.patch_lin, t.patch_out, C, B * t.P));
+  }
   KCHK(vit_assemble_tokens(t.patch_out, t.cls, t.pos, t.h, B, t.P, C, stream));
   KCHK(layernorm_lp(t.h, t.pre_g, t.pre_b, t.x, rows, C, 1e-5f, nullptr, 0, stream));
   if (t.fold) {
diff --git a/vstar_amd/csrc/gemm.hip b/vstar_amd/csrc/gemm.hip
--- a/vstar_amd/csrc/gemm.hip
+++ b/vstar_amd/csrc/gemm.hip
@@ -25,6 +25,8 @@
   return gemm_map_row(r, group, gstride, off);
 }
 
+__device__ __attribute__((aligned(16))) const uint32_t g_zero_chunk[4] = {0u, 0u, 0u, 0u};
+
 #define BAR128()                                       \
   do {                                                 \
     __builtin_amdgcn_sched_barrier(0);                 \
@@ -32,9 +34,10 @@
     __builtin_amdgcn_sched_barrier(0);                 \
   } while (0)
 
-template <int EPI, bool OUT_F32, int MODE, int NW = 2>
+template <int EPI, bool OUT_F32, int MODE, int NW = 2, int GA = GEMM_GATHER_NONE>
 __global__ __launch_bounds__(MODE == 5 ? (NW == 4 ? 576 : 320) : 256, (NW != 4 && (MODE == 2 || NW == 1)) ? 2 : 1) void gemm128_kernel(const GemmParams p) {
   constexpr bool LDR = MODE == 5;
+  static_assert(GA == GEMM_GATHER_NONE || (MODE == 2 && NW == 2), "gathered A: double-buffer kernel only");
   constexpr int STAGES = LDR ? 3 : MODE;
   static_assert(NW == 2 || LDR, "the 128 x 64 and 128 x 256 tiles exist in loader-wave mode only");
   constexpr int BN = 64 * NW;
@@ -70,23 +73,82 @@
   const int st_c = lane & 7;
   const lp_t* a_src[4];
   const lp_t* w_src[4];
+  int g_y[4], g_x[4];
 #pragma unroll
   for (int i = 0; i < 4; ++i) {
     const int r = (i * 4 + wave) * 8 + st_r;
     const int cg = st_c ^ ((r >> 1) & 7);
     int ar = m0 + r;
     ar = ar < p.M ? ar : p.M - 1;
-    a_src[i] = p.A + map_row(ar, p.a_group, p.a_gstride, p.a_off) * p.lda + cg * 8;
+    if constexpr (GA == GEMM_GATHER_CONV3X3) {
+      a_src[i] = p.A + (int64_t)ar * p.g_c + cg * 8;
+      g_x[i] = ar % p.g_w;
+      g_y[i] = (ar / p.g_w) % p.g_h;
+    } else if constexpr (GA == GEMM_GATHER_PATCH) {
+      const int gx = p.g_w / p.g_c, gy = p.g_h / p.g_c;
+      const int px = ar % gx, py = (ar / gx) % gy, b = ar / (gx * gy);
+      a_src[i] = p.A + ((int64_t)b * 3 * p.g_h + py * p.g_c) * p.g_w + px * p.g_c;
+    } else {
+      a_src[i] = p.A + map_row(ar, p.a_group, p.a_gstride, p.a_off) * p.lda + cg * 8;
+    }
     w_src[i] = p.W + (int64_t)(n0 + r) * p.K + cg * 8;
+  }
+  int pk = 0, pc = 0, pky = 0, pkx = 0;
+  if constexpr (GA == GEMM_GATHER_PATCH) {
+    const int ps = p.g_c;
+    pk = (st_c ^ (((wave & 1) * 4 + (st_r >> 1)) & 7)) * 8;
+    pc = pk / (ps * ps);
+    pky = (pk - pc * ps * ps) / ps;
+    pkx = pk - pc * ps * ps - pky * ps;
   }
 
   auto stage = [&](int buf, int k0) {
     char* base = smem + buf * LDS_BUF;
-#pragma unroll
-    for (int i = 0; i < 4; ++i) {
-      const int piece = (i * 4 + wave) * 1024;
-      __builtin_amdgcn_global_load_lds((gptr_t)(a_src[i] + k0), (lptr_t)(base + piece), 16, 0, 0);
-      __builtin_amdgcn_global_load_lds((gptr_t)(w_src[i] + k0), (lptr_t)(base + LDS_TILE + piece), 16, 0, 0);
+    if constexpr (GA == GEMM_GATHER_CONV3X3) {
+      const int tap = k0 / p.g_c, c0 = k0 - tap * p.g_c;
+      const int dy = tap / 3 - 1, dx = tap - (tap / 3) * 3 - 1;
+      const int64_t off = ((int64_t)dy * p.g_w + dx) * p.g_c + c0;
+#pragma unroll
+      for (int i = 0; i < 4; ++i) {
+        const int piece = (i * 4 + wave) * 1024;
+        const bool in = (unsigned)(g_y[i] + dy) < (unsigned)p.g_h && (unsigned)(g_x[i] + dx) < (unsigned)p.g_w;
+        const lp_t* src = in ? a_src[i] + off : (const lp_t*)g_zero_chunk;
+        __builtin_amdgcn_global_load_lds((gptr_t)src, (lptr_t)(base + piece), 16, 0, 0);
+        __builtin_amdgcn_global_load_lds((gptr_t)(w_src[i] + k0), (lptr_t)(base + LDS_TILE + piece), 16, 0, 0);
+      }
+    } else if constexpr (GA == GEMM_GATHER_PATCH) {
+      const int ps = p.g_c;
+      const int64_t koff = ((int64_t)pc * p.g_h + pky) * p.g_w + pkx;
+      const bool whole = pk + 8 <= p.g_k && pkx + 8 <= ps;
+#pragma unroll
+      for (int i = 0; i < 4; ++i) {
+        const int piece = (i * 4 + wave) * 1024;
+        const lp_t* src = a_src[i] + koff;
+        if (whole && ((uintptr_t)src & 15) == 0) {
+          __builtin_amdgcn_global_load_lds((gptr_t)src, (lptr_t)(base + piece), 16, 0, 0);
+        } else {
+          lpx8 v = {0, 0, 0, 0, 0, 0, 0, 0};
+          int c = pc, ky = pky, kx = pkx;
+#pragma unroll
+          for (int e = 0; e < 8; ++e) {
+            if (pk + e < p.g_k) v[e] = (short)a_src[i][((int64_t)c * p.g_h + ky) * p.g_w + kx];
+            if (++kx == ps) { kx = 0; if (++ky == ps) { ky = 0; ++c; } }
+          }
+          *(lpx8*)(base + piece + lane * 16) = v;
+        }
+        __builtin_amdgcn_global_load_lds((gptr_t)(w_src[i] + k0), (lptr_t)(base + LDS_TILE + piece), 16, 0, 0);
+      }
+      pk += BK;
+      pkx += BK;
+      while (pkx >= ps) { pkx -= ps; ++pky; }
+      while (pky >= ps) { pky -= ps; ++pc; }
+    } else {
+#pragma unroll
+      for (int i = 0; i < 4; ++i) {
+        const int piece = (i * 4 + wave) * 1024;
+        __builtin_amdgcn_global_load_lds((gptr_t)(a_src[i] + k0), (lptr_t)(base + piece), 16, 0, 0);
+        __builtin_amdgcn_global_load_lds((gptr_t)(w_src[i] + k0), (lptr_t)(base + LDS_TILE + piece), 16, 0, 0);
+      }
     }
   };
 
@@ -252,12 +314,12 @@
 int gemm_device_cus();
 namespace {
 
-template <int EPI, bool OUT_F32, int MODE, int NW = 2>
+template <int EPI, bool OUT_F32, int MODE, int NW = 2, int GA = GEMM_GATHER_NONE>
 hipError_t launch_stages(const GemmParams& p, hipStream_t s) {
   t_last_mode = MODE == 5 ? (NW == 4 ? 7 : (NW == 1 ? 6 : 5)) : MODE;
   if (t_plan_only) return hipSuccess;
   static bool attr_done = false;
-  auto kern = gemm128_kernel<EPI, OUT_F32, MODE, NW>;
+  auto kern = gemm128_kernel<EPI, OUT_F32, MODE, NW, GA>;
   constexpr int bn = 64 * NW;
   constexpr int lds = (MODE == 5 ? 3 : MODE) * (LDS_TILE + bn * BK * 2);
   if (!attr_done) {
@@ -309,11 +371,34 @@
   return n_cu;
 }
 
+static hipError_t gemm_gather_lp(const GemmParams& p, int epilogue, bool out_f32, hipStream_t s) {
+  if (out_f32 || p.a_group > 0 || p.row_scale || p.sumsq_out || p.rope_cs || p.a_scale || p.a_mx || p.c_mx || ((uintptr_t)p.W & 15))
+    return hipErrorInvalidValue;
+  if (p.g_h <= 0 || p.g_w <= 0 || p.g_c <= 0) return hipErrorInvalidValue;
+  if (p.a_gather == GEMM_GATHER_CONV3X3) {
+    if (p.g_c % BK || p.K != 9 * p.g_c || p.M % (p.g_h * p.g_w) || ((uintptr_t)p.A & 15)) return hipErrorInvalidValue;
+    t_last_tile = 128;
+    if (epilogue == VSTAR_EPI_NONE) return launch_stages<VSTAR_EPI_NONE, false, 2, 2, GEMM_GATHER_CONV3X3>(p, s);
+    if (epilogue == VSTAR_EPI_GELU) return launch_stages<VSTAR_EPI_GELU, false, 2, 2, GEMM_GATHER_CONV3X3>(p, s);
+    return hipErrorInvalidValue;
+  }
+  if (p.a_gather == GEMM_GATHER_PATCH) {
+    const int ps = p.g_c;
+    if (p.g_h % ps || p.g_w % ps || p.g_k != 3 * ps * ps || p.K < p.g_k || p.K - p.g_k >= BK || p.M % ((p.g_h / ps) * (p.g_w / ps)) ||
+        ((uintptr_t)p.A & 1) || epilogue != VSTAR_EPI_NONE)
+      return hipErrorInvalidValue;
+    t_last_tile = 128;
+    return launch_stages<VSTAR_EPI_NONE, false, 2, 2, GEMM_GATHER_PATCH>(p, s);
+  }
+  return hipErrorInvalidValue;
+}
+
 hipError_t gemm_lp(const GemmParams& p, int epilogue, bool out_f32, hipStream_t s) {
   t_last_tile = 0;
   t_last_mode = 0;
   if (p.M <= 0 || p.N <= 0) return hipSuccess;
   if (p.K % BK != 0 || p.K <= 0 || p.norm_w) return hipErrorInvalidValue;
+  if (p.a_gather != GEMM_GATHER_NONE) return gemm_gather_lp(p, epilogue, out_f32, s);
   if (((uintptr_t)p.A & 15) || ((uintptr_t)p.W & 15) || (p.lda % 8)) return hipErrorInvalidValue;
   static const int env_force = [] { const char* e = getenv("VSTAR_GEMM_TILE"); return e ? atoi(e) : 0; }();
   const int force = p.tile_force ? p.tile_force : env_force;
diff --git a/vstar_amd/csrc/heads.hip b/vstar_amd/csrc/heads.hip
--- a/vstar_amd/csrc/heads.hip
+++ b/vstar_amd/csrc/heads.hip
@@ -88,6 +88,36 @@
   *(lpx8*)(A + idx * 8) = o;
 }
 
+__global__ void up2x_bilinear_kernel(const lp_t* __restrict__ src, lp_t* __restrict__ dst, int B, int h, int w, int C) {
+  const int cv = C >> 3;
+  const int H2 = 2 * h, W2 = 2 * w;
+  const int64_t idx = (int64_t)blockIdx.x * blockDim.x + threadIdx.x;
+  const int64_t total = (int64_t)B * H2 * W2 * cv;
+  if (idx >= total) return;
+  const int v = (int)(idx % cv);
+  const int64_t r = idx / cv;
+  const int xx = (int)(r % W2);
+  const int yy = (int)((r / W2) % H2);
+  const int b = (int)(r / ((int64_t)W2 * H2));
+  const float sy = fmaxf(0.5f * (yy + 0.5f) - 0.5f, 0.f), sx = fmaxf(0.5f * (xx + 0.5f) - 0.5f, 0.f);
+  const int y0 = (int)sy, x0 = (int)sx;
+  const int y1 = y0 + (y0 < h - 1 ? 1 : 0), x1 = x0 + (x0 < w - 1 ? 1 : 0);
+  const float ly = sy - y0, lx = sx - x0;
+  const lp_t* base = src + (int64_t)b * h * w * C + v * 8;
+  const lpx8 v00 = *(const lpx8*)(base + ((int64_t)y0 * w + x0) * C);
+  const lpx8 v01 = *(const lpx8*)(base + ((int64_t)y0 * w + x1) * C);
+  const lpx8 v10 = *(const lpx8*)(base + ((int64_t)y1 * w + x0) * C);
+  const lpx8 v11 = *(const lpx8*)(base + ((int64_t)y1 * w + x1) * C);
+  lpx8 o;
+#pragma unroll
+  for (int e = 0; e < 8; ++e) {
+    const float t = (1.f - ly) * ((1.f - lx) * lp2f((lp_t)v00[e]) + lx * lp2f((lp_t)v01[e])) +
+                    ly * ((1.f - lx) * lp2f((lp_t)v10[e]) + lx * lp2f((lp_t)v11[e]));
+    o[e] = (short)f2lp(t);
+  }
+  *(lpx8*)(dst + idx * 8) = o;
+}
+
 template <int C>
 __global__ void hyper_mask_kernel(const lp_t* __restrict__ hyper, const lp_t* __restrict__ up, float* __restrict__ out,
                                   int out_stride_crop, int B, int npix) {
@@ -231,6 +261,11 @@
                      w, C);
   return hipGetLastError();
 }
+hipError_t upsample2x_bilinear(const lp_t* src, lp_t* dst, int B, int h, int w, int C, hipStream_t s) {
+  if (C % 8) return hipErrorInvalidValue;
+  hipLaunchKernelGGL(up2x_bilinear_kernel, dim3(nblk((int64_t)B * 4 * h * w * (C / 8))), dim3(256), 0, s, src, dst, B, h, w, C);
+  return hipGetLastError();
+}
 hipError_t hyper_mask(const lp_t* hyper, const lp_t* up, float* out, int out_stride_crop, int B, int npix, int C,
                       hipStream_t s) {
   if (C != 32) return hipErrorInvalidValue;
diff --git a/vstar_amd/csrc/kernels.hpp b/vstar_amd/csrc/kernels.hpp
--- a/vstar_amd/csrc/kernels.hpp
+++ b/vstar_amd/csrc/kernels.hpp
@@ -26,7 +26,9 @@
   const lp_t* W_tiled;
   const uint8_t* a_mx; uint8_t* c_mx;
   uint8_t* c8; int64_t ldc8;
+  int a_gather; int g_h, g_w, g_c, g_k;
 };
+enum { GEMM_GATHER_NONE = 0, GEMM_GATHER_CONV3X3 = 1, GEMM_GATHER_PATCH = 2 };
 bool gemm_mx_supported(const GemmParams& p, int epilogue);
 hipError_t gemm_lp(const GemmParams& p, int epilogue, bool out_f32, hipStream_t s);
 constexpr int GEMM_TILE_4W = 2564;
@@ -91,6 +93,7 @@
                            int D, hipStream_t s);
 
 hipError_t im2col_patch(const lp_t* pix, lp_t* A, int B, int I, int ps, int Kpad, hipStream_t s);
+hipError_t im2col_patch_hw(const lp_t* pix, lp_t* A, int B, int IH, int IW, int ps, int Kpad, hipStream_t s);
 hipError_t vit_assemble_tokens(const lp_t* patch, const lp_t* cls, const lp_t* pos, lp_t* tokens, int B, int P,
                                int C, hipStream_t s);
 hipError_t llm_embed_text(const int32_t* ids, int L, int img_col, int P, const lp_t* table, int vocab, lp_t* x, int B,
@@ -106,6 +109,7 @@
                             int B, int rows_per_crop, hipStream_t s, int img_div = 1);
 hipError_t owl_box_finish(const float* raw, int ld, float* out, int out_stride_crop, int B, int grid, hipStream_t s, int img_div = 1);
 hipError_t upsample2x_im2col3x3(const lp_t* src, lp_t* A, int B, int h, int w, int C, hipStream_t s);
+hipError_t upsample2x_bilinear(const lp_t* src, lp_t* dst, int B, int h, int w, int C, hipStream_t s);
 hipError_t hyper_mask(const lp_t* hyper, const lp_t* up, float* out, int out_stride_crop, int B, int npix, int C,
                       hipStream_t s);
 hipError_t resize_bilinear_clamp(const float* in, int hin, int win, float* out, int hout, int wout, hipStream_t s, int clamp_min0 = 1);
```

After: 143.2 crops/s (median of 6 runs). About the same (+0.6%).
